# claudiotomasi/LearnMultigrid

Hardware: AMD Instinct MI355X
Metric: fine-level DoF*sweeps/s, 2-D Poisson V-cycle (higher is better)
Workload: dtype f64; 1 GPU; 2-D structured P1 Poisson 4096x4096 elements (16785409 DoF, 83861509 nnz, CSR fp64/int32), 6-level V(3,3) cycle, weighted Jacobi omega=0.80, tensor-product geometric transfer, Galerkin RAP by device SpGEMM; mode=vcycle, step=one full V-cycle, hipgraph=True, partition=row blocks of grid lines over 1 rank(s), sweep_variant=0, packed_csr=True, fine_level_format=stencil, problem=poisson, transfer=geometric

## Files before the change

include/lmg.h:

```cpp
#ifndef LMG_H
#define LMG_H

#include <stddef.h>
#include <stdint.h>

#ifdef __cplusplus
extern "C" {
#endif

#define LMG_VERSION 100

typedef enum {
    LMG_OK = 0,
    LMG_ERR_ARG = -1,
    LMG_ERR_ALIGN = -2,
    LMG_ERR_LAUNCH = -3,
    LMG_ERR_CAPACITY = -4,
    LMG_ERR_NODEVICE = -5
} lmg_status;

int lmg_version(void);
const char *lmg_status_string(int status);
int lmg_device_count(void);

int lmg_tune_set(const char *key, int value);
int lmg_tune_get(const char *key);

int64_t lmg_partials_count(int64_t n);

int lmg_csr_residual_norm2(int64_t n, int64_t nnz, const int32_t *d_rowptr, const int32_t *d_colidx,
                           const double *d_vals, const double *d_x, const double *d_b, double *d_r,
                           double *d_partials, double *d_norm2, void *stream);

int lmg_csr_jacobi(int64_t n, int64_t nnz, const int32_t *d_rowptr, const int32_t *d_colidx,
                   const double *d_vals, const double *d_x_in, const double *d_b, double omega,
                   double *d_x_out, void *stream);

int lmg_csr_spmv(int64_t n_rows, int64_t nnz, const int32_t *d_rowptr, const int32_t *d_colidx,
                 const double *d_vals, const double *d_x, double *d_y, double alpha, double beta,
                 void *stream);

int lmg_pcsr_tile_rows(void);
int lmg_pcsr_sweep(int mode, int64_t n, int64_t nnz, int32_t tile_rows, int32_t tile_cap,
                   const int32_t *d_tile_base,
                   const int32_t *d_tile_colbase, const uint8_t *d_rowlen, const void *d_col,
                   int colmode, const void *d_val, int valmode, const double *d_dict, int32_t ndict,
                   const double *d_x, const double *d_b, double *d_out, double alpha, double beta,
                   double *d_partials, double *d_norm2, void *stream);

int lmg_rpat_limits(int32_t *max_patterns, int32_t *max_entries);
int lmg_rpat_sweep(int mode, int64_t n, const uint8_t *d_pid, int32_t npat, int32_t nent, int32_t max_len,
                   const int32_t *d_pat_ptr, const int32_t *d_pat_off, const double *d_pat_val,
                   const double *d_x, const double *d_b, double *d_out, double alpha, double beta,
                   double *d_partials, double *d_norm2, void *stream);
int lmg_rpat_row_hash(int64_t n, const int32_t *d_rowptr, const int32_t *d_colidx, const double *d_vals,
                      uint64_t *d_hash, void *stream);
int lmg_rpat_claim(int64_t n, const uint8_t *d_pid, int32_t *d_rep, void *stream);
int lmg_rpat_verify(int64_t n, int64_t ncols, const int32_t *d_rowptr, const int32_t *d_colidx,
                    const double *d_vals, const uint8_t *d_pid, int32_t npat, const int32_t *d_pat_ptr,
                    const int32_t *d_pat_off, const double *d_pat_val, int32_t *d_mismatch, void *stream);

int lmg_rpat_sweep_grid(int mode, int64_t n, const int32_t *h_grid_map, const uint8_t *d_pid, int32_t npat,
                        int32_t nent, int32_t max_len, const int32_t *d_pat_ptr, const int32_t *d_pat_off,
                        const double *d_pat_val, const double *d_x, const double *d_b, double *d_out,
                        double alpha, double beta, double *d_partials, double *d_norm2, void *stream);
int lmg_rpat_row_hash_grid(int64_t n, const int32_t *h_grid_map, const int32_t *d_rowptr,
                           const int32_t *d_colidx, const double *d_vals, uint64_t *d_hash, void *stream);
int lmg_rpat_verify_grid(int64_t n, int64_t ncols, const int32_t *h_grid_map, const int32_t *d_rowptr,
                         const int32_t *d_colidx, const double *d_vals, const uint8_t *d_pid, int32_t npat,
                         const int32_t *d_pat_ptr, const int32_t *d_pat_off, const double *d_pat_val,
                         int32_t *d_mismatch, void *stream);

int lmg_stencil_limits(int32_t *max_patterns);
int lmg_stencil_sweep(int mode, int64_t n, int32_t line_stride, const uint8_t *d_pid, int32_t npat,
                      const double *d_st_val, const int32_t *d_st_mask, uint32_t union_mask, const double *d_x,
                      const double *d_b, double *d_out, double alpha, double beta, double *d_partials,
                      double *d_norm2, void *stream);

int lmg_stencil_smooth_supported(uint32_t union_mask);
int lmg_stencil_smooth(int64_t n, int32_t line_stride, const uint8_t *d_pid, int32_t npat,
                       const double *d_st_val, const int32_t *d_st_mask, uint32_t union_mask,
                       int32_t hot_pattern, const double *h_hot_val, int sweeps, const double *d_x_in,
                       const double *d_b, double omega, double *d_x_out, double *d_r_out, void *stream);

int lmg_stencil_smooth_tiled_supported(uint32_t union_mask);
int lmg_stencil_smooth_tiled(int64_t n, int32_t line_stride, const uint8_t *d_pid, int32_t npat,
                             const double *d_st_val, const int32_t *d_st_mask, uint32_t union_mask,
                             int32_t hot_pattern, const double *h_hot_val, int sweeps, const double *d_x_in,
                             const double *d_b, double omega, double *d_x_out, double *d_r_out, void *stream);
int lmg_stencil_smooth_tiled_prolong(int64_t n, int32_t line_stride, const uint8_t *d_pid, int32_t npat,
                                     const double *d_st_val, const int32_t *d_st_mask, uint32_t union_mask,
                                     int32_t hot_pattern, const double *h_hot_val, int sweeps, const double *d_x_in,
                                     const double *d_b, double omega, double *d_x_out, int64_t n_coarse,
                                     int32_t coarse_stride, const double *d_e_coarse, const uint8_t *d_p_pid,
                                     int32_t p_npat, const double *d_p_val, const int32_t *d_p_mask,
                                     const int32_t *h_hot_pairs, const double *h_hot_pval, void *stream);
int lmg_stencil_smooth_tiled_restrict(int64_t n, int32_t line_stride, const uint8_t *d_pid, int32_t npat,
                                      const double *d_st_val, const int32_t *d_st_mask, uint32_t union_mask,
                                      int32_t hot_pattern, const double *h_hot_val, int sweeps, const double *d_x_in,
                                      const double *d_b, double omega, double *d_x_out, int64_t n_coarse,
                                      int32_t coarse_stride, double *d_b_coarse, const uint8_t *d_r_pid,
                                      int32_t r_npat, const double *d_r_val, const int32_t *d_r_mask, int32_t hot_r,
                                      const double *h_hot_rval, void *stream);
int lmg_stencil_cheby_tiled(int64_t n, int32_t line_stride, const uint8_t *d_pid, int32_t npat,
                            const double *d_st_val, const int32_t *d_st_mask, uint32_t union_mask,
                            int32_t hot_pattern, const double *h_hot_val, int degree, const double *h_coef,
                            const double *d_x_in, const double *d_b, double *d_x_out, double *d_r_out, void *stream);
int lmg_stencil_cheby_tiled_prolong(int64_t n, int32_t line_stride, const uint8_t *d_pid, int32_t npat,
                                    const double *d_st_val, const int32_t *d_st_mask, uint32_t union_mask,
                                    int32_t hot_pattern, const double *h_hot_val, int degree, const double *h_coef,
                                    const double *d_x_in, const double *d_b, double *d_x_out, int64_t n_coarse,
                                    int32_t coarse_stride, const double *d_e_coarse, const uint8_t *d_p_pid,
                                    int32_t p_npat, const double *d_p_val, const int32_t *d_p_mask,
                                    const int32_t *h_hot_pairs, const double *h_hot_pval, void *stream);
int lmg_stencil_cheby_tiled_restrict(int64_t n, int32_t line_stride, const uint8_t *d_pid, int32_t npat,
                                     const double *d_st_val, const int32_t *d_st_mask, uint32_t union_mask,
                                     int32_t hot_pattern, const double *h_hot_val, int degree, const double *h_coef,
                                     const double *d_x_in, const double *d_b, double *d_x_out, int64_t n_coarse,
                                     int32_t coarse_stride, double *d_b_coarse, const uint8_t *d_r_pid,
                                     int32_t r_npat, const double *d_r_val, const int32_t *d_r_mask, int32_t hot_r,
                                     const double *h_hot_rval, void *stream);
int lmg_stencil_smooth_tiled_turnaround(int64_t n, int32_t line_stride, const uint8_t *d_pid, int32_t npat,
                                        const double *d_st_val, const int32_t *d_st_mask, uint32_t union_mask,
                                        int32_t hot_pattern, const double *h_hot_val, int sweeps_post, int sweeps_pre,
                                        const double *d_x_in, const double *d_b, double omega, double *d_x_out,
                                        int64_t n_coarse, int32_t coarse_stride, const double *d_e_coarse,
                                        const uint8_t *d_p_pid, int32_t p_npat, const double *d_p_val,
                                        const int32_t *d_p_mask, const int32_t *h_hot_pairs, const double *h_hot_pval,
                                        double *d_b_coarse, const uint8_t *d_r_pid, int32_t r_npat,
                                        const double *d_r_val, const int32_t *d_r_mask, int32_t hot_r,
                                        const double *h_hot_rval, void *stream);

int lmg_dia_smooth_supported(uint32_t union_mask);
int lmg_dia_fill(int64_t n, int32_t line_stride, const int32_t *d_rowptr, const int32_t *d_colidx, const double *d_vals,
                 uint32_t union_mask, double *d_dia, int32_t *d_mismatch, uint32_t *d_mask_out, void *stream);
int lmg_dia_smooth(int64_t n, int32_t line_stride, uint32_t union_mask, const double *d_dia, int sweeps,
                   const double *d_x_in, const double *d_b, double omega, double *d_x_out, double *d_r_out, void *stream);
int lmg_dia_cheby(int64_t n, int32_t line_stride, uint32_t union_mask, const double *d_dia, int degree,
                  const double *h_coef, const double *d_x_in, const double *d_b, double *d_x_out, double *d_r_out,
                  void *stream);
int lmg_dia_fill_f32(int64_t n, int32_t line_stride, const int32_t *d_rowptr, const int32_t *d_colidx, const double *d_vals,
                     uint32_t union_mask, float *d_dia, int32_t *d_mismatch, uint32_t *d_mask_out, void *stream);
int lmg_dia_smooth_f32(int64_t n, int32_t line_stride, uint32_t union_mask, const float *d_dia, int sweeps,
                       const double *d_x_in, const double *d_b, double omega, double *d_x_out, double *d_r_out,
                       void *stream);
int lmg_dia_cheby_f32(int64_t n, int32_t line_stride, uint32_t union_mask, const float *d_dia, int degree,
                      const double *h_coef, const double *d_x_in, const double *d_b, double *d_x_out, double *d_r_out,
                      void *stream);

int lmg_stencil_smooth_prolong_supported(uint32_t union_mask);
int lmg_stencil_smooth_prolong(int64_t n, int32_t line_stride, const uint8_t *d_pid, int32_t npat,
                               const double *d_st_val, const int32_t *d_st_mask, uint32_t union_mask,
                               int32_t hot_pattern, const double *h_hot_val, int sweeps, const double *d_x_in,
                               const double *d_b, double omega, double *d_x_out, int64_t n_coarse,
                               int32_t coarse_stride, const double *d_e_coarse, const uint8_t *d_p_pid,
                               int32_t p_npat, const double *d_p_val, const int32_t *d_p_mask,
                               const int32_t *h_hot_pairs, const double *h_hot_pval, void *stream);

int lmg_stencil_smooth_restrict(int64_t n, int32_t line_stride, const uint8_t *d_pid, int32_t npat,
                                const double *d_st_val, const int32_t *d_st_mask, uint32_t union_mask,
                                int32_t hot_pattern, const double *h_hot_val, int sweeps, const double *d_x_in,
                                const double *d_b, double omega, double *d_x_out, int64_t n_coarse,
                                int32_t coarse_stride, double *d_b_coarse, const uint8_t *d_r_pid,
                                int32_t r_npat, const double *d_r_val, const int32_t *d_r_mask, int32_t hot_r,
                                const double *h_hot_rval, void *stream);

int lmg_sell_sweep(int mode, int64_t n, const int64_t *d_slice_base, const int32_t *d_slice_len,
                   const int32_t *d_slice_cmin, const int32_t *d_rowlen, const void *d_col, int colmode,
                   const double *d_val, int32_t max_len, const double *d_x, const double *d_b, double *d_out,
                   double alpha, double beta, double *d_partials, double *d_norm2, void *stream);
int lmg_sell_slice_info(int64_t n, const int32_t *d_rowptr, const int32_t *d_colidx, int32_t *d_slice_len,
                        int32_t *d_cmin, int32_t *d_cmax, void *stream);
int lmg_sell_fill(int64_t n, const int32_t *d_rowptr, const int32_t *d_colidx, const double *d_vals,
                  const int64_t *d_slice_base, const int32_t *d_slice_cmin, int colmode, void *d_col_out,
                  double *d_val_out, void *stream);
int lmg_sell_sweep_f32(int mode, int64_t n, const int64_t *d_slice_base, const int32_t *d_slice_len,
                       const int32_t *d_slice_cmin, const int32_t *d_rowlen, const void *d_col, int colmode,
                       const float *d_val, int32_t max_len, const double *d_x, const double *d_b, double *d_out,
                       double alpha, double beta, double *d_partials, double *d_norm2, void *stream);
int lmg_sell_fill_f32(int64_t n, const int32_t *d_rowptr, const int32_t *d_colidx, const double *d_vals,
                      const int64_t *d_slice_base, const int32_t *d_slice_cmin, int colmode, void *d_col_out,
                      float *d_val_out, int32_t *d_flag, void *stream);

int64_t lmg_block_partials_count(int64_t n, int k);
int lmg_sell_sweep_block(int mode, int k, int64_t n, const int64_t *d_slice_base, const int32_t *d_slice_len,
                         const int32_t *d_slice_cmin, const int32_t *d_rowlen, const void *d_col, int colmode,
                         const double *d_val, int32_t max_len, const double *d_X, const double *d_B, double *d_Out,
                         double alpha, double beta, double *d_partials, double *d_norm2, void *stream);
int lmg_dense_gemv_block(int k, int64_t n, int64_t m, const double *d_M, const double *d_X, double *d_Y, void *stream);

int lmg_pcsr_tile_colrange(int64_t n, int32_t tile_rows, const int32_t *d_rowptr, const int32_t *d_colidx,
                           int32_t *d_cmin, int32_t *d_cmax, void *stream);
int lmg_pcsr_encode_cols16(int64_t n, int32_t tile_rows, const int32_t *d_rowptr, const int32_t *d_colidx,
                           const int32_t *d_colbase, uint16_t *d_out, void *stream);
int lmg_value_set_collect(const uint64_t *d_table, int64_t table_slots, uint64_t *d_out, int32_t cap, int32_t *d_count,
                          void *stream);
int lmg_value_set_insert(int64_t count, const double *d_vals, uint64_t *d_table, int64_t table_slots,
                         int32_t limit, int32_t *d_state, void *stream);
int lmg_value_encode(int64_t count, const double *d_vals, const double *d_dict, int32_t ndict, int width,
                     void *d_out, int32_t *d_missing, void *stream);
int lmg_csr_inverse_diagonal(int64_t n, const int32_t *d_rowptr, const int32_t *d_colidx, const double *d_vals,
                             double *d_dinv, void *stream);

int lmg_cheby_update(int64_t n, double a, double c, int first, const double *d_dinv, const double *d_r, double *d_d,
                     double *d_x, void *stream);
int lmg_csr_gershgorin(int64_t n, const int32_t *d_rowptr, const int32_t *d_colidx, const double *d_vals, double *d_lmax,
                       void *stream);

int lmg_line_factor(int64_t n, int32_t line_stride, int dir, const int32_t *d_rowptr, const int32_t *d_colidx,
                    const double *d_vals, double *d_lo, double *d_minv, double *d_cp, int32_t *d_flags, void *stream);
int lmg_line_solve(int64_t n, int32_t line_stride, int dir, int64_t first, int64_t step, const double *d_lo,
                   const double *d_minv, const double *d_cp, double *d_r, double omega, double *d_x, void *stream);

int lmg_line_factor_banded(int64_t n, int32_t line_stride, int dir, int band, const int32_t *d_rowptr,
                           const int32_t *d_colidx, const double *d_vals, double *d_fac, int32_t *d_flags, void *stream);
int lmg_line_solve_banded(int64_t n, int32_t line_stride, int dir, int band, int64_t first, int64_t step,
                          const double *d_fac, double *d_r, double omega, double *d_x, void *stream);

int lmg_csr_transpose_max_row(void);
int lmg_csr_transpose_count(int64_t nnz, int64_t ncols, const int32_t *d_colidx, int32_t *d_counts, void *stream);
int lmg_csr_transpose_fill(int64_t n, int64_t ncols, const int32_t *d_rowptr, const int32_t *d_colidx,
                           const double *d_vals, const int32_t *d_t_rowptr, int32_t *d_cursor, int32_t *d_t_colidx,
                           double *d_t_vals, void *stream);

int lmg_csr_gs_rows(const int32_t *d_rowptr, const int32_t *d_colidx, const double *d_vals,
                    double *d_x, const double *d_b, const int32_t *d_rows, int64_t nrows,
                    void *stream);

int lmg_csr_gs_schedule(const int32_t *d_rowptr, const int32_t *d_colidx, const double *d_vals,
                        double *d_x, const double *d_b, const int32_t *d_set_rows,
                        const int32_t *d_set_ptr, const int32_t *h_set_ptr, int64_t nsets,
                        int64_t max_set, int sweeps, void *stream);
int lmg_csr_gs_schedule_ell(int64_t n, const double *d_vals, double *d_x, const double *d_b, const int32_t *d_ell_row,
                            const int32_t *d_ell_start, const int32_t *d_ell_len, const int32_t *d_ell_cols,
                            int32_t ell_k, int64_t total_rows, const int32_t *d_set_ptr, int64_t nsets,
                            int sweeps, void *stream);

int lmg_stencil_gs_supported(uint32_t union_mask);
int64_t lmg_stencil_gs_work_bytes(int64_t n, int32_t line_stride);
int lmg_stencil_gs_sweep(int64_t n, int32_t line_stride, const uint8_t *d_pid, int32_t npat,
                         const double *d_st_val, const int32_t *d_st_mask, uint32_t union_mask,
                         int32_t hot_pattern, const double *h_hot_val, double *d_x, const double *d_b,
                         void *d_work, int sweeps, void *stream);
int lmg_stencil_gs_sweep_backward(int64_t n, int32_t line_stride, const uint8_t *d_pid, int32_t npat,
                                  const double *d_st_val, const int32_t *d_st_mask, uint32_t union_mask,
                                  int32_t hot_pattern, const double *h_hot_val, double *d_x, const double *d_b,
                                  void *d_work, int sweeps, void *stream);

int64_t lmg_host_gs_levels(int64_t n, const int32_t *h_rowptr, const int32_t *h_colidx,
                           int32_t *h_level_out);
int64_t lmg_host_greedy_colors(int64_t n, const int32_t *h_rowptr, const int32_t *h_colidx,
                               int32_t *h_color_out);
int64_t lmg_host_greedy_cf(int64_t n, const int32_t *h_rowptr, const int32_t *h_colidx, const double *h_vals,
                           int32_t *h_is_coarse_out);

int lmg_axpby(int64_t n, double alpha, const double *d_x, double beta, double *d_y, void *stream);
int lmg_vmul(int64_t n, double alpha, const double *d_x, const double *d_y, double *d_out, void *stream);
int lmg_copy(int64_t n, const double *d_src, double *d_dst, void *stream);
int lmg_zero(int64_t n, double *d_x, void *stream);
int lmg_dot(int64_t n, const double *d_x, const double *d_y, double *d_partials, double *d_out,
            void *stream);
int lmg_gather(int64_t n, const int32_t *d_idx, const double *d_x, double *d_buf, void *stream);
int lmg_scatter(int64_t n, const int32_t *d_idx, const double *d_buf, double *d_x, void *stream);

int lmg_krylov_max_vectors(void);
int64_t lmg_multi_partials_count(int64_t n, int k);
int lmg_multi_dot(int64_t n, int k, const double *d_V, int64_t ldv, const double *d_w, double *d_partials, double *d_out,
                  void *stream);
int lmg_multi_axpy(int64_t n, int k, int subtract, const double *d_V, int64_t ldv, const double *d_coef, double *d_w,
                   double *d_partials, double *d_norm2, void *stream);

int64_t lmg_block_dot_partials_count(int64_t n, int k);
int lmg_block_dot(int k, int64_t n, const double *d_X, const double *d_Y, double *d_partials, double *d_out, void *stream);
int lmg_block_cg_step(int k, int64_t n, const double *d_rz, const double *d_pAp, const double *d_tol2, double *d_mask,
                      const double *d_P, const double *d_AP, double *d_X, double *d_R, double *d_partials, double *d_rr,
                      void *stream);
int lmg_block_cg_direction(int k, int64_t n, const double *d_rz_new, const double *d_rz_old, const double *d_mask,
                           const double *d_Z, double *d_P, void *stream);

int64_t lmg_block_multi_partials_count(int64_t n, int k, int nb);
int lmg_block_multi_dot(int k, int64_t n, int nb, const double *d_V, int64_t ldb, const double *d_W, double *d_partials,
                        double *d_out, void *stream);
int lmg_block_multi_axpy(int k, int64_t n, const int *h_counts, int subtract, const double *d_V, int64_t ldb, const double *d_coef,
                         double *d_W, double *d_partials, double *d_norm2, void *stream);
int lmg_block_scale(int k, int64_t n, const double *h_scale, double *d_W, void *stream);

int lmg_dense_gemv(int64_t n, int64_t m, const double *d_M, const double *d_x, double *d_y,
                   void *stream);
int lmg_dense_gemv_blockdiag(int64_t nblocks, int64_t bs, const double *d_M, const double *d_x,
                             double *d_y, void *stream);

int lmg_dense_gemv_windows(int64_t nblocks, int64_t rows, int64_t cols, const double *d_M, const double *d_x,
                           int64_t x_stride, const double *d_z, int64_t z_stride, double alpha, double *d_y,
                           int64_t y_stride, void *stream);

int lmg_dense_gemv_windows_off(int64_t nblocks, int64_t rows, int64_t cols, const double *d_M, const double *d_x,
                               const int32_t *d_x_offsets, const double *d_z, int64_t z_stride, double alpha,
                               double *d_y, int64_t y_stride, void *stream);

int lmg_coarse_front(int64_t nblocks, int64_t bs, const double *d_M, const double *d_b, const int32_t *d_perm, double *d_y,
                     int64_t ntail, double *d_tail_out, void *stream);
int lmg_coarse_back(int64_t nblocks, int64_t rows, int64_t cols, const double *d_M, const double *d_x,
                    const int32_t *d_x_offsets, const double *d_z, int64_t z_stride, double alpha, const int32_t *d_perm,
                    double *d_out, int accumulate, int64_t ntail, void *stream);

int lmg_coarse_front_gather(int64_t nblocks, int64_t bs, const double *d_M, const double *d_b, const int32_t *d_idx,
                            double *d_y, int64_t ntail, const int32_t *d_tail_idx, double *d_tail_out, void *stream);
int lmg_coarse_back_gather(int64_t nblocks, int64_t rows, int64_t cols, const double *d_M, const double *d_x,
                           const int32_t *d_xidx, const double *d_z, int64_t z_stride, double alpha, const int32_t *d_oidx,
                           double *d_out, int accumulate, int64_t ntail, const int32_t *d_tail_idx, void *stream);

int lmg_batched_gemm(int64_t batch, int64_t M, int64_t N, int64_t K, double alpha, const double *d_A, int64_t lda,
                     int64_t stride_a, const double *d_B, int64_t ldb, int64_t stride_b, double beta, double *d_C,
                     int64_t ldc, int64_t stride_c, void *stream);
int lmg_copy2d(int64_t batch, int64_t rows, int64_t cols, double alpha, const double *d_src, int64_t ld_src,
               int64_t stride_src, double *d_dst, int64_t ld_dst, int64_t stride_dst, int accumulate, void *stream);

int lmg_pattern_parity_counts(int64_t n, int32_t line_stride, const uint8_t *d_pid, int32_t *d_counts, void *stream);
int lmg_block_copy(int64_t nblocks, int64_t bs, const double *d_src, int64_t src_stride, double *d_dst,
// ... 234 lines not shown
```

learnmultigrid_amd/_lib.py:

```python
import ctypes
import os
import subprocess

import torch

_HERE = os.path.dirname(os.path.abspath(__file__))
LIB_PATH = os.environ.get("LMG_LIB_PATH") or os.path.join(_HERE, "liblmg_hip.so")
CSRC = os.path.join(_HERE, "csrc")

_c = ctypes
_i64, _i32, _f64, _p, _cp = _c.c_int64, _c.c_int32, _c.c_double, _c.c_void_p, _c.c_char_p

SIGNATURES = {
    "lmg_version": (_c.c_int, []),
    "lmg_status_string": (_cp, [_c.c_int]),
    "lmg_device_count": (_c.c_int, []),
    "lmg_tune_set": (_c.c_int, [_cp, _c.c_int]),
    "lmg_tune_get": (_c.c_int, [_cp]),
    "lmg_partials_count": (_i64, [_i64]),
    "lmg_csr_residual_norm2": (_c.c_int, [_i64, _i64, _p, _p, _p, _p, _p, _p, _p, _p, _p]),
    "lmg_csr_jacobi": (_c.c_int, [_i64, _i64, _p, _p, _p, _p, _p, _f64, _p, _p]),
    "lmg_csr_spmv": (_c.c_int, [_i64, _i64, _p, _p, _p, _p, _p, _f64, _f64, _p]),
    "lmg_pcsr_tile_rows": (_c.c_int, []),
    "lmg_pcsr_sweep": (_c.c_int, [_c.c_int, _i64, _i64, _i32, _i32, _p, _p, _p, _p, _c.c_int, _p, _c.c_int, _p, _i32,
                                  _p, _p, _p, _f64, _f64, _p, _p, _p]),
    "lmg_rpat_limits": (_c.c_int, [_p, _p]),
    "lmg_rpat_sweep": (_c.c_int, [_c.c_int, _i64, _p, _i32, _i32, _i32, _p, _p, _p, _p, _p, _p, _f64, _f64, _p, _p, _p]),
    "lmg_rpat_row_hash": (_c.c_int, [_i64, _p, _p, _p, _p, _p]),
    "lmg_rpat_claim": (_c.c_int, [_i64, _p, _p, _p]),
    "lmg_rpat_verify": (_c.c_int, [_i64, _i64, _p, _p, _p, _p, _i32, _p, _p, _p, _p, _p]),
    "lmg_rpat_sweep_grid": (_c.c_int, [_c.c_int, _i64, _p, _p, _i32, _i32, _i32, _p, _p, _p, _p, _p, _p, _f64, _f64, _p, _p, _p]),
    "lmg_rpat_row_hash_grid": (_c.c_int, [_i64, _p, _p, _p, _p, _p, _p]),
    "lmg_rpat_verify_grid": (_c.c_int, [_i64, _i64, _p, _p, _p, _p, _p, _i32, _p, _p, _p, _p, _p]),
    "lmg_stencil_limits": (_c.c_int, [_p]),
    "lmg_stencil_sweep": (_c.c_int, [_c.c_int, _i64, _i32, _p, _i32, _p, _p, _c.c_uint32, _p, _p, _p, _f64, _f64, _p, _p, _p]),
    "lmg_stencil_smooth_supported": (_c.c_int, [_c.c_uint32]),
    "lmg_stencil_smooth": (_c.c_int, [_i64, _i32, _p, _i32, _p, _p, _c.c_uint32, _i32, _p, _c.c_int, _p, _p, _f64, _p, _p, _p]),
    "lmg_stencil_smooth_tiled_supported": (_c.c_int, [_c.c_uint32]),
    "lmg_stencil_smooth_tiled": (_c.c_int, [_i64, _i32, _p, _i32, _p, _p, _c.c_uint32, _i32, _p, _c.c_int, _p, _p, _f64, _p, _p, _p]),
    "lmg_stencil_smooth_tiled_prolong": (_c.c_int, [_i64, _i32, _p, _i32, _p, _p, _c.c_uint32, _i32, _p, _c.c_int, _p, _p, _f64, _p,
                                                    _i64, _i32, _p, _p, _i32, _p, _p, _p, _p, _p]),
    "lmg_stencil_smooth_tiled_restrict": (_c.c_int, [_i64, _i32, _p, _i32, _p, _p, _c.c_uint32, _i32, _p, _c.c_int, _p, _p, _f64, _p,
                                                     _i64, _i32, _p, _p, _i32, _p, _p, _i32, _p, _p]),
    "lmg_stencil_cheby_tiled": (_c.c_int, [_i64, _i32, _p, _i32, _p, _p, _c.c_uint32, _i32, _p, _c.c_int, _p, _p, _p, _p, _p, _p]),
    "lmg_stencil_cheby_tiled_prolong": (_c.c_int, [_i64, _i32, _p, _i32, _p, _p, _c.c_uint32, _i32, _p, _c.c_int, _p, _p, _p, _p,
                                                   _i64, _i32, _p, _p, _i32, _p, _p, _p, _p, _p]),
    "lmg_stencil_cheby_tiled_restrict": (_c.c_int, [_i64, _i32, _p, _i32, _p, _p, _c.c_uint32, _i32, _p, _c.c_int, _p, _p, _p, _p,
                                                    _i64, _i32, _p, _p, _i32, _p, _p, _i32, _p, _p]),
    "lmg_stencil_smooth_tiled_turnaround": (_c.c_int, [_i64, _i32, _p, _i32, _p, _p, _c.c_uint32, _i32, _p, _c.c_int, _c.c_int, _p,
                                                       _p, _f64, _p, _i64, _i32, _p, _p, _i32, _p, _p, _p, _p,
                                                       _p, _p, _i32, _p, _p, _i32, _p, _p]),
    "lmg_dia_smooth_supported": (_c.c_int, [_c.c_uint32]),
    "lmg_dia_fill": (_c.c_int, [_i64, _i32, _p, _p, _p, _c.c_uint32, _p, _p, _p, _p]),
    "lmg_dia_smooth": (_c.c_int, [_i64, _i32, _c.c_uint32, _p, _c.c_int, _p, _p, _f64, _p, _p, _p]),
    "lmg_dia_cheby": (_c.c_int, [_i64, _i32, _c.c_uint32, _p, _c.c_int, _p, _p, _p, _p, _p, _p]),
    "lmg_dia_fill_f32": (_c.c_int, [_i64, _i32, _p, _p, _p, _c.c_uint32, _p, _p, _p, _p]),
    "lmg_dia_smooth_f32": (_c.c_int, [_i64, _i32, _c.c_uint32, _p, _c.c_int, _p, _p, _f64, _p, _p, _p]),
    "lmg_dia_cheby_f32": (_c.c_int, [_i64, _i32, _c.c_uint32, _p, _c.c_int, _p, _p, _p, _p, _p, _p]),
    "lmg_stencil_smooth_prolong_supported": (_c.c_int, [_c.c_uint32]),
    "lmg_stencil_smooth_prolong": (_c.c_int, [_i64, _i32, _p, _i32, _p, _p, _c.c_uint32, _i32, _p, _c.c_int, _p, _p, _f64, _p,
                                              _i64, _i32, _p, _p, _i32, _p, _p, _p, _p, _p]),
    "lmg_stencil_smooth_restrict": (_c.c_int, [_i64, _i32, _p, _i32, _p, _p, _c.c_uint32, _i32, _p, _c.c_int, _p, _p, _f64, _p,
                                               _i64, _i32, _p, _p, _i32, _p, _p, _i32, _p, _p]),
    "lmg_sell_sweep": (_c.c_int, [_c.c_int, _i64, _p, _p, _p, _p, _p, _c.c_int, _p, _i32, _p, _p, _p, _f64, _f64, _p, _p, _p]),
    "lmg_sell_slice_info": (_c.c_int, [_i64, _p, _p, _p, _p, _p, _p]),
    "lmg_sell_fill": (_c.c_int, [_i64, _p, _p, _p, _p, _p, _c.c_int, _p, _p, _p]),
    "lmg_sell_sweep_f32": (_c.c_int, [_c.c_int, _i64, _p, _p, _p, _p, _p, _c.c_int, _p, _i32, _p, _p, _p, _f64, _f64, _p, _p, _p]),
    "lmg_sell_fill_f32": (_c.c_int, [_i64, _p, _p, _p, _p, _p, _c.c_int, _p, _p, _p, _p]),
    "lmg_block_partials_count": (_i64, [_i64, _c.c_int]),
    "lmg_sell_sweep_block": (_c.c_int, [_c.c_int, _c.c_int, _i64, _p, _p, _p, _p, _p, _c.c_int, _p, _i32, _p, _p, _p, _f64, _f64,
                                        _p, _p, _p]),
    "lmg_dense_gemv_block": (_c.c_int, [_c.c_int, _i64, _i64, _p, _p, _p, _p]),
    "lmg_pcsr_tile_colrange":(_c.c_int, [_i64, _i32, _p, _p, _p, _p, _p]),
    "lmg_pcsr_encode_cols16": (_c.c_int, [_i64, _i32, _p, _p, _p, _p, _p]),
    "lmg_value_set_collect": (_c.c_int, [_p, _i64, _p, _i32, _p, _p]),
    "lmg_value_set_insert": (_c.c_int, [_i64, _p, _p, _i64, _i32, _p, _p]),
    "lmg_value_encode": (_c.c_int, [_i64, _p, _p, _i32, _c.c_int, _p, _p, _p]),
    "lmg_csr_inverse_diagonal": (_c.c_int, [_i64, _p, _p, _p, _p, _p]),
    "lmg_cheby_update": (_c.c_int, [_i64, _f64, _f64, _c.c_int, _p, _p, _p, _p, _p]),
    "lmg_csr_gershgorin": (_c.c_int, [_i64, _p, _p, _p, _p, _p]),
    "lmg_line_factor": (_c.c_int, [_i64, _i32, _c.c_int, _p, _p, _p, _p, _p, _p, _p, _p]),
    "lmg_line_solve": (_c.c_int, [_i64, _i32, _c.c_int, _i64, _i64, _p, _p, _p, _p, _f64, _p, _p]),
    "lmg_line_factor_banded": (_c.c_int, [_i64, _i32, _c.c_int, _c.c_int, _p, _p, _p, _p, _p, _p]),
    "lmg_line_solve_banded": (_c.c_int, [_i64, _i32, _c.c_int, _c.c_int, _i64, _i64, _p, _p, _f64, _p, _p]),
    "lmg_csr_transpose_max_row": (_c.c_int, []),
    "lmg_csr_transpose_count": (_c.c_int, [_i64, _i64, _p, _p, _p]),
    "lmg_csr_transpose_fill": (_c.c_int, [_i64, _i64, _p, _p, _p, _p, _p, _p, _p, _p]),
    "lmg_csr_gs_rows": (_c.c_int, [_p, _p, _p, _p, _p, _p, _i64, _p]),
    "lmg_csr_gs_schedule": (_c.c_int, [_p, _p, _p, _p, _p, _p, _p, _p, _i64, _i64, _c.c_int, _p]),
    "lmg_csr_gs_schedule_ell": (_c.c_int, [_i64, _p, _p, _p, _p, _p, _p, _p, _i32, _i64, _p, _i64, _c.c_int, _p]),
    "lmg_stencil_gs_supported": (_c.c_int, [_c.c_uint32]),
    "lmg_stencil_gs_work_bytes": (_i64, [_i64, _i32]),
    "lmg_stencil_gs_sweep": (_c.c_int, [_i64, _i32, _p, _i32, _p, _p, _c.c_uint32, _i32, _p, _p, _p, _p, _c.c_int, _p]),
    "lmg_stencil_gs_sweep_backward": (_c.c_int, [_i64, _i32, _p, _i32, _p, _p, _c.c_uint32, _i32, _p, _p, _p, _p, _c.c_int, _p]),
    "lmg_host_gs_levels": (_i64, [_i64, _p, _p, _p]),
    "lmg_host_greedy_colors": (_i64, [_i64, _p, _p, _p]),
    "lmg_host_greedy_cf": (_i64, [_i64, _p, _p, _p, _p]),
    "lmg_axpby": (_c.c_int, [_i64, _f64, _p, _f64, _p, _p]),
    "lmg_vmul": (_c.c_int, [_i64, _f64, _p, _p, _p, _p]),
    "lmg_copy": (_c.c_int, [_i64, _p, _p, _p]),
    "lmg_zero": (_c.c_int, [_i64, _p, _p]),
    "lmg_dot": (_c.c_int, [_i64, _p, _p, _p, _p, _p]),
    "lmg_gather": (_c.c_int, [_i64, _p, _p, _p, _p]),
    "lmg_scatter": (_c.c_int, [_i64, _p, _p, _p, _p]),
    "lmg_krylov_max_vectors": (_c.c_int, []),
    "lmg_multi_partials_count": (_i64, [_i64, _c.c_int]),
    "lmg_multi_dot": (_c.c_int, [_i64, _c.c_int, _p, _i64, _p, _p, _p, _p]),
    "lmg_multi_axpy": (_c.c_int, [_i64, _c.c_int, _c.c_int, _p, _i64, _p, _p, _p, _p, _p]),
    "lmg_block_dot_partials_count": (_i64, [_i64, _c.c_int]),
    "lmg_block_dot": (_c.c_int, [_c.c_int, _i64, _p, _p, _p, _p, _p]),
    "lmg_block_cg_step": (_c.c_int, [_c.c_int, _i64, _p, _p, _p, _p, _p, _p, _p, _p, _p, _p, _p]),
    "lmg_block_cg_direction": (_c.c_int, [_c.c_int, _i64, _p, _p, _p, _p, _p, _p]),
    "lmg_block_multi_partials_count": (_i64, [_i64, _c.c_int, _c.c_int]),
    "lmg_block_multi_dot": (_c.c_int, [_c.c_int, _i64, _c.c_int, _p, _i64, _p, _p, _p, _p]),
    "lmg_block_multi_axpy": (_c.c_int, [_c.c_int, _i64, _p, _c.c_int, _p, _i64, _p, _p, _p, _p, _p]),
    "lmg_block_scale": (_c.c_int, [_c.c_int, _i64, _p, _p, _p]),
    "lmg_dense_gemv": (_c.c_int, [_i64, _i64, _p, _p, _p, _p]),
    "lmg_dense_gemv_blockdiag": (_c.c_int, [_i64, _i64, _p, _p, _p, _p]),
    "lmg_dense_gemv_windows": (_c.c_int, [_i64, _i64, _i64, _p, _p, _i64, _p, _i64, _f64, _p, _i64, _p]),
    "lmg_dense_gemv_windows_off": (_c.c_int, [_i64, _i64, _i64, _p, _p, _p, _p, _i64, _f64, _p, _i64, _p]),
    "lmg_coarse_front": (_c.c_int, [_i64, _i64, _p, _p, _p, _p, _i64, _p, _p]),
    "lmg_coarse_back": (_c.c_int, [_i64, _i64, _i64, _p, _p, _p, _p, _i64, _f64, _p, _p, _c.c_int, _i64, _p]),
    "lmg_coarse_front_gather": (_c.c_int, [_i64, _i64, _p, _p, _p, _p, _i64, _p, _p, _p]),
    "lmg_coarse_back_gather": (_c.c_int, [_i64, _i64, _i64, _p, _p, _p, _p, _i64, _f64, _p, _p, _c.c_int, _i64, _p, _p]),
    "lmg_batched_gemm": (_c.c_int, [_i64, _i64, _i64, _i64, _f64, _p, _i64, _i64, _p, _i64, _i64, _f64, _p, _i64, _i64, _p]),
    "lmg_copy2d": (_c.c_int, [_i64, _i64, _i64, _f64, _p, _i64, _i64, _p, _i64, _i64, _c.c_int, _p]),
    "lmg_pattern_parity_counts": (_c.c_int, [_i64, _i32, _p, _p, _p]),
    "lmg_block_copy": (_c.c_int, [_i64, _i64, _p, _i64, _p, _i64, _p]),
    "lmg_csr_to_dense": (_c.c_int, [_i64, _i64, _p, _p, _p, _p, _p]),
    "lmg_batched_inverse": (_c.c_int, [_i64, _i32, _p, _p, _p, _p]),
    "lmg_spgemm_count": (_c.c_int, [_i64, _p, _p, _p, _p, _p, _p]),
    "lmg_spgemm_symbolic": (_c.c_int, [_i64, _p, _p, _p, _p, _p, _i32, _p, _p]),
    "lmg_spgemm_numeric": (_c.c_int, [_i64, _p, _p, _p, _p, _p, _p, _p, _i32, _p, _p, _p, _p]),
    "lmg_spgemm_numeric_record": (_c.c_int, [_i64, _p, _p, _p, _p, _p, _p, _p, _i32, _p, _p, _p, _p, _p, _p, _p]),
    "lmg_spgemm_numeric_replay": (_c.c_int, [_i64, _p, _p, _p, _p, _p, _p, _i32, _p, _p, _p, _p, _p, _p]),
    "lmg_spgemm_long_rows": (_c.c_int, [_c.c_int, _i64, _p, _p, _p, _p, _p, _p, _p, _i64, _i32, _p, _p, _p, _p, _p, _p, _p]),
    "lmg_scan_scratch_count": (_i64, [_i64]),
    "lmg_exclusive_scan_i32": (_c.c_int, [_i64, _p, _p, _p, _p]),
    "lmg_p1_assemble_2d": (_c.c_int, [_i64, _p, _p, _p, _p, _p, _p, _p, _f64, _p, _p, _p, _p, _p, _p]),
    "lmg_l2_coupling_count": (_c.c_int, [_i64, _i64, _p, _p, _p, _p]),
    "lmg_l2_coupling_fill": (_c.c_int, [_c.c_int, _i64, _i64, _p, _p, _p, _p, _p, _p]),
    "lmg_l2p2d_limits": (_c.c_int, [_p, _p]),
    "lmg_l2p2d_cell_count": (_c.c_int, [_i64, _p, _p, _p, _p, _i32, _p, _p]),
    "lmg_l2p2d_cell_fill": (_c.c_int, [_i64, _p, _p, _p, _p, _i32, _i64, _p, _p, _p]),
    "lmg_l2p2d_cand_count": (_c.c_int, [_i64, _p, _p, _p, _i64, _p, _p, _p, _p, _i32, _p, _p, _p, _p]),
    "lmg_l2p2d_cand_fill": (_c.c_int, [_i64, _p, _p, _p, _i64, _p, _p, _p, _p, _i32, _p, _p, _i64, _i32, _p, _p, _p]),
    "lmg_l2p2d_rows_count": (_c.c_int, [_i64, _i64, _p, _p, _p, _p, _p, _p, _i64, _i64, _p, _p, _p, _p, _p, _f64, _p, _p]),
    "lmg_l2p2d_rows_fill": (_c.c_int, [_c.c_int, _i64, _i64, _p, _p, _p, _p, _p, _p, _i64, _i64, _p, _p, _p, _p, _p, _f64,
                                       _i64, _i32, _p, _p, _p, _p]),
    "lmg_nmg2d_check": (_c.c_int, [_i64, _p, _p, _p, _p, _p]),
    "lmg_nmg2d_count": (_c.c_int, [_i64, _p, _p, _p, _p, _p, _p, _p]),
    "lmg_nmg2d_patches": (_c.c_int, [_i64, _p, _p, _i64, _p, _p, _p, _p, _p, _p, _p, _p]),
    "lmg_nmg2d_contrib": (_c.c_int, [_i64, _i64, _i64, _p, _p, _p, _p, _p]),
    "lmg_nmg2d_fold": (_c.c_int, [_i64, _p, _p, _p, _p, _i64, _p, _p, _p, _p]),
    "lmg_nmg2d_normalize": (_c.c_int, [_i64, _p, _p, _p, _p]),
    "lmg_nmg2d_dneighs": (_c.c_int, [_i64, _p, _p, _p, _p, _p]),
    "lmg_nmg2d_cut_mark": (_c.c_int, [_i64, _p, _p, _p, _p, _p]),
    "lmg_nmg2d_cut_fill": (_c.c_int, [_i64, _p, _p, _p, _p, _p, _p, _p, _p]),
    "lmg_mesh2d_limits": (_c.c_int, [_p]),
    "lmg_mesh2d_construct": (_c.c_int, [_i64, _i64, _p, _p, _p, _p]),
    "lmg_mesh2d_check": (_c.c_int, [_i64, _i64, _p, _p, _p]),
    "lmg_mesh2d_edge_keys": (_c.c_int, [_i64, _p, _p, _p]),
    "lmg_mesh2d_edge_runs": (_c.c_int, [_i64, _i64, _p, _p, _p, _p, _p, _p]),
    "lmg_mesh2d_refine": (_c.c_int, [_i64, _i64, _i64, _p, _p, _p, _p, _p, _p, _p, _p, _p, _p]),
    "lmg_mesh2d_n2e_fill": (_c.c_int, [_i64, _p, _p, _p, _p]),
    "lmg_mesh2d_rows_count": (_c.c_int, [_i64, _i64, _p, _p, _p, _p, _p]),
    "lmg_mesh2d_rows_fill": (_c.c_int, [_i64, _i64, _p, _p, _p, _i64, _i32, _p, _p, _p]),
    "lmg_csr_identity_rows": (_c.c_int, [_i64, _p, _p, _p, _p, _p, _p, _p, _p]),
    "lmg_amg_strength_count": (_c.c_int, [_i64, _p, _p, _p, _f64, _p, _p]),
    "lmg_amg_strength_fill": (_c.c_int, [_i64, _p, _p, _p, _f64, _p, _p, _p]),
    "lmg_amg_pmis_keys": (_c.c_int, [_i64, _p, _p, _p, _p, _p, _p]),
    "lmg_amg_pmis_select": (_c.c_int, [_i64, _p, _p, _p, _p, _p, _p, _p, _p]),
    "lmg_amg_pmis_blocks": (_i64, [_i64]),
    "lmg_amg_pmis_update": (_c.c_int, [_i64, _p, _p, _p, _p, _p, _p, _p]),
    "lmg_amg_interp_count": (_c.c_int, [_i64, _p, _p, _p, _p, _p]),
    "lmg_amg_interp_fill": (_c.c_int, [_i64, _p, _p, _p, _p, _p, _p, _p, _p, _p, _p, _p, _p]),
    "lmg_amg_smooth_count": (_c.c_int, [_i64, _p, _p, _p, _p, _p, _p, _p, _p, _p, _p, _p, _f64, _f64, _p, _p]),
    "lmg_amg_smooth_fill": (_c.c_int, [_i64, _p, _p, _p, _p, _p, _p, _p, _p, _p, _p, _p, _f64, _f64, _p, _p, _p, _p]),
    "lmg_sa_diagonal": (_c.c_int, [_i64, _p, _p, _p, _p, _p]),
    "lmg_sa_strength_count": (_c.c_int, [_i64, _p, _p, _p, _p, _f64, _p, _p]),
    "lmg_sa_strength_fill": (_c.c_int, [_i64, _p, _p, _p, _p, _f64, _p, _p, _p]),
    "lmg_sa_graph_count": (_c.c_int, [_i64, _p, _p, _p, _p, _p, _p]),
    "lmg_sa_graph_fill": (_c.c_int, [_i64, _p, _p, _p, _p, _p, _p, _p]),
    "lmg_sa_mis2_init": (_c.c_int, [_i64, _p, _p, _p, _p]),
    "lmg_sa_mis2_t1": (_c.c_int, [_i64, _p, _p, _p, _p, _p]),
    "lmg_sa_mis2_t2": (_c.c_int, [_i64, _p, _p, _p, _p, _p, _p]),
    "lmg_sa_mis2_c1": (_c.c_int, [_i64, _p, _p, _p, _p, _p, _p]),
    "lmg_sa_blocks": (_i64, [_i64]),
    "lmg_sa_mis2_update": (_c.c_int, [_i64, _p, _p, _p, _p, _p, _p, _p, _p]),
    "lmg_sa_assign1": (_c.c_int, [_i64, _p, _p, _p, _p, _p, _p]),
    "lmg_sa_assign2": (_c.c_int, [_i64, _p, _p, _p, _p, _p, _p]),
    "lmg_sa_tentative_count": (_c.c_int, [_i64, _i64, _p, _p, _p]),
    "lmg_sa_tentative_pattern": (_c.c_int, [_i64, _i64, _p, _p, _p, _p, _p, _p]),
    "lmg_sa_norms": (_c.c_int, [_i64, _p, _p, _p, _p, _p, _p]),
    "lmg_sa_tentative_fill": (_c.c_int, [_i64, _i64, _p, _p, _p, _p, _p, _p]),
    "lmg_sa_row_states": (_c.c_int, [_i64, _p, _p, _p]),
    "lmg_color_select": (_c.c_int, [_i64, _p, _p, _p, _p, _p, _p, _p]),
    "lmg_color_blocks": (_i64, [_i64]),
    "lmg_color_assign": (_c.c_int, [_i64, _p, _p, _p, _p, _p, _p, _p, _p, _p]),
    "lmg_color_twin_count": (_c.c_int, [_i64, _i32, _p, _p, _p, _p, _p, _p, _p, _p]),
    "lmg_color_twin_fill": (_c.c_int, [_i64, _p, _p, _p, _p, _p, _p, _p, _p, _p]),
    "lmg_color_twin_refill": (_c.c_int, [_i64, _p, _p, _p, _p]),
    "lmg_color_sweep": (_c.c_int, [_i32, _p, _p, _p, _p, _p, _p, _p, _i32, _i64, _p, _p, _c.c_int, _c.c_int, _p]),
    "lmg_graph_begin": (_c.c_int, [_p]),
    "lmg_graph_end": (_c.c_int, [_p, _c.POINTER(_p)]),
    "lmg_graph_launch": (_c.c_int, [_p, _p]),
    "lmg_graph_destroy": (_c.c_int, [_p]),
}

_lib = None


class LmgError(RuntimeError):
    pass


# ... 33 lines not shown
```

learnmultigrid_amd/csrc/lmg_common.hpp:

```cpp
#pragma once
#include <hip/hip_runtime.h>
#include <limits.h>
#include <stdint.h>
#include <string.h>
#include <type_traits>
#include "lmg.h"

#define LMG_WAVE 64

#define LMG_CHECK_LAUNCH()                                          \
    do {                                                            \
        hipError_t e__ = hipGetLastError();                         \
        if (e__ != hipSuccess) return LMG_ERR_LAUNCH;               \
    } while (0)

static inline hipStream_t lmg_stream(void *s) { return reinterpret_cast<hipStream_t>(s); }
static inline bool lmg_aligned16(const void *p) { return (reinterpret_cast<uintptr_t>(p) & 15u) == 0; }

constexpr int kLmgBlock = 256;
constexpr int kLmgMaxGrid = 256 * 8;

static inline unsigned lmg_grid_for(int64_t n, int per_block)
{
    int64_t g = (n + per_block - 1) / per_block;
    if (g > kLmgMaxGrid) g = kLmgMaxGrid;
    if (g < 1) g = 1;
    return (unsigned)g;
}

enum { MODE_RESIDUAL = 0, MODE_JACOBI = 1, MODE_SPMV = 2 };

static inline int lmg_check_sweep_args(int mode, const double *x, const double *b, const double *out,
                                       const double *partials, const double *norm2)
{
    if (mode == MODE_SPMV) {
        if (!out || x == out) return LMG_ERR_ARG;
    } else if (mode == MODE_JACOBI) {
        if (!b || !out || x == out) return LMG_ERR_ARG;
    } else if (mode == MODE_RESIDUAL) {
        if (!b || (partials == nullptr) != (norm2 == nullptr) || (!out && !partials)) return LMG_ERR_ARG;
    } else {
        return LMG_ERR_ARG;
    }
    return LMG_OK;
}

int lmg_reduce_partials(const double *partials, int64_t count, double *norm2, hipStream_t st);
int lmg_reduce_partials_strided(const double *partials, int64_t count, int k, double *norm2, hipStream_t st);

__device__ __forceinline__ int lmg_xcd_tile(int tiles_per_xcd)
{
    return (int)(blockIdx.x & 7u) * tiles_per_xcd + (int)(blockIdx.x >> 3);
}
struct LmgXcdTiles {
    int begin, end, first, stride;
};
__device__ __forceinline__ LmgXcdTiles lmg_xcd_tiles(int tiles, int tiles_per_xcd)
{
    LmgXcdTiles o;
    const int xcd = (int)(blockIdx.x & 7u), slot = (int)(blockIdx.x >> 3);
    o.stride = (int)(gridDim.x >> 3);
    o.begin = xcd * tiles_per_xcd;
    o.end = min(tiles, o.begin + tiles_per_xcd);
    o.first = o.begin + slot;
    return o;
}
template <int BLOCK, typename Kernel>
static inline unsigned lmg_persistent_grid(Kernel kernel, size_t lds_bytes, int max_per_cu, int tune_per_cu,
                                           int tiles_per_xcd)
{
    int per_cu = 0;
    if (hipOccupancyMaxActiveBlocksPerMultiprocessor(&per_cu, kernel, BLOCK, lds_bytes) != hipSuccess || per_cu < 1)
        per_cu = 4;
    if (per_cu > max_per_cu) per_cu = max_per_cu;
    if (tune_per_cu > 0 && tune_per_cu < per_cu) per_cu = tune_per_cu;
    int64_t grid = 256 * (int64_t)per_cu;
    if (grid > (int64_t)tiles_per_xcd * 8) grid = (int64_t)tiles_per_xcd * 8;
    return (unsigned)grid;
}

__device__ __forceinline__ double lmg_wave_sum(double v)
{
#pragma unroll
    for (int off = LMG_WAVE / 2; off > 0; off >>= 1) v += __shfl_down(v, off, LMG_WAVE);
    return v;
}

template <int BLOCK>
__device__ __forceinline__ double lmg_block_sum(double v, double *s_red)
{
    v = lmg_wave_sum(v);
    const int lane = threadIdx.x & (LMG_WAVE - 1), wave = threadIdx.x / LMG_WAVE;
    if (lane == 0) s_red[wave] = v;
    __syncthreads();
    double tot = 0.0;
    if (threadIdx.x == 0) {
#pragma unroll
        for (int w = 0; w < BLOCK / LMG_WAVE; ++w) tot += s_red[w];
    }
    return tot;
}

template <int CTRL, bool BOUND_CTRL>
__device__ __forceinline__ double lmg_dpp_shift(double old, double src)
{
    const int lo = __builtin_amdgcn_update_dpp(__double2loint(old), __double2loint(src), CTRL, 0xf, 0xf, BOUND_CTRL);
    const int hi = __builtin_amdgcn_update_dpp(__double2hiint(old), __double2hiint(src), CTRL, 0xf, 0xf, BOUND_CTRL);
    return __hiloint2double(hi, lo);
}
template <bool BOUND_CTRL>
__device__ __forceinline__ double dpp_lower(double src)
{
    return lmg_dpp_shift<0x138, BOUND_CTRL>(0.0, src);
}
template <bool BOUND_CTRL>
__device__ __forceinline__ double dpp_upper(double src)
{
    return lmg_dpp_shift<0x130, BOUND_CTRL>(0.0, src);
}
__device__ __forceinline__ double dpp_from_lower_lane(double src, double lane0) { return lmg_dpp_shift<0x138, false>(lane0, src); }
__device__ __forceinline__ double dpp_from_upper_lane(double src, double lane63) { return lmg_dpp_shift<0x130, false>(lane63, src); }

typedef double d2 __attribute__((ext_vector_type(2)));
struct __attribute__((aligned(8))) d2u { double a, b; };

constexpr int kMaxPat = 64;
constexpr unsigned kMask9 = 0x1FFu;
constexpr unsigned kMask5 = 0x0BAu;
constexpr unsigned kMask1D = 0x038u;
constexpr unsigned kMask7a = 0x1BBu;
constexpr unsigned kMask7b = 0x0FEu;
constexpr unsigned kMaskUpper = 0x007u;
constexpr unsigned kMaskLower = 0x1C0u;
constexpr unsigned kMaskCorners = 0x145u;
constexpr unsigned kMaskOffLine = kMaskUpper | kMaskLower;



struct LmgTuneKey {
    const char *key;
    int *value;
    int lo, hi;
    int nlist, list[6];
};
constexpr LmgTuneKey lmg_tune_range(const char *key, int *value, int lo, int hi = INT_MAX)
{
    return {key, value, lo, hi, 0, {}};
}
template <typename... V>
constexpr LmgTuneKey lmg_tune_list(const char *key, int *value, V... v)
{
    return {key, value, 0, 0, (int)sizeof...(V), {v...}};
}
constexpr LmgTuneKey kLmgTuneEnd = {nullptr, nullptr, 0, 0, 0, {}};
extern const LmgTuneKey lmg_tune_sweep[], lmg_tune_pcsr[], lmg_tune_rpat[], lmg_tune_stencil[], lmg_tune_fused[],
    lmg_tune_tile[], lmg_tune_dia[], lmg_tune_sell[], lmg_tune_gsw[], lmg_tune_gs[];

static inline const LmgTuneKey *lmg_tune_find(const LmgTuneKey *table, const char *key)
{
    for (; table->key; ++table)
        if (strcmp(table->key, key) == 0) return table;
    return nullptr;
}
static inline bool lmg_tune_accepts(const LmgTuneKey &k, int v)
{
    if (k.nlist == 0) return v >= k.lo && v <= k.hi;
    for (int i = 0; i < k.nlist; ++i)
        if (k.list[i] == v) return true;
    return false;
}

template <int LO, int HI, typename F>
int lmg_with_sweeps(int sweeps, F &&f)
{
    if constexpr (LO < HI) {
        if (sweeps == LO) return f(std::integral_constant<int, LO>{});
        return lmg_with_sweeps<LO + 1, HI>(sweeps, f);
    } else {
        return f(std::integral_constant<int, HI>{});
    }
}
template <typename F>
int lmg_with_flag(bool flag, F &&f)
{
    return flag ? f(std::true_type{}) : f(std::false_type{});
}
template <unsigned... M, typename F>
int lmg_with_mask(uint32_t union_mask, F &&f)
{
    int rc = LMG_ERR_CAPACITY;
    (void)((union_mask == M && (rc = f(std::integral_constant<unsigned, M>{}), true)) || ...);
    return rc;
}
#define LMG_CT(c) decltype(c)::value

struct LmgOperator {
    int64_t n;
    int32_t line_stride;
    const uint8_t *pid;
    int32_t npat;
    const double *st_val;
    const int32_t *st_mask;
    uint32_t union_mask;
    int32_t hot_pattern;
    const double *h_hot_val;
};
struct LmgSolve {
    int sweeps;
    const double *x_in, *b;
    double omega;
    double *x_out, *r_out;
};
struct LmgProl {
    int64_t n_coarse;
    int32_t coarse_stride;
    const double *e_coarse;
    const uint8_t *p_pid;
    int32_t p_npat;
    const double *p_val;
    const int32_t *p_mask;
    const int32_t *h_hot_pairs;
    const double *h_hot_pval;
};
struct LmgRest {
    int64_t n_coarse;
    int32_t coarse_stride;
    double *b_coarse;
    const uint8_t *r_pid;
    int32_t r_npat;
    const double *r_val;
    const int32_t *r_mask;
    int32_t hot_r;
    const double *h_hot_rval;
};

static inline bool lmg_hot_usable(int32_t hot_pattern, int32_t npat, const double *h_hot_val)
{
    return hot_pattern >= 0 && hot_pattern < npat && h_hot_val && h_hot_val[4] != 0.0;
}

template <typename A>
int lmg_smooth_fill(A &a, const LmgOperator &op, const LmgSolve &v)
{
    const int64_t n = op.n;
    if (n < 0 || n >= A::kRowLimit || op.npat < 1 || op.npat > kMaxPat || (op.union_mask & ~kMask9)) return LMG_ERR_ARG;
    if (v.sweeps < 1 || v.sweeps > 3) return LMG_ERR_ARG;
    if (n == 0) return LMG_OK;
    if (A::kOneRowIsCapacity && n < 2) return LMG_ERR_CAPACITY;
    if (!op.pid || !op.st_val || !op.st_mask || !v.b || !v.x_out || v.x_in == v.x_out || v.r_out == v.x_out ||
        (v.r_out && v.r_out == v.x_in))
        return LMG_ERR_ARG;
    if (op.line_stride < 3 || op.line_stride > n) return LMG_ERR_ARG;
    a.n = (int)n;
    a.W = op.line_stride;
    a.lines = (int)((n + op.line_stride - 1) / op.line_stride);
    a.npat = op.npat;
    a.pid = op.pid;
    a.st_val = op.st_val;
    a.st_mask = op.st_mask;
    a.x = v.x_in;
    a.b = v.b;
    a.out = v.x_out;
    a.r = v.r_out;
    a.omega = v.omega;
    const bool hot = lmg_hot_usable(op.hot_pattern, op.npat, op.h_hot_val);
    a.hot = hot ? op.hot_pattern : -1;
    for (int k = 0; k < 9; ++k) a.hot_val[k] = hot ? op.h_hot_val[k] : 0.0;
    a.hot_rdiag = hot ? 1.0 / op.h_hot_val[4] : 0.0;
    a.ec = nullptr;
    a.nc = a.Wc = 0;
    a.ppid = nullptr;
    a.pp_val = nullptr;
    a.pp_mask = nullptr;
    a.pp_npat = 0;
    a.bc = nullptr;
    a.rpid = nullptr;
    a.rp_val = nullptr;
    a.rp_mask = nullptr;
    a.rp_npat = 0;
    a.phot[0] = a.phot[1] = a.rhot = -1;
    for (int k = 0; k < 9; ++k) a.phv[k] = a.rhv[k] = 0.0;
    return 1;
}

template <typename A>
int lmg_prol_check(const LmgOperator &op, const LmgSolve &v, const LmgProl &p)
{
    if (!v.x_in || !p.e_coarse || !p.p_pid || !p.p_val || !p.p_mask || p.p_npat < 1 || p.p_npat > kMaxPat) return LMG_ERR_ARG;
// ... 69 lines not shown
```

learnmultigrid_amd/csrc/stencil_fused.hip:

```cpp
#include "lmg_common.hpp"

#ifndef LMG_FUSED_NT_REST
#define LMG_FUSED_NT_REST 3
#endif
#ifndef LMG_FUSED_NT_PROL
#define LMG_FUSED_NT_PROL 0
#endif
#ifndef LMG_FUSED_NT_PLAIN
#define LMG_FUSED_NT_PLAIN 0
#endif

namespace {

constexpr int kBlock = 256;
constexpr int kWavesPerBlock = kBlock / LMG_WAVE;
constexpr int kStripCols = 2 * LMG_WAVE;

struct MArgs {
    static constexpr int64_t kRowLimit = (1ll << 29) - 4096;
    static constexpr bool kOneRowIsCapacity = true;
    static constexpr int64_t kProlMinCoarse = 1;
    static constexpr bool kProlStrideCovers = true, kProlChecksPairs = false;
    static constexpr int64_t kRestCoarseLimit = 1ll << 28;
    int n;
    int W;
    int lines;
    int npat;
    unsigned umask;
    int strips, segs, seg_lines;
    int items;
    int nb_strips;
    int segs_b, seg_lines_b;
    int edge_lines;
    int allow_fast;
    const unsigned char *pid;
    const double *st_val;
    const int *st_mask;
    const double *x;
    const double *b;
    double *out;
    double *r;
    double omega;
    int hot;
    double hot_val[9];
    double hot_rdiag;
    const double *ec;
    int nc, Wc;
    const unsigned char *ppid;
    const double *pp_val;
    const int *pp_mask;
    int pp_npat;
    int phot[2];
    double phv[9];
    double *bc;
    const unsigned char *rpid;
    const double *rp_val;
    const int *rp_mask;
    int rp_npat;
    int rhot;
    double rhv[9];
};

template <int H, bool PROL, bool REST> struct StripGeom {
    static constexpr bool EVEN = true;
    static constexpr int MLmin = REST ? H + 1 : H, MRmin = REST ? H + 1 : (PROL ? H + 2 : H);
    static constexpr int ML = EVEN ? ((MLmin + 1) & ~1) : MLmin;
    static constexpr int U = EVEN ? ((kStripCols - ML - MRmin) & ~1) : kStripCols - ML - MRmin;
};

struct Line {
    d2 x, b;
    double e;
    int pp;
    int rp;
    int praw;
    int ok;
};

typedef unsigned int u4 __attribute__((ext_vector_type(4)));
typedef unsigned int u2 __attribute__((ext_vector_type(2)));
constexpr unsigned kOOB = 0xFFFFFFF0u;

template <bool SIDES>
__device__ __forceinline__ void window(const d2 &c, double (&w)[4])
{
    w[1] = c.x;
    w[2] = c.y;
    if (SIDES) {
        w[0] = dpp_lower<true>(c.y);
        w[3] = dpp_upper<true>(c.x);
    } else {
        w[0] = w[3] = 0.0;
    }
}

template <unsigned UM>
__device__ __forceinline__ void apply_rows(const double *s_val, int pA, int pB, int mA, int mB,
                                           const d2 &u, const d2 &c, const d2 &d, double &accA, double &accB)
{
    constexpr bool DIAG = (UM & kMaskCorners) != 0;
    double wu[4], wc[4], wd[4];
    window<true>(c, wc);
    window<DIAG>(u, wu);
    window<DIAG>(d, wd);
    accA = 0.0;
    accB = 0.0;
#pragma unroll
    for (int s = 0; s < 9; ++s) {
        if (!((UM >> s) & 1u)) continue;
        const int cc = s / 3, dd = s % 3;
        const double *w = cc == 0 ? wu : (cc == 1 ? wc : wd);
        const double vA = s_val[pA * 9 + s], vB = s_val[pB * 9 + s];
        const double tA = accA + vA * w[dd], tB = accB + vB * w[dd + 1];
        accA = ((mA >> s) & 1) ? tA : accA;
        accB = ((mB >> s) & 1) ? tB : accB;
    }
}

template <unsigned UM>
__device__ __forceinline__ void apply_rows_hot(const double (&hv)[9], const d2 &u, const d2 &c,
                                               const d2 &d, double &accA, double &accB)
{
    constexpr bool DIAG = (UM & kMaskCorners) != 0;
    double wu[4], wc[4], wd[4];
    window<true>(c, wc);
    window<DIAG>(u, wu);
    window<DIAG>(d, wd);
    accA = 0.0;
    accB = 0.0;
#pragma unroll
    for (int s = 0; s < 9; ++s) {
        if (!((UM >> s) & 1u)) continue;
        const int cc = s / 3, dd = s % 3;
        const double *w = cc == 0 ? wu : (cc == 1 ? wc : wd);
        accA = accA + hv[s] * w[dd];
        accB = accB + hv[s] * w[dd + 1];
    }
}

#ifdef LMG_FUSED_TRACE
__device__ unsigned long long g_fused_trace[64 * 8];
__device__ int g_fused_trace_item;
#define LMG_TRACE(slot)                                                                                   \
    do {                                                                                                  \
        if (FAST && trace_me && (t - y_begin) < 64) g_fused_trace[(t - y_begin) * 8 + (slot)] = __builtin_readcyclecounter(); \
    } while (0)
#else
#define LMG_TRACE(slot)
#endif
#ifdef LMG_FUSED_WAVETIME
__device__ unsigned long long g_fused_wavetime[2 * LMG_FUSED_WAVETIME];
#endif

constexpr int kUF = 6;
constexpr int kNBR = 6;

struct Item {
    int strip, out_y0, out_y1;
};

__device__ __forceinline__ Item decode_item(const MArgs &a, int item)
{
    Item it;
    const int nb_items = a.nb_strips * a.segs_b;
    if (item < nb_items) {
        const int sb = item / a.segs_b, k = item - sb * a.segs_b;
        it.strip = sb == 0 ? 0 : a.strips - 1;
        it.out_y0 = k * a.seg_lines_b;
        it.out_y1 = min(a.lines, it.out_y0 + a.seg_lines_b);
        return it;
    }
    const int k = item - nb_items, ns = a.strips - a.nb_strips;
    const int seg = k / ns;
    it.strip = k - seg * ns + (a.nb_strips > 0 ? 1 : 0);
    if (a.edge_lines > 0) {
        if (seg == 0) {
            it.out_y0 = 0;
            it.out_y1 = a.edge_lines;
        } else if (seg == 1) {
            it.out_y0 = a.lines - a.edge_lines;
            it.out_y1 = a.lines;
        } else {
            it.out_y0 = a.edge_lines + (seg - 2) * a.seg_lines;
            it.out_y1 = min(a.lines - a.edge_lines, it.out_y0 + a.seg_lines);
        }
    } else {
        it.out_y0 = seg * a.seg_lines;
        it.out_y1 = min(a.lines, it.out_y0 + a.seg_lines);
    }
    return it;
}

struct Tables {
    const double *val;
    const int *mask;
    const double *rdiag;
    const double *pv;
    const int *pm;
    const double *rv;
    const int *rm;
};

template <int S, unsigned UM, bool RESID, bool ZERO, int PF, bool PROL, bool REST, bool FAST>
__device__ __forceinline__ void fused_march(const MArgs &a, const Tables &T, const int lane, const int strip, const int out_y0,
                                            const int out_y1)
{
    constexpr int H = S + (RESID ? 1 : 0) - (ZERO ? 1 : 0);
    const double *s_val = T.val;
    const int *s_mask = T.mask;
    const double *s_rdiag = T.rdiag;
    const double *s_pv = T.pv;
    const int *s_pm = T.pm;
    const double *s_rv = T.rv;
    const int *s_rm = T.rm;
    constexpr int U = StripGeom<H, PROL, REST>::U, ML = StripGeom<H, PROL, REST>::ML;
    constexpr int HL = H + (REST ? 1 : 0);
    const int n = a.n;
    const int64_t W = a.W;
    const int c0 = strip * U - ML;
    const int y_begin = out_y0 - HL - ((out_y0 - HL) & 1), y_end = out_y1 + HL;
    const int cidx = 2 * lane;
    const bool colA = cidx >= ML && cidx < ML + U && c0 + cidx < W;
    const bool colB = cidx + 1 >= ML && cidx + 1 < ML + U && c0 + cidx + 1 < W;
    const double omega = a.omega;
    const int hot2 = a.hot >= 0 ? (FAST ? (a.hot | (a.hot << 8)) : (a.hot | (a.hot << 8) | (3 << 16))) : -1;
    double hv[9];
#pragma unroll
    for (int s = 0; s < 9; ++s) hv[s] = a.hot_val[s];
    const double hrd = a.hot_rdiag;
    double hp[9];
#pragma unroll
    for (int s = 0; s < 9; ++s) hp[s] = PROL ? a.phv[s] : 0.0;
    const int okbits = FAST ? 0 : (3 << 16);
    const int hotq_even = (PROL && a.phot[0] >= 0) ? (a.phot[0] | okbits) : -1;
    const int hotq_odd = (PROL && a.phot[1] >= 0) ? (a.phot[1] | okbits) : -1;
    double e_prev = 0.0;

    const unsigned lane16 = (unsigned)lane * 16u, lane8 = (unsigned)lane * 8u, lane2 = (unsigned)lane * 2u;
    const unsigned st_off_ab = (colA && colB) ? lane16 : kOOB;
    const unsigned st_off_a = (colA && !colB) ? lane16 : kOOB;
    const unsigned st_off_c = colA ? lane8 : kOOB;

    constexpr int NTL = REST ? LMG_FUSED_NT_REST : (PROL ? LMG_FUSED_NT_PROL : LMG_FUSED_NT_PLAIN);
    auto fetch = [&](int y, Line &L) {
        if (FAST) {
#ifdef LMG_FUSED_HALOPROBE
            const int64_t i0 = (int64_t)min(max(y, out_y0), out_y1 - 1) * W + c0;
#else
            const int64_t i0 = (int64_t)y * W + c0;
#endif
            L.ok = 3;
            const unsigned short *pp2 = reinterpret_cast<const unsigned short *>(reinterpret_cast<const char *>(a.pid + i0) + lane2);
            L.praw = (int)((NTL & 4) ? __builtin_nontemporal_load(pp2) : *pp2);
            typedef double dv2 __attribute__((ext_vector_type(2), aligned(8)));
            const dv2 *pb = reinterpret_cast<const dv2 *>(reinterpret_cast<const char *>(a.b + i0) + lane16);
            const dv2 bb = (NTL & 1) ? __builtin_nontemporal_load(pb) : *pb;
            L.b.x = bb.x;
            L.b.y = bb.y;
            if (!ZERO) {
                const dv2 *px = reinterpret_cast<const dv2 *>(reinterpret_cast<const char *>(a.x + i0) + lane16);
                const dv2 xx = (NTL & 2) ? __builtin_nontemporal_load(px) : *px;
                L.x.x = xx.x;
                L.x.y = xx.y;
            } else {
                L.x.x = L.x.y = 0.0;
            }
            if (PROL) {
                unsigned short twop;
                __builtin_memcpy(&twop, reinterpret_cast<const char *>(a.ppid + i0) + lane2, 2);
                L.pp = (int)twop;
                const int64_t jc0 = (int64_t)((y + 1) >> 1) * a.Wc + (c0 >> 1);
                L.e = *reinterpret_cast<const double *>(reinterpret_cast<const char *>(a.ec + jc0) + lane8);
            } else {
                L.pp = 0;
                L.e = 0.0;
            }
            if (REST) {
                const int64_t jr0 = (int64_t)((y - S) >> 1) * a.Wc + (c0 >> 1);
                L.rp = (int)*(reinterpret_cast<const unsigned char *>(a.rpid + jr0) + lane);
            } else {
                L.rp = 0;
            }
            return;
        }
        const bool line_ok = y < y_end;
        const int yc = min(max(y, 0), a.lines - 1);
        const int64_t i = (int64_t)y * W + c0 + cidx;
        const bool okA = line_ok && i >= 0 && i < n, okB = line_ok && i + 1 >= 0 && i + 1 < n;
        const int64_t j = min(max(i, (int64_t)0), (int64_t)n - 2);
        L.ok = (okA ? 1 : 0) | (okB ? 2 : 0) | (i == -1 ? 4 : 0) | (i == (int64_t)n - 1 ? 8 : 0);
        unsigned short two;
        __builtin_memcpy(&two, a.pid + j, 2);
        L.praw = (int)two;
        const d2u bb = *reinterpret_cast<const d2u *>(a.b + j);
        L.b.x = bb.a;
        L.b.y = bb.b;
        if (!ZERO) {
            const d2u xx = *reinterpret_cast<const d2u *>(a.x + j);
            L.x.x = xx.a;
            L.x.y = xx.b;
        } else {
            L.x.x = L.x.y = 0.0;
        }
        if (PROL) {
            unsigned short twop;
            __builtin_memcpy(&twop, a.ppid + j, 2);
            L.pp = (int)twop;
            const int64_t jc = (int64_t)((yc + 1) >> 1) * a.Wc + (c0 >> 1) + lane;
            L.e = a.ec[min(max(jc, (int64_t)0), (int64_t)a.nc - 1)];
        } else {
            L.pp = 0;
            L.e = 0.0;
        }
        if (REST) {
            const int64_t jr = (int64_t)((y - S) >> 1) * a.Wc + (c0 >> 1) + lane;
            L.rp = (int)a.rpid[min(max(jr, (int64_t)0), (int64_t)a.nc - 1)];
        } else {
            L.rp = 0;
        }
    };
    const __amdgpu_buffer_rsrc_t rs_out = __builtin_amdgcn_make_buffer_rsrc(a.out, 0, (int)((unsigned)n * 8u), 0x00020000);
    const __amdgpu_buffer_rsrc_t rs_r = __builtin_amdgcn_make_buffer_rsrc((RESID && !REST) ? a.r : a.out, 0, (int)((unsigned)n * 8u), 0x00020000);
    const __amdgpu_buffer_rsrc_t rs_bc = __builtin_amdgcn_make_buffer_rsrc(REST ? a.bc : a.out, 0, (int)((unsigned)(REST ? a.nc : n) * 8u), 0x00020000);
    double hr[9];
#pragma unroll
    for (int s = 0; s < 9; ++s) hr[s] = REST ? a.rhv[s] : 0.0;
    double acc_cur = 0.0;
    int rp_cur = 0, rp_now = 0;
    bool st_cur = false, hot_cur = false;
    bool sty_cur = false;
    auto store2 = [&](const __amdgpu_buffer_rsrc_t &rs, double *base, int y, int p2, double va, double vb) {
        const bool yok = y >= out_y0 && y < out_y1;
        u4 v4;
        v4.x = (unsigned)__double2loint(va);
        v4.y = (unsigned)__double2hiint(va);
        v4.z = (unsigned)__double2loint(vb);
        v4.w = (unsigned)__double2hiint(vb);
        if (FAST) {
            const __amdgpu_buffer_rsrc_t rl = __builtin_amdgcn_make_buffer_rsrc(base + ((int64_t)y * W + c0), 0, yok ? 8 * kStripCols : 0, 0x00020000);
            __builtin_amdgcn_raw_buffer_store_b128(v4, rl, st_off_ab, 0, 0);
            u2 v2;
            v2.x = v4.x;
            v2.y = v4.y;
            __builtin_amdgcn_raw_buffer_store_b64(v2, rl, st_off_a, 0, 0);
            return;
        }
        const int64_t i = (int64_t)y * W + c0 + cidx;
        const bool stA = yok && colA && ((p2 >> 16) & 1), stB = yok && colB && ((p2 >> 17) & 1);
        __builtin_amdgcn_raw_buffer_store_b128(v4, rs, (stA && stB) ? (unsigned)i * 8u : kOOB, 0, 0);
        u2 v2;
        v2.x = stA ? v4.x : v4.z;
        v2.y = stA ? v4.y : v4.w;
        __builtin_amdgcn_raw_buffer_store_b64(v2, rs, (stA != stB) ? (unsigned)(stA ? i : i + 1) * 8u : kOOB, 0, 0);
    };

    d2 X[S + 1][3];
    d2 Bq[kNBR];
    int Pq[kNBR];
    bool Hq[kNBR];
    const d2 zero2 = {0.0, 0.0};
#pragma unroll
    for (int s = 0; s <= S; ++s) X[s][0] = X[s][1] = X[s][2] = zero2;
#pragma unroll
    for (int k = 0; k < kNBR; ++k) {
        Bq[k] = zero2;
        Pq[k] = 0;
        Hq[k] = false;
    }

    Line pre[PF];
#pragma unroll
    for (int u = 0; u < PF; ++u) fetch(y_begin + u, pre[u]);

    const int t_last = out_y1 - 1 + S + (RESID ? 1 : 0) + (REST ? 1 : 0);
#ifdef LMG_FUSED_TRACE
    const bool trace_me = lane == 0 && strip == g_fused_trace_item / 100000 && out_y0 <= g_fused_trace_item % 100000 &&
                          g_fused_trace_item % 100000 < out_y1;
#endif
    for (int tb = y_begin; tb <= t_last; tb += kUF) {
#pragma unroll
        for (int u = 0; u < kUF; ++u) {
            const int t = tb + u;
            LMG_TRACE(0);
            const int q0 = u % kNBR;
            {
                const Line &L = pre[u % PF];
                const bool okA = FAST || (L.ok & 1), okB = FAST || (L.ok & 2), up = !FAST && (L.ok & 4), down = !FAST && (L.ok & 8);
                d2 bv, xv;
                int pa, pb;
                if (FAST) {
                    bv = L.b;
                    xv = L.x;
                    pa = L.praw & 0xff;
                    pb = L.praw >> 8;
                } else {
                    bv.x = okA ? (down ? L.b.y : L.b.x) : 0.0;
                    bv.y = okB ? (up ? L.b.x : L.b.y) : 0.0;
                    xv.x = okA ? (down ? L.x.y : L.x.x) : 0.0;
                    xv.y = okB ? (up ? L.x.x : L.x.y) : 0.0;
                    pa = down ? (L.praw >> 8) & 0xff : L.praw & 0xff;
                    pb = up ? L.praw & 0xff : (L.praw >> 8) & 0xff;
                }
                if (REST) rp_now = L.rp;
                if (PROL) {
                    const bool odd = (u & 1) != 0;
                    int qa, qb, q2;
                    if (FAST) {
                        qa = L.pp & 0xff;
                        qb = L.pp >> 8;
                        q2 = L.pp;
                    } else {
                        qa = down ? (L.pp >> 8) & 0xff : L.pp & 0xff;
                        qb = up ? L.pp & 0xff : (L.pp >> 8) & 0xff;
                        q2 = (okA ? qa : 0) | ((okB ? qb : 0) << 8) | ((L.ok & 3) << 16);
                    }
                    const double en = L.e;
                    const double e0 = odd ? e_prev : en, e1 = en;
                    const double e0r = dpp_upper<true>(e0), e1r = dpp_upper<true>(e1);
                    double accA, accB;
                    if (__all(q2 == (odd ? hotq_odd : hotq_even))) {
                        if (!odd) {
                            accA = 0.0 + hp[0] * e0;
                            accB = (0.0 + hp[1] * e0) + hp[2] * e0r;
                        } else {
                            accA = (0.0 + hp[3] * e0) + hp[4] * e1;
                            accB = (((0.0 + hp[5] * e0) + hp[6] * e0r) + hp[7] * e1) + hp[8] * e1r;
                        }
                    } else {
                        const int mA = s_pm[qa], mB = s_pm[qb];
                        const double w[4] = {e0, e0r, e1, e1r};
                        accA = 0.0;
                        accB = 0.0;
#pragma unroll
                        for (int k = 0; k < 4; ++k) {
                            const double tA = accA + s_pv[qa * 4 + k] * w[k], tB = accB + s_pv[qb * 4 + k] * w[k];
                            accA = ((mA >> k) & 1) ? tA : accA;
                            accB = ((mB >> k) & 1) ? tB : accB;
                        }
                    }
                    xv.x = okA ? xv.x + accA : 0.0;
                    xv.y = okB ? xv.y + accB : 0.0;
                    e_prev = en;
                }
                Bq[q0] = bv;
                X[0][u % 3] = xv;
                Pq[q0] = FAST ? L.praw : ((okA ? pa : 0) | ((okB ? pb : 0) << 8) | ((L.ok & 3) << 16));
                Hq[q0] = __all(Pq[q0] == hot2);
            }
            LMG_TRACE(1);
            fetch(t + PF, pre[u % PF]);
            LMG_TRACE(2);
#pragma unroll
            for (int s = 1; s <= S; ++s) {
                const int q = ((u - s) % kNBR + kNBR) % kNBR;
                const int xm = ((u - s - 1) % 3 + 3) % 3, xc = ((u - s) % 3 + 3) % 3, xp = ((u - s + 1) % 3 + 3) % 3;
                const int p2 = Pq[q];
                const d2 bq = Bq[q];
                d2 nx;
                if (Hq[q]) {
                    if (ZERO && s == 1) {
                        nx.x = omega * (hrd * bq.x);
                        nx.y = omega * (hrd * bq.y);
                    } else {
                        double accA, accB;
                        apply_rows_hot<UM>(hv, X[s - 1][xm], X[s - 1][xc], X[s - 1][xp], accA, accB);
                        nx.x = X[s - 1][xc].x + omega * (hrd * (bq.x - accA));
                        nx.y = X[s - 1][xc].y + omega * (hrd * (bq.y - accB));
                    }
                } else {
                    const int pA = p2 & 0xff, pB = (p2 >> 8) & 0xff;
                    const int mA = s_mask[pA], mB = s_mask[pB];
                    if (ZERO && s == 1) {
                        nx.x = omega * (s_rdiag[pA] * bq.x);
                        nx.y = omega * (s_rdiag[pB] * bq.y);
                    } else {
                        double accA, accB;
                        apply_rows<UM>(s_val, pA, pB, mA, mB, X[s - 1][xm], X[s - 1][xc], X[s - 1][xp], accA, accB);
                        const double xa = X[s - 1][xc].x, xb = X[s - 1][xc].y;
                        const double rA = bq.x - accA, rB = bq.y - accB;
                        nx.x = (mA >> 16) ? xa : xa + omega * (s_rdiag[pA] * rA);
                        nx.y = (mB >> 16) ? xb : xb + omega * (s_rdiag[pB] * rB);
                    }
                    if (!FAST) {
                        if (!((p2 >> 16) & 1)) nx.x = 0.0;
                        if (!((p2 >> 17) & 1)) nx.y = 0.0;
                    }
                }
                X[s][xc] = nx;
                if (s == S) store2(rs_out, a.out, t - S, p2, nx.x, nx.y);
                LMG_TRACE(2 + s);
            }
            if (RESID) {
                const int y = t - S - 1;
                const int q = ((u - S - 1) % kNBR + kNBR) % kNBR;
                const int xm = ((u - S - 2) % 3 + 3) % 3, xc = ((u - S - 1) % 3 + 3) % 3, xp = ((u - S) % 3 + 3) % 3;
                const int p2 = Pq[q];
                double accA, accB;
                if (Hq[q]) {
                    apply_rows_hot<UM>(hv, X[S][xm], X[S][xc], X[S][xp], accA, accB);
                } else {
                    const int pA = p2 & 0xff, pB = (p2 >> 8) & 0xff;
                    apply_rows<UM>(s_val, pA, pB, s_mask[pA], s_mask[pB], X[S][xm], X[S][xc], X[S][xp], accA, accB);
                }
                if (!REST) {
                    store2(rs_r, a.r, y, p2, Bq[q].x - accA, Bq[q].y - accB);
                } else {
                    const double rA = Bq[q].x - accA, rB = Bq[q].y - accB;
                    const double wl[3] = {dpp_lower<true>(rB), rA, rB};
                    const bool y_odd = ((u - S - 1) & 1) != 0;
                    unsigned off_bc = kOOB;
                    bool emit_line = false;
                    double emit = 0.0;
                    if (!y_odd) {
                        if (hot_cur) {
#pragma unroll
                            for (int k = 0; k < 3; ++k) acc_cur = acc_cur + hr[3 + k] * wl[k];
                        } else {
                            const int mk = s_rm[rp_cur];
#pragma unroll
                            for (int k = 0; k < 3; ++k) {
                                const double tv = acc_cur + s_rv[rp_cur * 9 + 3 + k] * wl[k];
                                acc_cur = ((mk >> (3 + k)) & 1) ? tv : acc_cur;
                            }
                        }
                    } else {
                        if (hot_cur) {
#pragma unroll
                            for (int k = 0; k < 3; ++k) acc_cur = acc_cur + hr[6 + k] * wl[k];
                        } else {
                            const int mk = s_rm[rp_cur];
#pragma unroll
                            for (int k = 0; k < 3; ++k) {
                                const double tv = acc_cur + s_rv[rp_cur * 9 + 6 + k] * wl[k];
                                acc_cur = ((mk >> (6 + k)) & 1) ? tv : acc_cur;
                            }
                        }
                        emit = acc_cur;
                        emit_line = sty_cur;
                        if (!FAST && st_cur) off_bc = (unsigned)(((y - 1) >> 1) * a.Wc + (c0 >> 1) + lane) * 8u;
                        rp_cur = rp_now;
                        sty_cur = y + 1 >= out_y0 && y + 1 < out_y1;
                        st_cur = sty_cur && colA;
                        hot_cur = __all(!st_cur || rp_cur == a.rhot);
                        acc_cur = 0.0;
                        if (hot_cur) {
#pragma unroll
                            for (int k = 0; k < 3; ++k) acc_cur = acc_cur + hr[k] * wl[k];
                        } else {
                            const int mk = s_rm[rp_cur];
#pragma unroll
                            for (int k = 0; k < 3; ++k) {
                                const double tv = acc_cur + s_rv[rp_cur * 9 + k] * wl[k];
                                acc_cur = ((mk >> k) & 1) ? tv : acc_cur;
                            }
                        }
                    }
                    u2 v2;
                    v2.x = (unsigned)__double2loint(emit);
                    v2.y = (unsigned)__double2hiint(emit);
                    if (FAST) {
                        const __amdgpu_buffer_rsrc_t rl = __builtin_amdgcn_make_buffer_rsrc(
                            a.bc + ((int64_t)((y - 1) >> 1) * a.Wc + (c0 >> 1)), 0, (y_odd && emit_line) ? 8 * LMG_WAVE : 0, 0x00020000);
                        __builtin_amdgcn_raw_buffer_store_b64(v2, rl, st_off_c, 0, 0);
                    } else {
                        __builtin_amdgcn_raw_buffer_store_b64(v2, rs_bc, off_bc, 0, 0);
                    }
                }
            }
            LMG_TRACE(7);
        }
    }
}

template <int S, unsigned UM, bool RESID, bool ZERO, int PF, bool PROL = false, bool REST = false>
__global__ void __launch_bounds__(kBlock, (REST && S >= 3) ? 2 : 3) stencil_fused_kernel(MArgs a)
{
    static_assert(!PROL || (!RESID && !ZERO), "the correction is fused into post-smoothing passes only");
    static_assert(!REST || (RESID && !PROL), "the restriction replaces the store of the residual");
    static_assert(kUF % 3 == 0 && kUF % kNBR == 0 && kUF % PF == 0 && S + 2 <= kNBR, "ring periods");
    constexpr int H = S + (RESID ? 1 : 0) - (ZERO ? 1 : 0);
    __shared__ double s_val[kMaxPat * 9];
    __shared__ int s_mask[kMaxPat];
    __shared__ double s_rdiag[kMaxPat];
    __shared__ double s_pv[PROL ? kMaxPat * 4 : 1];
    __shared__ int s_pm[PROL ? kMaxPat : 1];
    __shared__ double s_rv[REST ? kMaxPat * 9 : 1];
    __shared__ int s_rm[REST ? kMaxPat : 1];

    const int t_ = threadIdx.x;
    for (int i = t_; i < a.npat * 9; i += kBlock) s_val[i] = a.st_val[i];
    for (int i = t_; i < a.npat; i += kBlock) {
        const int m = a.st_mask[i];
        const double dg = (m & 16) ? a.st_val[i * 9 + 4] : 0.0;
        s_rdiag[i] = dg != 0.0 ? 1.0 / dg : 0.0;
        s_mask[i] = dg == 0.0 ? (m | (1 << 16)) : m;
    }
    if (PROL) {
        for (int i = t_; i < a.pp_npat * 4; i += kBlock) s_pv[i] = a.pp_val[i];
        for (int i = t_; i < a.pp_npat; i += kBlock) s_pm[i] = a.pp_mask[i];
    }
    if (REST) {
        for (int i = t_; i < a.rp_npat * 9; i += kBlock) s_rv[i] = a.rp_val[i];
        for (int i = t_; i < a.rp_npat; i += kBlock) s_rm[i] = a.rp_mask[i];
    }
    __syncthreads();

    const int lane = t_ & (LMG_WAVE - 1);
    const int item = (int)blockIdx.x * kWavesPerBlock + __builtin_amdgcn_readfirstlane(t_ >> 6);
    if (item >= a.items) return;
    const Item it = decode_item(a, item);
    const Tables T = {s_val, s_mask, s_rdiag, s_pv, s_pm, s_rv, s_rm};

    constexpr int U = StripGeom<H, PROL, REST>::U, ML = StripGeom<H, PROL, REST>::ML;
    constexpr int HL = H + (REST ? 1 : 0);
    const int c0 = it.strip * U - ML;
    const int y_begin = it.out_y0 - HL - ((it.out_y0 - HL) & 1);
    const int t_last = it.out_y1 - 1 + S + (RESID ? 1 : 0) + (REST ? 1 : 0);
    const int y_fetch = y_begin + ((t_last - y_begin) / kUF + 1) * kUF - 1 + PF;
    bool fast = a.allow_fast && y_begin >= (REST ? S + 2 : 1) && y_fetch <= a.lines - 2 &&
                (int64_t)y_begin * a.W + c0 >= 0 && (int64_t)y_fetch * a.W + c0 + kStripCols < (int64_t)a.n;
    if (PROL) fast = fast && (int64_t)((y_fetch + 1) >> 1) * a.Wc + (c0 >> 1) + LMG_WAVE <= (int64_t)a.nc;
    if (REST) fast = fast && (int64_t)((y_fetch - S) >> 1) * a.Wc + (c0 >> 1) + LMG_WAVE <= (int64_t)a.nc;
#ifdef LMG_FUSED_WAVETIME
    const unsigned long long wt0 = __builtin_amdgcn_s_memrealtime();
#endif
    if (fast) fused_march<S, UM, RESID, ZERO, PF, PROL, REST, true>(a, T, lane, it.strip, it.out_y0, it.out_y1);
    else fused_march<S, UM, RESID, ZERO, PF, PROL, REST, false>(a, T, lane, it.strip, it.out_y0, it.out_y1);
#ifdef LMG_FUSED_WAVETIME
    if (lane == 0 && item < LMG_FUSED_WAVETIME) {
        g_fused_wavetime[2 * item] = wt0;
        g_fused_wavetime[2 * item + 1] = (__builtin_amdgcn_s_memrealtime() & ~3ull) | (fast ? 1ull : 0ull) | 2ull;
    }
#endif
}

int g_fused_seg_lines = 0;
int g_fused_seg_min_lines = 0;
int g_fused_seg_max_lines = 0x7fffffff;
int g_fused_pf = 0;
int g_fused_seg_lines_prol = 0;
int g_fused_seg_lines_rest = 0;
int g_fused_want_waves = 5120;
int g_fused_want_waves_rest3 = 2700;
int g_fused_floor_halos = 4;
int g_fused_balance = 1;
int g_fused_slow_pct = 55;
int g_fused_fast = 1;

template <int S, unsigned UM, bool RESID, bool ZERO, bool PROL = false, bool REST = false>
int launch4(MArgs a, hipStream_t st)
{
    constexpr int H = S + (RESID ? 1 : 0) - (ZERO ? 1 : 0);
    constexpr int U = StripGeom<H, PROL, REST>::U;
    constexpr int HL = H + (REST ? 1 : 0);
    a.strips = (a.W + U - 1) / U;
    int seg_lines = (a.lines >= g_fused_seg_min_lines && a.lines <= g_fused_seg_max_lines) ? g_fused_seg_lines : 0;
    if (PROL && g_fused_seg_lines_prol > 0) seg_lines = g_fused_seg_lines_prol;
    if (REST && g_fused_seg_lines_rest > 0) seg_lines = g_fused_seg_lines_rest;
    if (seg_lines <= 0) {
        const int want = ((REST || PROL) && S >= 3 && !ZERO) ? g_fused_want_waves_rest3 : g_fused_want_waves;
        const int want_segs = (want + a.strips - 1) / a.strips;
        seg_lines = (a.lines + want_segs - 1) / want_segs;
        const int floor_lines = H > 0 ? g_fused_floor_halos * H : 4;
        if (seg_lines < floor_lines) seg_lines = floor_lines;
    }
    a.seg_lines = seg_lines;
    a.allow_fast = g_fused_fast;
    a.nb_strips = 0;
    a.segs_b = 1;
    a.seg_lines_b = seg_lines;
    a.edge_lines = 0;
    if (g_fused_balance) {
        const int steps = seg_lines + 2 * HL;
        int slow = (steps * g_fused_slow_pct) / 100 - 2 * HL;
        if (slow < 2) slow = 2;
        if (slow < seg_lines) {
            a.nb_strips = a.strips < 2 ? a.strips : 2;
            a.seg_lines_b = slow;
            a.segs_b = (a.lines + slow - 1) / slow;
            int edge = slow < HL + 2 + kUF + 2 ? HL + 2 + kUF + 2 : slow;
            if (a.strips > a.nb_strips && a.lines >= 2 * edge + seg_lines) a.edge_lines = edge;
        }
    }
    if (a.edge_lines > 0) a.segs = 2 + (a.lines - 2 * a.edge_lines + seg_lines - 1) / seg_lines;
    else a.segs = (a.lines + seg_lines - 1) / seg_lines;
    a.items = a.nb_strips * a.segs_b + (a.strips - a.nb_strips) * a.segs;
    const int grid = (a.items + kWavesPerBlock - 1) / kWavesPerBlock;
    hipLaunchKernelGGL((stencil_fused_kernel<S, UM, RESID, ZERO, 2, PROL, REST>), dim3((unsigned)grid), dim3(kBlock), 0, st, a);
    LMG_CHECK_LAUNCH();
    return LMG_OK;
}

template <unsigned UM>
int launch_plain(MArgs a, int sweeps, bool resid, bool zero, hipStream_t st)
{
    return lmg_with_sweeps<1, 3>(sweeps, [&](auto s) {
        return lmg_with_flag(resid, [&](auto r) {
            return lmg_with_flag(zero, [&](auto z) { return launch4<LMG_CT(s), UM, LMG_CT(r), LMG_CT(z)>(a, st); });
        });
    });
}

template <unsigned UM>
int launch_prol(MArgs a, int sweeps, hipStream_t st)
{
    return lmg_with_sweeps<1, 3>(sweeps, [&](auto s) { return launch4<LMG_CT(s), UM, false, false, true>(a, st); });
}

template <unsigned UM>
int launch_rest(MArgs a, int sweeps, bool zero, hipStream_t st)
{
    return lmg_with_sweeps<1, 3>(sweeps, [&](auto s) {
        return lmg_with_flag(zero, [&](auto z) { return launch4<LMG_CT(s), UM, true, LMG_CT(z), false, true>(a, st); });
    });
}

MArgs own_fields(uint32_t union_mask)
{
    MArgs a;
    a.umask = union_mask;
    a.strips = a.segs = a.seg_lines = 0;
    a.items = a.nb_strips = a.edge_lines = a.allow_fast = 0;
    a.segs_b = a.seg_lines_b = 1;
    return a;
}

}

constexpr LmgTuneKey lmg_tune_fused[] = {
    lmg_tune_range("fused_seg_lines", &g_fused_seg_lines, 0),
    lmg_tune_range("fused_seg_min_lines", &g_fused_seg_min_lines, 0),
    lmg_tune_range("fused_seg_max_lines", &g_fused_seg_max_lines, 0),
    lmg_tune_list("fused_pf", &g_fused_pf, 0, 2),
    lmg_tune_range("fused_seg_lines_prol", &g_fused_seg_lines_prol, 0),
    lmg_tune_range("fused_seg_lines_rest", &g_fused_seg_lines_rest, 0),
    lmg_tune_range("fused_want_waves", &g_fused_want_waves, 1),
    lmg_tune_range("fused_want_waves_rest3", &g_fused_want_waves_rest3, 1),
    lmg_tune_range("fused_floor_halos", &g_fused_floor_halos, 1),
    lmg_tune_list("fused_balance", &g_fused_balance, 0, 1),
    lmg_tune_range("fused_slow_pct", &g_fused_slow_pct, 10, 100),
    lmg_tune_list("fused_fast", &g_fused_fast, 0, 1),
    kLmgTuneEnd,
};

extern "C" {

int lmg_stencil_smooth(int64_t n, int32_t line_stride, const uint8_t *pid, int32_t npat, const double *st_val,
                       const int32_t *st_mask, uint32_t union_mask, int32_t hot_pattern, const double *h_hot_val,
                       int sweeps, const double *x_in, const double *b, double omega, double *x_out, double *r_out,
                       void *stream)
{
    return lmg_fused_pass<kMask5, kMask9, kMask1D>(
        own_fields(union_mask), {n, line_stride, pid, npat, st_val, st_mask, union_mask, hot_pattern, h_hot_val},
        {sweeps, x_in, b, omega, x_out, r_out}, nullptr, nullptr, [&](const MArgs &a, auto m) {
            return launch_plain<LMG_CT(m)>(a, sweeps, r_out != nullptr, x_in == nullptr, lmg_stream(stream));
        });
}

int lmg_stencil_smooth_prolong(int64_t n, int32_t line_stride, const uint8_t *pid, int32_t npat, const double *st_val,
                               const int32_t *st_mask, uint32_t union_mask, int32_t hot_pattern, const double *h_hot_val,
                               int sweeps, const double *x_in, const double *b, double omega, double *x_out,
                               int64_t n_coarse, int32_t coarse_stride, const double *e_coarse, const uint8_t *p_pid,
                               int32_t p_npat, const double *p_val, const int32_t *p_mask, const int32_t *h_hot_pairs,
                               const double *h_hot_pval, void *stream)
{
    const LmgProl p = {n_coarse, coarse_stride, e_coarse, p_pid, p_npat, p_val, p_mask, h_hot_pairs, h_hot_pval};
    return lmg_fused_pass<kMask5, kMask9>(
        own_fields(union_mask), {n, line_stride, pid, npat, st_val, st_mask, union_mask, hot_pattern, h_hot_val},
        {sweeps, x_in, b, omega, x_out, nullptr}, &p, nullptr,
        [&](const MArgs &a, auto m) { return launch_prol<LMG_CT(m)>(a, sweeps, lmg_stream(stream)); });
}

int lmg_stencil_smooth_restrict(int64_t n, int32_t line_stride, const uint8_t *pid, int32_t npat, const double *st_val,
                                const int32_t *st_mask, uint32_t union_mask, int32_t hot_pattern, const double *h_hot_val,
                                int sweeps, const double *x_in, const double *b, double omega, double *x_out,
                                int64_t n_coarse, int32_t coarse_stride, double *b_coarse, const uint8_t *r_pid,
                                int32_t r_npat, const double *r_val, const int32_t *r_mask, int32_t hot_r,
                                const double *h_hot_rval, void *stream)
{
    const LmgRest r = {n_coarse, coarse_stride, b_coarse, r_pid, r_npat, r_val, r_mask, hot_r, h_hot_rval};
    return lmg_fused_pass<kMask5, kMask9>(
        own_fields(union_mask), {n, line_stride, pid, npat, st_val, st_mask, union_mask, hot_pattern, h_hot_val},
        {sweeps, x_in, b, omega, x_out, nullptr}, nullptr, &r,
        [&](const MArgs &a, auto m) { return launch_rest<LMG_CT(m)>(a, sweeps, x_in == nullptr, lmg_stream(stream)); });
}

int lmg_stencil_smooth_supported(uint32_t union_mask)
{
    return union_mask == kMask5 || union_mask == kMask9 || union_mask == kMask1D;
}

int lmg_stencil_smooth_prolong_supported(uint32_t union_mask)
{
    return union_mask == kMask5 || union_mask == kMask9;
}

}
```

learnmultigrid_amd/csrc/vec.hip:

```cpp
#include "lmg_common.hpp"

namespace {

__global__ void __launch_bounds__(kLmgBlock) axpby_kernel(int64_t n, double alpha, const double *x,
                                                          double beta, double *y)
{
    const int64_t n2 = n >> 1;
    const int64_t stride = (int64_t)gridDim.x * kLmgBlock;
    const double2 *x2 = reinterpret_cast<const double2 *>(x);
    double2 *y2 = reinterpret_cast<double2 *>(y);
    for (int64_t i = (int64_t)blockIdx.x * kLmgBlock + threadIdx.x; i < n2; i += stride) {
        const double2 xv = x2[i];
        double2 yv;
        if (beta == 0.0) {
            yv.x = alpha * xv.x;
            yv.y = alpha * xv.y;
        } else {
            yv = y2[i];
            yv.x = alpha * xv.x + beta * yv.x;
            yv.y = alpha * xv.y + beta * yv.y;
        }
        y2[i] = yv;
    }
    if ((n & 1) && blockIdx.x == 0 && threadIdx.x == 0) {
        const int64_t i = n - 1;
        y[i] = (beta == 0.0) ? alpha * x[i] : alpha * x[i] + beta * y[i];
    }
}

__global__ void __launch_bounds__(kLmgBlock) vmul_kernel(int64_t n, double alpha, const double *x,
                                                         const double *y, double *out)
{
    const int64_t stride = (int64_t)gridDim.x * kLmgBlock;
    for (int64_t i = (int64_t)blockIdx.x * kLmgBlock + threadIdx.x; i < n; i += stride)
        out[i] = alpha * (x[i] * y[i]);
}

template <bool FIRST>
__global__ void __launch_bounds__(kLmgBlock) cheby_update_kernel(int64_t n, double a, double c, const double *dinv,
                                                                 const double *r, double *d, double *x)
{
    const int64_t n2 = n >> 1;
    const int64_t stride = (int64_t)gridDim.x * kLmgBlock;
    const double2 *dinv2 = reinterpret_cast<const double2 *>(dinv), *r2 = reinterpret_cast<const double2 *>(r);
    double2 *d2 = reinterpret_cast<double2 *>(d), *x2 = reinterpret_cast<double2 *>(x);
    for (int64_t i = (int64_t)blockIdx.x * kLmgBlock + threadIdx.x; i < n2; i += stride) {
        const double2 iv = dinv2[i], rv = r2[i];
        double2 xv = x2[i], dv;
        if (FIRST) {
            dv.x = c * (iv.x * rv.x);
            dv.y = c * (iv.y * rv.y);
        } else {
            dv = d2[i];
            dv.x = a * dv.x + c * (iv.x * rv.x);
            dv.y = a * dv.y + c * (iv.y * rv.y);
        }
        xv.x = xv.x + dv.x;
        xv.y = xv.y + dv.y;
        d2[i] = dv;
        x2[i] = xv;
    }
    if ((n & 1) && blockIdx.x == 0 && threadIdx.x == 0) {
        const int64_t i = n - 1;
        const double z = c * (dinv[i] * r[i]);
        const double dv = FIRST ? z : a * d[i] + z;
        d[i] = dv;
        x[i] = x[i] + dv;
    }
}

__global__ void __launch_bounds__(kLmgBlock) csr_gershgorin_kernel(int64_t n, const int *rowptr, const int *colidx,
                                                                   const double *vals, unsigned long long *out)
{
    const int64_t stride = (int64_t)gridDim.x * kLmgBlock;
    double m = 0.0;
    for (int64_t row = (int64_t)blockIdx.x * kLmgBlock + threadIdx.x; row < n; row += stride) {
        double sum = 0.0, dg = 0.0;
        for (int e = rowptr[row]; e < rowptr[row + 1]; ++e) {
            const double v = vals[e];
            sum += fabs(v);
            if (colidx[e] == row) dg += v;
        }
        if (dg != 0.0) {
            const double q = sum / fabs(dg);
            m = q > m ? q : m;
        }
    }
#pragma unroll
    for (int off = LMG_WAVE / 2; off > 0; off >>= 1) {
        const double o = __shfl_down(m, off, LMG_WAVE);
        m = o > m ? o : m;
    }
    if ((threadIdx.x & (LMG_WAVE - 1)) == 0 && m > 0.0) atomicMax(out, (unsigned long long)__double_as_longlong(m));
}

__global__ void __launch_bounds__(kLmgBlock) dot_kernel(int64_t n, const double *x, const double *y,
                                                        double *partial)
{
    __shared__ double s_red[kLmgBlock / LMG_WAVE];
    double v = 0.0;
    const int64_t stride = (int64_t)gridDim.x * kLmgBlock;
    for (int64_t i = (int64_t)blockIdx.x * kLmgBlock + threadIdx.x; i < n; i += stride) v += x[i] * y[i];
    const double tot = lmg_block_sum<kLmgBlock>(v, s_red);
    if (threadIdx.x == 0) partial[blockIdx.x] = tot;
}

__global__ void __launch_bounds__(1024) dot_final_kernel(const double *partial, int count, double *out)
{
    __shared__ double s_red[1024 / LMG_WAVE];
    double v = (int)threadIdx.x < count ? partial[threadIdx.x] : 0.0;
    const double tot = lmg_block_sum<1024>(v, s_red);
    if (threadIdx.x == 0) out[0] = tot;
}

__global__ void __launch_bounds__(kLmgBlock) gather_kernel(int64_t n, const int *idx, const double *x,
                                                           double *buf)
{
    const int64_t stride = (int64_t)gridDim.x * kLmgBlock;
    for (int64_t i = (int64_t)blockIdx.x * kLmgBlock + threadIdx.x; i < n; i += stride) buf[i] = x[idx[i]];
}

__global__ void __launch_bounds__(kLmgBlock) scatter_kernel(int64_t n, const int *idx, const double *buf,
                                                            double *x)
{
    const int64_t stride = (int64_t)gridDim.x * kLmgBlock;
    for (int64_t i = (int64_t)blockIdx.x * kLmgBlock + threadIdx.x; i < n; i += stride) x[idx[i]] = buf[i];
}

__global__ void __launch_bounds__(kLmgBlock) pattern_parity_counts_kernel(int64_t n, int W, const unsigned char *pid, int *counts)
{
    __shared__ int s_cnt[4 * 256];
    for (int i = threadIdx.x; i < 4 * 256; i += kLmgBlock) s_cnt[i] = 0;
    __syncthreads();
    for (int64_t i = (int64_t)blockIdx.x * kLmgBlock + threadIdx.x; i < n; i += (int64_t)gridDim.x * kLmgBlock) {
        const unsigned y = (unsigned)(i / W), x = (unsigned)(i - (int64_t)y * W);
        atomicAdd(&s_cnt[(((y & 1u) << 1) | (x & 1u)) * 256 + pid[i]], 1);
    }
    __syncthreads();
    for (int i = threadIdx.x; i < 4 * 256; i += kLmgBlock)
        if (s_cnt[i]) atomicAdd(&counts[i], s_cnt[i]);
}

constexpr int kScanBlock = 1024;
constexpr int kScanItems = 4;
constexpr int kScanTile = kScanBlock * kScanItems;

__device__ __forceinline__ int wave_incl_scan(int v, int lane)
{
#pragma unroll
    for (int off = 1; off < LMG_WAVE; off <<= 1) {
        const int u = __shfl_up(v, off, LMG_WAVE);
        if (lane >= off) v += u;
    }
    return v;
}

__global__ void __launch_bounds__(kScanBlock) scan_tile_kernel(int64_t n, const int *in, int *out,
                                                               int *block_sums)
{
    __shared__ int s_wave[kScanBlock / LMG_WAVE];
    const int t = threadIdx.x, lane = t & 63, wave = t >> 6;
    const int64_t base = (int64_t)blockIdx.x * kScanTile + (int64_t)t * kScanItems;
    int v[kScanItems];
    int sum = 0;
#pragma unroll
    for (int k = 0; k < kScanItems; ++k) {
        v[k] = (base + k < n) ? in[base + k] : 0;
        sum += v[k];
    }
    const int incl = wave_incl_scan(sum, lane);
    if (lane == 63) s_wave[wave] = incl;
    __syncthreads();
    if (wave == 0) {
        const int w = (lane < kScanBlock / LMG_WAVE) ? s_wave[lane] : 0;
        const int wi = wave_incl_scan(w, lane);
        if (lane < kScanBlock / LMG_WAVE) s_wave[lane] = wi - w;
        if (lane == kScanBlock / LMG_WAVE - 1 && block_sums) block_sums[blockIdx.x] = wi;
    }
    __syncthreads();
    int run = s_wave[wave] + incl - sum;
#pragma unroll
    for (int k = 0; k < kScanItems; ++k) {
        run += v[k];
        if (base + k < n) out[base + k + 1] = run;
    }
    if (blockIdx.x == 0 && t == 0) out[0] = 0;
}

__global__ void __launch_bounds__(kScanBlock) scan_add_kernel(int64_t n, int *out, const int *block_offs)
{
    const int off = block_offs[blockIdx.x];
    if (off == 0) return;
    const int64_t base = (int64_t)blockIdx.x * kScanTile;
    for (int i = threadIdx.x; i < kScanTile; i += kScanBlock)
        if (base + i < n) out[base + i + 1] += off;
}

int scan_rec(int64_t n, const int *in, int *out, int *scratch, hipStream_t st)
{
    const int64_t blocks = (n + kScanTile - 1) / kScanTile;
    if (blocks <= 1) {
        hipLaunchKernelGGL(scan_tile_kernel, dim3(1), dim3(kScanBlock), 0, st, n, in, out, (int *)nullptr);
        LMG_CHECK_LAUNCH();
        return LMG_OK;
    }
    int *sums = scratch;
    int *offs = scratch + blocks;
    int *rest = offs + blocks + 1;
    hipLaunchKernelGGL(scan_tile_kernel, dim3((unsigned)blocks), dim3(kScanBlock), 0, st, n, in, out, sums);
    LMG_CHECK_LAUNCH();
    int rc = scan_rec(blocks, sums, offs, rest, st);
    if (rc != LMG_OK) return rc;
    hipLaunchKernelGGL(scan_add_kernel, dim3((unsigned)blocks), dim3(kScanBlock), 0, st, n, out, offs);
    LMG_CHECK_LAUNCH();
    return LMG_OK;
}

}

extern "C" {

int lmg_version(void) { return LMG_VERSION; }

const char *lmg_status_string(int s)
{
    switch (s) {
    case LMG_OK: return "ok";
    case LMG_ERR_ARG: return "invalid argument";
    case LMG_ERR_ALIGN: return "array base not 16-byte aligned";
    case LMG_ERR_LAUNCH: return "HIP launch/runtime error";
    case LMG_ERR_CAPACITY: return "row exceeds kernel capacity";
    case LMG_ERR_NODEVICE: return "no HIP device";
    default: return "unknown status";
    }
}

int lmg_device_count(void)
{
    int c = 0;
    if (hipGetDeviceCount(&c) != hipSuccess) return LMG_ERR_NODEVICE;
    return c;
}

static const LmgTuneKey *const kTuneTables[] = {lmg_tune_sweep, lmg_tune_pcsr,  lmg_tune_rpat, lmg_tune_stencil, lmg_tune_fused,
                                                lmg_tune_tile,  lmg_tune_dia,   lmg_tune_sell, lmg_tune_gsw,     lmg_tune_gs};

static const LmgTuneKey *tune_find(const char *key)
{
    if (!key) return nullptr;
    for (const LmgTuneKey *table : kTuneTables)
        if (const LmgTuneKey *k = lmg_tune_find(table, key)) return k;
    return nullptr;
}

int lmg_tune_set(const char *key, int value)
{
    if (key && strcmp(key, "rpat_variant") == 0 && value >= 1000) key = "rpat_nt_rows";
    const LmgTuneKey *k = tune_find(key);
    if (!k || !lmg_tune_accepts(*k, value)) return LMG_ERR_ARG;
    *k->value = value;
    return LMG_OK;
}

int lmg_tune_get(const char *key)
{
    const LmgTuneKey *k = tune_find(key);
    return k ? *k->value : LMG_ERR_ARG;
}

int lmg_axpby(int64_t n, double alpha, const double *x, double beta, double *y, void *stream)
{
    if (n < 0 || (n > 0 && (!x || !y))) return LMG_ERR_ARG;
    if (n == 0) return LMG_OK;
    if (!lmg_aligned16(x) || !lmg_aligned16(y)) return LMG_ERR_ALIGN;
    hipLaunchKernelGGL(axpby_kernel, dim3(lmg_grid_for(n, kLmgBlock * 2)), dim3(kLmgBlock), 0, lmg_stream(stream),
                       n, alpha, x, beta, y);
    LMG_CHECK_LAUNCH();
    return LMG_OK;
}

int lmg_vmul(int64_t n, double alpha, const double *x, const double *y, double *out, void *stream)
{
    if (n < 0 || (n > 0 && (!x || !y || !out))) return LMG_ERR_ARG;
    if (n == 0) return LMG_OK;
    hipLaunchKernelGGL(vmul_kernel, dim3(lmg_grid_for(n, kLmgBlock)), dim3(kLmgBlock), 0, lmg_stream(stream), n, alpha, x, y, out);
    LMG_CHECK_LAUNCH();
    return LMG_OK;
}

int lmg_cheby_update(int64_t n, double a, double c, int first, const double *dinv, const double *r, double *d, double *x,
                     void *stream)
{
    if (n < 0 || (n > 0 && (!dinv || !r || !d || !x))) return LMG_ERR_ARG;
    if (n == 0) return LMG_OK;
    if (d == x || d == r || d == dinv || x == r || x == dinv) return LMG_ERR_ARG;
    if (!lmg_aligned16(dinv) || !lmg_aligned16(r) || !lmg_aligned16(d) || !lmg_aligned16(x)) return LMG_ERR_ALIGN;
    const unsigned grid = lmg_grid_for(n, kLmgBlock * 2);
    if (first)
        hipLaunchKernelGGL(cheby_update_kernel<true>, dim3(grid), dim3(kLmgBlock), 0, lmg_stream(stream), n, a, c, dinv, r, d, x);
    else
        hipLaunchKernelGGL(cheby_update_kernel<false>, dim3(grid), dim3(kLmgBlock), 0, lmg_stream(stream), n, a, c, dinv, r, d, x);
    LMG_CHECK_LAUNCH();
    return LMG_OK;
}

int lmg_csr_gershgorin(int64_t n, const int32_t *rowptr, const int32_t *colidx, const double *vals, double *lmax, void *stream)
{
    if (n < 0 || n >= INT32_MAX || !lmax || (n > 0 && (!rowptr || !colidx || !vals))) return LMG_ERR_ARG;
    if (hipMemsetAsync(lmax, 0, sizeof(double), lmg_stream(stream)) != hipSuccess) return LMG_ERR_LAUNCH;
    if (n == 0) return LMG_OK;
    hipLaunchKernelGGL(csr_gershgorin_kernel, dim3(lmg_grid_for(n, kLmgBlock)), dim3(kLmgBlock), 0, lmg_stream(stream), n, rowptr, colidx,
                       vals, reinterpret_cast<unsigned long long *>(lmax));
    LMG_CHECK_LAUNCH();
    return LMG_OK;
}

int lmg_copy(int64_t n, const double *src, double *dst, void *stream)
{
    if (n < 0 || (n > 0 && (!src || !dst))) return LMG_ERR_ARG;
    if (n == 0) return LMG_OK;
    if (hipMemcpyAsync(dst, src, (size_t)n * sizeof(double), hipMemcpyDeviceToDevice,
                       lmg_stream(stream)) != hipSuccess)
        return LMG_ERR_LAUNCH;
    return LMG_OK;
}

int lmg_zero(int64_t n, double *x, void *stream)
{
    if (n < 0 || (n > 0 && !x)) return LMG_ERR_ARG;
    if (n == 0) return LMG_OK;
    if (hipMemsetAsync(x, 0, (size_t)n * sizeof(double), lmg_stream(stream)) != hipSuccess)
        return LMG_ERR_LAUNCH;
    return LMG_OK;
}

int lmg_dot(int64_t n, const double *x, const double *y, double *partials, double *out, void *stream)
{
    if (n < 0 || !partials || !out || (n > 0 && (!x || !y))) return LMG_ERR_ARG;
    const unsigned grid = 1024;
    hipLaunchKernelGGL(dot_kernel, dim3(grid), dim3(kLmgBlock), 0, lmg_stream(stream), n, x, y, partials);
    LMG_CHECK_LAUNCH();
    hipLaunchKernelGGL(dot_final_kernel, dim3(1), dim3(1024), 0, lmg_stream(stream), partials, (int)grid, out);
    LMG_CHECK_LAUNCH();
    return LMG_OK;
}

int lmg_gather(int64_t n, const int32_t *idx, const double *x, double *buf, void *stream)
{
    if (n < 0 || (n > 0 && (!idx || !x || !buf))) return LMG_ERR_ARG;
    if (n == 0) return LMG_OK;
    hipLaunchKernelGGL(gather_kernel, dim3(lmg_grid_for(n, kLmgBlock)), dim3(kLmgBlock), 0, lmg_stream(stream), n, idx, x, buf);
    LMG_CHECK_LAUNCH();
    return LMG_OK;
}

int lmg_scatter(int64_t n, const int32_t *idx, const double *buf, double *x, void *stream)
{
    if (n < 0 || (n > 0 && (!idx || !x || !buf))) return LMG_ERR_ARG;
    if (n == 0) return LMG_OK;
    hipLaunchKernelGGL(scatter_kernel, dim3(lmg_grid_for(n, kLmgBlock)), dim3(kLmgBlock), 0, lmg_stream(stream), n, idx, buf, x);
    LMG_CHECK_LAUNCH();
    return LMG_OK;
}

int lmg_pattern_parity_counts(int64_t n, int32_t line_stride, const uint8_t *pid, int32_t *counts, void *stream)
{
    if (n < 0 || line_stride < 1 || (n > 0 && (!pid || !counts))) return LMG_ERR_ARG;
    if (n == 0) return LMG_OK;
    hipLaunchKernelGGL(pattern_parity_counts_kernel, dim3(lmg_grid_for(n, kLmgBlock * 16)), dim3(kLmgBlock), 0, lmg_stream(stream), n,
                       line_stride, pid, counts);
    LMG_CHECK_LAUNCH();
    return LMG_OK;
}

int64_t lmg_scan_scratch_count(int64_t n)
{
    int64_t total = 0;
    int64_t blocks = (n + kScanTile - 1) / kScanTile;
    while (blocks > 1) {
        total += 2 * blocks + 1;
        blocks = (blocks + kScanTile - 1) / kScanTile;
    }
    return total + 16;
}

int lmg_exclusive_scan_i32(int64_t n, const int32_t *in, int32_t *out, int32_t *scratch, void *stream)
{
    if (n < 0 || !out || (n > 0 && !in)) return LMG_ERR_ARG;
    if (n > kScanTile && !scratch) return LMG_ERR_ARG;
    return scan_rec(n, in, out, scratch, lmg_stream(stream));
}

int lmg_graph_begin(void *stream)
{
    if (hipStreamBeginCapture(lmg_stream(stream), hipStreamCaptureModeThreadLocal) != hipSuccess)
        return LMG_ERR_LAUNCH;
    return LMG_OK;
}

int lmg_graph_end(void *stream, void **exec_out)
{
    if (!exec_out) return LMG_ERR_ARG;
    hipGraph_t g = nullptr;
    if (hipStreamEndCapture(lmg_stream(stream), &g) != hipSuccess || !g) return LMG_ERR_LAUNCH;
    hipGraphExec_t ex = nullptr;
    hipError_t e = hipGraphInstantiate(&ex, g, nullptr, nullptr, 0);
    (void)hipGraphDestroy(g);
    if (e != hipSuccess) return LMG_ERR_LAUNCH;
    *exec_out = ex;
    return LMG_OK;
}

int lmg_graph_launch(void *exec, void *stream)
{
    if (!exec) return LMG_ERR_ARG;
    if (hipGraphLaunch(reinterpret_cast<hipGraphExec_t>(exec), lmg_stream(stream)) != hipSuccess)
        return LMG_ERR_LAUNCH;
    return LMG_OK;
}

int lmg_graph_destroy(void *exec)
{
    if (!exec) return LMG_OK;
    (void)hipGraphExecDestroy(reinterpret_cast<hipGraphExec_t>(exec));
    return LMG_OK;
}

}
```

learnmultigrid_amd/hierarchy.py:

```python
import math

import numpy as np
import scipy.sparse as sp
import torch

from . import ops, smoothing
from .coarse import make_coarse_solver
from .ops import DeviceCSR, F64
from .smoothing import (CHEBY_RATIO, GS_SWEEPS, LINE_DIRS, LINE_ORDERS, _directions, chebyshev_coefficients,
                        chebyshev_degree, gs_sweep_pair, line_band_value, line_config, line_half_steps)
from .twins import DiaTwin, check_values, line_reach, line_stride


CYCLE_SHAPES = ("V", "W", "F")
_CHILDREN = {"V": ("V",), "W": ("W", "W"), "F": ("F", "V")}


def cycle_children(shape):
    if shape not in _CHILDREN:
        raise ValueError("cycle shape must be one of %s, got %r" % (CYCLE_SHAPES, shape))
    return _CHILDREN[shape]


def capture_cycle(ops_mod, levels, run, swap_from=None):
# ... 447 lines not shown
        if smoother == "Chebyshev":
            name = CHEBY_TWIN[name]
        return smoothing.ask(self.ops, name, *args)

    def _wavefront_gs(self, l, gs_mode, direction="forward"):
        return gs_mode == "lexicographic" and smoothing.wavefront_gs(self.ops, self.levels[l].A, direction)

    def _fusable(self, l, smoother, steps):
        if smoother not in ("Jacobi", "Chebyshev") or steps < 1:
            return False
        if not self._ask("stencil_smooth_available", self.levels[l].A, smoother=smoother):
            return False
        return smoother == "Jacobi" or steps <= self.ops.FUSED_MAX_SWEEPS

    def smooth_fused(self, l, steps, omega, x_is_zero=False, want_residual=False, correction=None, restrict_to=None,
                     smoother="Jacobi"):
        coef = self._cheby_coef(l, steps) if smoother == "Chebyshev" and steps > 0 else None
        smoothing.fused_passes(self.ops, self.levels[l].A, self.levels[l], steps, omega, x_is_zero, want_residual,
                               correction, restrict_to, coef)

    def coarse_solve(self):
        lev = self.levels[-1]
        self.coarse.apply(lev.b, lev.x)
        for _ in range(self.coarse_refine):
            self.ops.csr_residual_norm2(lev.A, lev.x, lev.b, lev.r, None, None)
            if getattr(self.coarse, "supports_accumulate", False):
                self.coarse.apply(lev.r, lev.x, accumulate=True)
            else:
                self.coarse.apply(lev.r, lev.tmp)
                self.ops.axpby(1.0, lev.tmp, 1.0, lev.x)

    def cycle(self, smoother, steps, omega=1.0, gs_mode="lexicographic", l=0, depth=None,
              after_presmooth=None, x_is_zero=False, gs_sweep=("forward", "forward"), shape="V", *,
              cheby_lmax=None, cheby_ratio=None, line_dir=None, line_order=None, line_band=None):
        children = cycle_children(shape)
        if smoother == "Chebyshev":
            chebyshev_degree(steps)
        pair = gs_sweep_pair(gs_sweep)
        self._prepare(smoother, cheby_lmax, cheby_ratio, line_dir, line_order, line_band)
        if smoother == "Line":
            pair = ("forward", "backward")
        self._visit(smoother, steps, omega, gs_mode, l, (len(self.levels) if depth is None else depth) - 1, children,
                    pair, x_is_zero, after_presmooth)

    def _visit(self, smoother, steps, omega, gs_mode, l, last, children, pair, x_is_zero=False, after_presmooth=None,
               entered=False, leave_open=False):
        if not entered:
            self._presmooth(smoother, steps, omega, gs_mode, l, x_is_zero, pair[0], after_presmooth)
        if l + 1 == last:
            self.coarse_solve()
        else:
            open_ = False
            for i, sub in enumerate(children):
                more = i + 1 < len(children)
                if open_:
                    self._turnaround(l + 1, steps, omega)
                open_ = self._visit(smoother, steps, omega, gs_mode, l + 1, last, cycle_children(sub), pair,
                                    x_is_zero=(i == 0), entered=open_, leave_open=more)
        if leave_open and self._turnaround_ok(l, smoother, steps):
            return True
        self._postsmooth(smoother, steps, omega, gs_mode, l, pair[1])
        return False

    def _presmooth(self, smoother, steps, omega, gs_mode, l, x_is_zero, pre, after_presmooth):
        lev, nxt = self.levels[l], self.levels[l + 1]
        fused = self._fusable(l, smoother, steps)
        restricted = fused and self._ask("stencil_smooth_restrict_available", lev.A, lev.R, smoother=smoother)
        if restricted:
            self.smooth_fused(l, steps, omega, x_is_zero, restrict_to=(lev.R, nxt.b), smoother=smoother)
        elif fused:
            self.smooth_fused(l, steps, omega, x_is_zero, want_residual=True, smoother=smoother)
        else:
            self.smooth(l, smoother, steps, omega, gs_mode, x_is_zero, pre)
        if after_presmooth is not None:
            after_presmooth(lev.x)
        if not fused:
            self.ops.csr_residual_norm2(lev.A, lev.x, lev.b, lev.r, None, None)
        if not restricted:
            self.ops.csr_spmv(lev.R, lev.r, nxt.b, 1.0, 0.0)

    def _postsmooth(self, smoother, steps, omega, gs_mode, l, post):
        lev, nxt = self.levels[l], self.levels[l + 1]
        fused = self._fusable(l, smoother, steps)
        if fused and self._ask("stencil_smooth_prolong_available", lev.A, lev.P, smoother=smoother):
            self.smooth_fused(l, steps, omega, correction=(lev.P, nxt.x), smoother=smoother)
            return
        self.ops.csr_spmv(lev.P, nxt.x, lev.x, 1.0, 1.0)
        if fused:
            self.smooth_fused(l, steps, omega, smoother=smoother)
        else:
            self.smooth(l, smoother, steps, omega, gs_mode, direction=post)

    def _turnaround_ok(self, l, smoother, steps):
        lev = self.levels[l]
        return bool(smoother == "Jacobi" and self._fusable(l, smoother, steps)
                    and self._ask("stencil_smooth_turnaround_selected", lev.A, lev.P, lev.R) and steps <= self.ops.FUSED_MAX_SWEEPS)

    def _turnaround(self, l, steps, omega):
        lev, nxt = self.levels[l], self.levels[l + 1]
        self.ops.stencil_smooth_turnaround(lev.A, lev.x, lev.b, omega, steps, steps, lev.tmp,
                                           prolong=(lev.P, nxt.x), restrict=(lev.R, nxt.b))
        lev.x, lev.tmp = lev.tmp, lev.x

    def residual_norm(self, want_vector=True):
        if self.cycle_values != "f64":
            raise ValueError("a hierarchy with cycle_values=%r is a preconditioner, not the operator of the outer iteration: "
                             "its sweeps read rounded values, so this would be the residual of A32 x = b.  Use it through "
                             "CG.solve / GMRES.solve(preconditioner=H), which take the residual with their own fp64 "
                             "operator" % (self.cycle_values,))
        lev = self.levels[0]
        self.ops.csr_residual_norm2(lev.A, lev.x, lev.b, self.outer_r if want_vector else None,
                               self.partials, self.norm2)
        return math.sqrt(self.norm2.item())

    def check_smoothers(self):
        for lev in self.levels[:-1]:
            self._ask("stencil_gs_check", lev.A)

    def prepare_smoother(self, smoother, gs_mode="lexicographic", l_from=0, gs_sweep=("forward", "forward"), *,
                         cheby_lmax=None, cheby_ratio=None, line_dir=None, line_order=None, line_band=None):
        self._prepare(smoother, cheby_lmax, cheby_ratio, line_dir, line_order, line_band)
        if smoother != "GaussSeidel":
            return
        dirs = []
        for sw in gs_sweep_pair(gs_sweep):
            dirs += [d for d in _directions(sw) if d not in dirs]
        for l in range(l_from, len(self.levels) - 1):
            for d in dirs:
                if self._wavefront_gs(l, gs_mode, d):
                    self.ops.stencil_gs(self.levels[l].A, self.levels[l].tmp, self.levels[l].b, 0)
                else:
                    self.gs_schedule(l, gs_mode, d)

    def captured_cycle(self, smoother, steps, omega, gs_mode, gs_sweep=("forward", "forward"), shape="V", *,
                       cheby_lmax=None, cheby_ratio=None, line_dir=None, line_order=None, line_band=None):
        pair = gs_sweep_pair(gs_sweep)
        cycle_children(shape)
        self._prepare(smoother, cheby_lmax, cheby_ratio, line_dir, line_order, line_band)
        key = (smoother, steps, omega, gs_mode, pair, shape) + self._smoother_key(smoother)
        g = self._graphs.get(key)
        if g is None:
            self.prepare_smoother(smoother, gs_mode, gs_sweep=pair)
            g = self._graphs[key] = capture_cycle(self.ops, self.levels, swap_from=1, run=lambda: self.cycle(
                smoother, steps, omega, gs_mode, gs_sweep=pair, shape=shape))
        return g

    def twin_bytes(self):
        tot = 0
        for lev in self.levels:
            for M in (lev.A, lev.P, lev.R):
                for name in ("patterns", "sell", "packed", "dia"):
                    T = getattr(M, name, None) if M is not None else None
                    tot += 0 if T is None else T.bytes()
        return tot

    @staticmethod
    def _csr_model_bytes(M):
        S = getattr(M, "sell", None)
        narrow = S is not None and getattr(S, "values", "f64") == "f32"
        return (8 if narrow else 12) * M.nnz + 4 * (M.shape[0] + 1)

    def memory_bytes(self):
        tot = 0
        for lev in self.levels:
            tot += lev.A.bytes() + (4 + (lev.d is not None)) * 8 * lev.n
            tot += 0 if lev.line is None else sum(8 * (2 * lev.line_band[d] + 1) * lev.n for d in lev.line if d != "W")
            for M in (lev.P, lev.R, lev.RA):
                if M is not None:
                    tot += M.bytes()
        return tot + self.coarse.bytes_per_apply()

    def cycle_bytes(self, steps):
        tot = 0
        for lev in self.levels[:-1]:
            n, nnz = lev.n, lev.A.nnz
            nc = lev.P.shape[1]
            D = getattr(lev.A, "dia", None)
            a_bytes = self._csr_model_bytes(lev.A) - (4 * nnz if D is not None and getattr(D, "values", "f64") == "f32" else 0)
            tot += (2 * steps + 1) * (a_bytes + 24 * n)
            tot += self._csr_model_bytes(lev.R) + 8 * n + 8 * nc
            tot += self._csr_model_bytes(lev.P) + 8 * nc + 16 * n
        coarse = (1 + self.coarse_refine) * self.coarse.bytes_per_apply()
        return tot, coarse
```

learnmultigrid_amd/ops.py:

```python
import ctypes

import numpy as np
import torch

from . import _lib
from ._lib import LmgError, check
from .twins import (F32, F64, I32, ColorSell, DiaTwin, PackedCSR, ProlongTwin, RestrictTwin, RowPatterns, SellCSR,
                    StencilTwin, _p, _s, check_values)


def _vec_ok(*ts):
    for t in ts:
        if t is None:
            continue
        if t.dtype != F64 or not t.is_contiguous() or not t.is_cuda:
            raise TypeError("expected contiguous float64 device tensors, got %s %s contiguous=%s"
                            % (t.dtype, t.device, t.is_contiguous()))


class DeviceCSR:

    __slots__ = ("rowptr", "colidx", "vals", "shape", "nnz", "packed", "patterns", "sell", "stencil", "prolong", "restrict",
                 "dia", "values", "twin_values")

    def __init__(self, rowptr, colidx, vals, shape):
        if rowptr.dtype != I32 or colidx.dtype != I32 or vals.dtype != F64:
            raise TypeError("DeviceCSR wants int32 indices and float64 values")
        if rowptr.numel() != shape[0] + 1 or colidx.numel() != vals.numel():
            raise ValueError("inconsistent CSR arrays")
        self.rowptr, self.colidx, self.vals = rowptr.contiguous(), colidx.contiguous(), vals.contiguous()
        self.shape = (int(shape[0]), int(shape[1]))
        self.nnz = int(vals.numel())
        self.packed = None
        self.patterns = None
        self.sell = None
        self.stencil = None
        self.prolong = None
        self.restrict = None
        self.dia = None
        self.values = "f64"
        self.twin_values = "f64"

    def pack(self, patterns=None, line_strides=None, values=None):
        if values is not None:
            check_values(values)
        if not self.vals.is_cuda:
            return None
        src = self
        if values is not None and values != self.values:
            self.values = values
            src = self._retarget()
        elif self.twin_values == "f32":
            src = self.cycle_source()
        vkw = {} if self.twin_values == "f64" else {"values": "f32"}
        if patterns is None:
            patterns = _PATTERNS_ENABLED
        if patterns and self.patterns is None and self.packed is None and self.sell is None:
            if self.shape[0] == self.shape[1]:
                self.patterns = RowPatterns.from_csr(src)
            else:
                for gm in (RowPatterns.grid_map_candidates(self.shape, line_strides) if _GRID_MAPS_ENABLED else []):
                    self.patterns = RowPatterns.from_csr(src, gm)
                    if self.patterns is not None:
                        break
            self._derive_grid_twins()
        if patterns and self.patterns is not None:
            return self.patterns
        if self.sell is not None:
            return self.sell
        if self.packed is None:
            if self.dia is None and _DIA_ENABLED and self.shape[0] == self.shape[1]:
                self.dia = DiaTwin.from_csr(self, **vkw)
            self.packed = PackedCSR.from_csr(src)
            pk = self.packed
            long_raw = pk is not None and pk.valmode == 2 and pk.tile_rows < 512
            unpackable = pk is None and self.nnz > 0
            if _SELL_ENABLED and (long_raw or unpackable) and self.nnz >= SELL_MIN_AVG * self.shape[0]:
                self.sell = SellCSR.from_csr(self, **vkw)
                if self.sell is not None:
                    self.packed = None
                    return self.sell
        return self.packed

    def _derive_grid_twins(self):
        self.stencil, self.prolong, self.restrict = (
            T.from_patterns(self.patterns, self.shape) if _STENCIL_ENABLED else None
            for T in (StencilTwin, ProlongTwin, RestrictTwin))
        S = self.stencil
        if S is not None and S.n >= min(FUSED_TRANSFER_MIN_ROWS, REG_PROLONG_MIN_ROWS, REG_RESTRICT_MIN_ROWS):
            S.line_end_coupling

    def invalidate_packed(self):
        self.packed = self.patterns = self.sell = self.stencil = self.prolong = self.restrict = self.dia = None

    def _rounded(self):
        v = self.vals
        r = v.to(F32).to(F64)
        m = r.abs()
        bad = (v != 0) & ~((m >= float(np.finfo(np.float32).tiny)) & (m <= float(np.finfo(np.float32).max)))
        return None if bool(bad.any()) else r

    def _retarget(self):
        r = self._rounded() if self.values == "f32" else None
        want = "f64" if r is None else "f32"
        if want != self.twin_values:
            self.invalidate_packed()
            self.twin_values = want
        return self if r is None else DeviceCSR(self.rowptr, self.colidx, r, self.shape)

    def cycle_source(self):
        if self.twin_values == "f64":
            return self
        r = self._rounded()
        if r is None:
            raise LmgError("the values no longer fit fp32: call repack_values() after changing the values of a matrix")
        return DeviceCSR(self.rowptr, self.colidx, r, self.shape)

    def plain(self):
        return DeviceCSR(self.rowptr, self.colidx, self.vals, self.shape)

    def repack_values(self):
        had = any(t is not None for t in (self.patterns, self.sell, self.dia, self.packed))
        src = self._retarget() if self.values == "f32" else self
        if had and not any(t is not None for t in (self.patterns, self.sell, self.dia, self.packed)):
            self.pack()
            return
        if self.patterns is not None:
            self.patterns = RowPatterns.from_csr(src, self.patterns.grid_map)
            self._derive_grid_twins()
            if self.patterns is None:
                self.pack()
        if self.sell is not None and not self.sell.update_values(self):
            self.sell = SellCSR.from_csr(self, colmode=self.sell.colmode, max_padding=float("inf"))
        if self.dia is not None and not self.dia.update_values(self):
            self.dia = None
        if self.packed is not None and not self.packed.update_values(src):
            self.packed = None
            self.pack(patterns=False)

    @classmethod
    def from_scipy(cls, A, device, canonical=True):
        import scipy.sparse as sp
        if not (sp.isspmatrix_csr(A) and A.dtype == np.float64):
            A = sp.csr_matrix(A, dtype=np.float64)
        if canonical and not A.has_canonical_format:
            A = A.copy()
            A.sum_duplicates()
        if A.nnz >= 2 ** 31 - 8192 or max(A.shape) >= 2 ** 31 - 1:
            raise ValueError("matrix too large for int32 indices")
        return cls(torch.from_numpy(np.ascontiguousarray(A.indptr, dtype=np.int32)).to(device),
                   torch.from_numpy(np.ascontiguousarray(A.indices, dtype=np.int32)).to(device),
                   torch.from_numpy(np.ascontiguousarray(A.data, dtype=np.float64)).to(device), A.shape)

    def transpose(self):
        n, m = self.shape
        dev = self.vals.device
        if self.vals.is_cuda and self.nnz and self.nnz < 2 ** 31 - 1:
            L = _lib.lib()
            counts = torch.zeros(m, dtype=I32, device=dev)
            check(L.lmg_csr_transpose_count(self.nnz, m, _p(self.colidx), _p(counts), _s(self.colidx)), "lmg_csr_transpose_count")
            if int(counts.max()) <= int(L.lmg_csr_transpose_max_row()):
                rp = torch.empty(m + 1, dtype=I32, device=dev)
                exclusive_scan_i32(counts, rp)
                counts.zero_()
                tc = torch.empty(self.nnz, dtype=I32, device=dev)
                tv = torch.empty(self.nnz, dtype=F64, device=dev)
                check(L.lmg_csr_transpose_fill(n, m, _p(self.rowptr), _p(self.colidx), _p(self.vals), _p(rp), _p(counts),
                                               _p(tc), _p(tv), _s(self.rowptr)), "lmg_csr_transpose_fill")
                return DeviceCSR(rp, tc, tv, (m, n))
        rows = torch.repeat_interleave(torch.arange(n, device=dev, dtype=I32),
                                       (self.rowptr[1:] - self.rowptr[:-1]).long())
        order = torch.sort(self.colidx, stable=True).indices
        rp = torch.zeros(m + 1, dtype=I32, device=dev)
        if self.nnz:
            rp[1:] = torch.cumsum(torch.bincount(self.colidx, minlength=m), 0).to(I32)
        return DeviceCSR(rp, rows[order].contiguous(), self.vals[order].contiguous(), (m, n))

    def to_scipy(self):
        import scipy.sparse as sp
        return sp.csr_matrix((self.vals.cpu().numpy(), self.colidx.cpu().numpy(),
                              self.rowptr.cpu().numpy()), shape=self.shape)

    @property
    def device(self):
        return self.vals.device

    def bytes(self):
        return 12 * self.nnz + 4 * (self.shape[0] + 1)


_PACKED_ENABLED = True
_PATTERNS_ENABLED = True
_STENCIL_ENABLED = True
_GRID_MAPS_ENABLED = True
_DIA_ENABLED = True


def set_dia_enabled(flag):
    global _DIA_ENABLED
    _DIA_ENABLED = bool(flag)


def set_grid_maps_enabled(flag):
    global _GRID_MAPS_ENABLED
    _GRID_MAPS_ENABLED = bool(flag)


def set_stencil_enabled(flag):
    global _STENCIL_ENABLED
    _STENCIL_ENABLED = bool(flag)


FUSED_MAX_SWEEPS = 3
FUSED_MIN_ROWS = 12_000_000
REG_MAX_ROWS = (1 << 29) - 4096
GS_WAVE_MAX_ROWS = (1 << 29) - 8192
TILED_MIN_ROWS = 4096
_TILED_ENABLED = True


def set_tiled_enabled(flag):
    global _TILED_ENABLED
    _TILED_ENABLED = bool(flag)


def _pass_kind(A, cheby):
    S = getattr(A, "stencil", None)
    D = getattr(A, "dia", None)
    if S is None and D is not None and _PACKED_ENABLED and _DIA_ENABLED and _FUSED_ENABLED:
        return "dia"
    if not (_PACKED_ENABLED and _STENCIL_ENABLED and _FUSED_ENABLED and S is not None):
        return None
    if S.n >= FUSED_MIN_ROWS and not cheby:
        return "reg" if (S.n < REG_MAX_ROWS and _lib.lib().lmg_stencil_smooth_supported(S.umask)) else None
    if (_TILED_ENABLED and S.n >= TILED_MIN_ROWS and not (cheby and S.n > CHEBY_TILED_MAX_ROWS) and S.W >= 3
            and _lib.lib().lmg_stencil_smooth_tiled_supported(S.umask)):
        return "tile"
    return None


def _fused_kind(A):
    return _pass_kind(A, False)


def stencil_smooth_available(A):
    return _fused_kind(A) is not None


_FUSED_ENABLED = True


def set_fused_enabled(flag):
    global _FUSED_ENABLED
    _FUSED_ENABLED = bool(flag)


def stencil_smooth(A, x_in, b, omega, sweeps, x_out, r_out=None, prolong=None, restrict=None):
    _vec_ok(x_in, b, x_out, r_out)
    if A.stencil is not None:
        kind = "tile" if _fused_kind(A) == "tile" else "reg"
    elif getattr(A, "dia", None) is not None:
        kind = "dia"
    else:
        raise LmgError("stencil_smooth needs a grid-stencil matrix")
    _run_pass("smooth", kind, A, (int(sweeps), _p(x_in), _p(b), float(omega), _p(x_out)), x_in, r_out, prolong, restrict)


def _run_pass(stem, kind, A, head, x_in, r_out, prolong, restrict):
    who = "stencil_" + stem
    if kind == "dia":
        D = A.dia
        if prolong is not None or restrict is not None:
            raise LmgError("%s: transfers cannot be fused into the pass of a variable-coefficient operator" % who)
        name = "lmg_dia_" + stem + ("_f32" if D.values == "f32" else "")
        check(getattr(_lib.lib(), name)(D.n, D.W, D.umask, _p(D.dia), *head, _p(r_out), _s(D.dia)), name)
        return
    S = A.stencil
    tiled = kind == "tile"
    form = "restrict" if restrict is not None else "prolong" if prolong is not None else None
    if form is None:
        tail = (_p(r_out),)
    else:
        M, vec = restrict if form == "restrict" else prolong
        T = getattr(M, form)
        _vec_ok(vec)
        other = prolong is not None if form == "restrict" else x_in is None
        if T is None or r_out is not None or other or T.n != S.n or T.W != S.W or vec.numel() != T.nc:
            what = "restriction" if form == "restrict" else "prolongation"
            raise LmgError("%s: this %s cannot be fused into the pass" % (who, what))
        reg_min = REG_RESTRICT_MIN_ROWS if form == "restrict" else REG_PROLONG_MIN_ROWS
        if (stem == "smooth" and S.n >= reg_min and _lib.lib().lmg_stencil_smooth_prolong_supported(S.umask)
                and not S.line_end_coupling):
            tiled = False
        if not tiled and S.line_end_coupling:
            raise LmgError("%s: the register pass folds no transfer into an operator with entries across a line end" % who)
        tail = T.c_args(vec)
    name = "lmg_stencil_%s%s%s" % (stem, "_tiled" if tiled else "", "_" + form if form else "")
    check(getattr(_lib.lib(), name)(*S.c_args(), *head, *tail, _s(S.pid)), name)


FUSED_TRANSFER_MIN_ROWS = 12_000_000
REG_PROLONG_MIN_ROWS = 1 << 62
REG_RESTRICT_MIN_ROWS = 1 << 62
_FUSED_PROLONG_ENABLED = True


def set_fused_prolong_enabled(flag):
    global _FUSED_PROLONG_ENABLED
    _FUSED_PROLONG_ENABLED = bool(flag)


def _twin_on_grid(A, M, form):
    T = getattr(M, form, None)
    S = getattr(A, "stencil", None)
    return T if (T is not None and S is not None and T.n == S.n and T.W == S.W) else None


def _prolong_available(A, P, kind):
    if not (_FUSED_PROLONG_ENABLED and kind in ("reg", "tile") and _twin_on_grid(A, P, "prolong") is not None):
        return False
    if kind == "tile":
        return True
    S = A.stencil
    return bool(S.n >= FUSED_TRANSFER_MIN_ROWS and _lib.lib().lmg_stencil_smooth_prolong_supported(S.umask)
                and not S.line_end_coupling)


def stencil_smooth_prolong_available(A, P):
    return _prolong_available(A, P, _fused_kind(A))


_FUSED_RESTRICT_ENABLED = True
TILED_RESTRICT_MAX_ROWS = 1 << 62


def set_fused_restrict_enabled(flag):
    global _FUSED_RESTRICT_ENABLED
    _FUSED_RESTRICT_ENABLED = bool(flag)


def _restrict_available(A, R, kind):
    T = _twin_on_grid(A, R, "restrict")
    if not (_FUSED_RESTRICT_ENABLED and kind in ("reg", "tile") and T is not None):
        return False
    S = A.stencil
    if kind == "reg" and not (S.n >= FUSED_TRANSFER_MIN_ROWS and _lib.lib().lmg_stencil_smooth_prolong_supported(S.umask)
                              and not S.line_end_coupling):
        return False
    if kind == "tile" and S.n > TILED_RESTRICT_MAX_ROWS:
        return False
    lines = (S.n + S.W - 1) // S.W
    return T.nc >= ((lines + 1) // 2 - 1) * T.Wc + (S.W + 1) // 2


def stencil_smooth_restrict_available(A, R):
    return _restrict_available(A, R, _fused_kind(A))


_FUSED_TURNAROUND_ENABLED = True
TURNAROUND_MIN_ROWS = 100_000
TURNAROUND_MAX_ROWS = 2_000_000


def set_fused_turnaround_enabled(flag):
    global _FUSED_TURNAROUND_ENABLED
    _FUSED_TURNAROUND_ENABLED = bool(flag)


def stencil_smooth_turnaround_available(A, P, R):
    if not (_FUSED_TURNAROUND_ENABLED and _fused_kind(A) == "tile"):
        return False
    if not (stencil_smooth_prolong_available(A, P) and stencil_smooth_restrict_available(A, R)):
        return False
    S, TP, TR = A.stencil, P.prolong, R.restrict
    lines = (S.n + S.W - 1) // S.W
    return bool(TP.nc == TR.nc and TP.Wc == TR.Wc and TR.nc >= 2 and S.n % S.W == 0
                and TR.Wc == (S.W + 1) // 2 and TR.nc == ((lines + 1) // 2) * TR.Wc)


def stencil_smooth_turnaround_selected(A, P, R):
    return bool(stencil_smooth_turnaround_available(A, P, R) and TURNAROUND_MIN_ROWS <= A.shape[0] <= TURNAROUND_MAX_ROWS)


def stencil_smooth_turnaround(A, x_in, b, omega, sweeps_post, sweeps_pre, x_out, prolong, restrict):
    (P, e), (R, bc) = prolong, restrict
    _vec_ok(x_in, b, x_out, e, bc)
    S, TP, TR = A.stencil, getattr(P, "prolong", None), getattr(R, "restrict", None)
    if (S is None or TP is None or TR is None or x_in is None or _fused_kind(A) != "tile" or TP.n != S.n or TP.W != S.W
            or TR.n != S.n or TR.W != S.W or e.numel() != TP.nc or bc.numel() != TR.nc):
        raise LmgError("stencil_smooth_turnaround: this level and its transfers cannot run the turnaround pass")
    check(_lib.lib().lmg_stencil_smooth_tiled_turnaround(
        *S.c_args(), int(sweeps_post), int(sweeps_pre), _p(x_in), _p(b), float(omega), _p(x_out), *TP.c_args(e),
        *TR.c_args(bc)[2:], _s(S.pid)), "lmg_stencil_smooth_tiled_turnaround")


CHEBY_TILED_MAX_ROWS = (1 << 31) - 4096 - 1


def _cheby_kind(A):
    return _pass_kind(A, True)


def stencil_cheby_available(A):
    return _cheby_kind(A) is not None


def stencil_cheby_prolong_available(A, P):
    return _prolong_available(A, P, _cheby_kind(A))


def stencil_cheby_restrict_available(A, R):
    return _restrict_available(A, R, _cheby_kind(A))


def _cheby_coef(coef):
    flat = [float(v) for pair in coef for v in pair]
    if not 1 <= len(coef) <= FUSED_MAX_SWEEPS or len(flat) != 2 * len(coef):
        raise LmgError("stencil_cheby takes 1..%d (a_k, c_k) pairs, got %r" % (FUSED_MAX_SWEEPS, coef))
    return (ctypes.c_double * len(flat))(*flat)


def stencil_cheby(A, x_in, b, coef, x_out, r_out=None, prolong=None, restrict=None):
    _vec_ok(x_in, b, x_out, r_out)
    kind = _cheby_kind(A)
    hc = _cheby_coef(coef)
    if kind is None:
        raise LmgError("stencil_cheby needs a level that runs the tiled passes (stencil_cheby_available)")
    _run_pass("cheby", kind, A, (len(coef), ctypes.addressof(hc), _p(x_in), _p(b), _p(x_out)), x_in, r_out, prolong, restrict)


def cheby_update(a, c, dinv, r, d, x, first=False):
    _vec_ok(dinv, r, d, x)
    check(_lib.lib().lmg_cheby_update(x.numel(), float(a), float(c), int(bool(first)), _p(dinv), _p(r), _p(d), _p(x), _s(x)),
          "lmg_cheby_update")


def csr_gershgorin(A, out):
    _vec_ok(out)
    check(_lib.lib().lmg_csr_gershgorin(A.shape[0], _p(A.rowptr), _p(A.colidx), _p(A.vals), _p(out), _s(A.rowptr)),
          "lmg_csr_gershgorin")


LINE_DIRS = {"x": 0, "y": 1}
LINE_COUPLED, LINE_PIVOT = 1, 2


def line_factor_flags(A, W, dir):
    if dir not in LINE_DIRS:
        raise ValueError("line direction must be 'x' or 'y', got %r" % (dir,))
    n = A.shape[0]
    if A.shape[0] != A.shape[1] or int(W) < 1 or n % int(W) != 0:
# ... 1181 lines not shown
```

learnmultigrid_amd/twins.py:

```python
import ctypes
import math

import numpy as np
import torch

from . import _lib
from ._lib import LmgError, check

F64 = torch.float64
F32 = torch.float32
I32 = torch.int32
VALUES = ("f64", "f32")


def check_values(values, what="values"):
    if values not in VALUES:
        raise ValueError("%s must be one of %s, got %r" % (what, VALUES, values))
    return values


def _s(*ts):
    for t in ts:
        if t is not None and getattr(t, "is_cuda", False):
            if t.device.index != torch.cuda.current_device():
                raise LmgError("operands live on %s but the current device is cuda:%d: wrap the call in "
                               "torch.cuda.device(...)" % (t.device, torch.cuda.current_device()))
            return torch.cuda.current_stream(t.device).cuda_stream
    return torch.cuda.current_stream().cuda_stream


def _p(t):
    return None if t is None else t.data_ptr()


def _decompose(off, W, radius=1):
    for c in range(-radius, radius + 1):
        d = off - c * W
        if -radius <= d <= radius:
            return c, d
    return None


def slot_3x3(W):
    def slot(off):
        cd = _decompose(off, W)
        return None if cd is None else (cd[0] + 1) * 3 + (cd[1] + 1)
    return slot


def slot_2x2(Wc):
    return {0: 0, 1: 1, Wc: 2, Wc + 1: 3}.get


def decode_window(ptr, off, val, nslots, slot_of):
    npat = len(ptr) - 1
    values = np.zeros(npat * nslots)
    mask = np.zeros(npat, dtype=np.int32)
    for p in range(npat):
        o = off[ptr[p]:ptr[p + 1]]
        if o.size > nslots or np.any(np.diff(o) <= 0):
            return None
        for j in range(ptr[p], ptr[p + 1]):
            k = slot_of(int(off[j]))
            if k is None or mask[p] & (1 << k):
                return None
            mask[p] |= 1 << k
            values[p * nslots + k] = val[j]
    return values, mask


def line_stride(off, n, radius=1):
    mx = int(np.abs(off).max()) if off.size else 0
    if mx <= 1:
        cands = [n] if n >= 3 else []
    else:
        cands = []
        for cy in range(1, radius + 1):
            for dx in [0] + [s * k for k in range(1, radius + 1) for s in (1, -1)]:
                w, rem = divmod(mx - dx, cy)
                if rem == 0 and 2 * radius + 1 <= w < n and w not in cands:
                    cands.append(w)
    fits = [w for w in cands if all(_decompose(int(o), w, radius) is not None for o in off)]
    return next((w for w in fits if n % w == 0), fits[0]) if fits else None


def line_reach(off, W, radius):
    cd = [_decompose(int(o), W, radius) for o in off]
    return max([1] + [abs(d) for _, d in cd]), max([1] + [abs(c) for c, _ in cd])


def hot_pattern(cand, counts):
    if len(cand) <= 1:
        return int(cand[0]) if cand else -1
    return int(max(cand, key=lambda p: counts[p]))


def prolong_hot_pairs(p_val, p_mask, counts):
    if np.any((counts[0].sum(axis=0) > 0) & ((p_mask & 0xC) != 0)):
        return None
    pairs, pval = [], []
    for yl, want in enumerate(((0x1, 0x3), (0x5, 0xF))):
        ids = [hot_pattern([p for p in range(len(p_mask)) if p_mask[p] == want[xl] and counts[yl][xl][p] > 0], counts[yl][xl])
               for xl in range(2)]
        pairs.append(-1 if min(ids) < 0 else ids[0] | (ids[1] << 8))
        for xl in range(2):
            pval += [float(p_val[ids[xl] * 4 + k]) if ids[xl] >= 0 else 0.0 for k in range(4) if (want[xl] >> k) & 1]
    return pairs, pval


def _table(R):
    return (R.pat_ptr.cpu().numpy(), R.pat_off.cpu().numpy().astype(np.int64)[: R.nent], R.pat_val.cpu().numpy()[: R.nent])


def _hot_values(values, hot):
    return None if hot < 0 else (ctypes.c_double * 9)(*[float(v) for v in values[hot * 9: hot * 9 + 9]])


class PackedCSR:

    __slots__ = ("n", "nnz", "shape", "tile_rows", "tile_cap", "tile_base", "tile_colbase", "rowlen", "col",
                 "colmode", "val", "valmode", "dict", "ndict", "bytes_")

    @staticmethod
    def _padded(t):
        raw = t.contiguous().view(torch.uint8)
        out = torch.zeros(((raw.numel() + 15) // 16) * 16 + 16, dtype=torch.uint8, device=t.device)
        out[: raw.numel()] = raw
        return out

    _VSET_SLOTS = 1 << 20
    _VSET_LIMIT = 65536

    @staticmethod
    def _padded_empty(nbytes, device):
        return torch.zeros(((nbytes + 15) // 16) * 16 + 16, dtype=torch.uint8, device=device)

    @classmethod
    def _distinct_values(cls, vals, limit=None):
        L = _lib.lib()
        dev = vals.device
        limit = cls._VSET_LIMIT if limit is None else int(limit)
        table = torch.full((cls._VSET_SLOTS,), -1, dtype=torch.int64, device=dev)
        state = torch.zeros(4, dtype=I32, device=dev)
        check(L.lmg_value_set_insert(vals.numel(), _p(vals), _p(table), cls._VSET_SLOTS, limit,
                                     _p(state), _s(vals)), "lmg_value_set_insert")
        st = state.cpu()
        if int(st[1]):
            return None
        cap = limit + 8
        out = torch.empty(cap, dtype=torch.int64, device=dev)
        cnt = torch.zeros(1, dtype=I32, device=dev)
        check(L.lmg_value_set_collect(_p(table), cls._VSET_SLOTS, _p(out), cap, _p(cnt), _s(vals)), "lmg_value_set_collect")
        k = int(cnt.cpu()[0])
        if k > cap:
            return None
        keys = out[:k].cpu().numpy()
        if int(st[2]):
            keys = np.concatenate([keys, np.array([-1], dtype=np.int64)])
        if keys.size > limit:
            return None
        return torch.from_numpy(np.sort(keys)).to(dev)

    @staticmethod
    def _encode_values(vals, uniq, width, out):
        missing = torch.zeros(1, dtype=I32, device=vals.device)
        check(_lib.lib().lmg_value_encode(vals.numel(), _p(vals), _p(uniq), int(uniq.numel()), width, _p(out),
                                          _p(missing), _s(vals)), "lmg_value_encode")
        if int(missing):
            raise LmgError("value dictionary does not cover the matrix values")

    @classmethod
    def from_csr(cls, A, tile_rows=None, colmode=None):
        n, nnz = A.shape[0], A.nnz
        if n == 0 or nnz == 0:
            return None
        if tile_rows is not None and int(tile_rows) not in (512, 128, 64):
            raise ValueError("tile_rows must be 512, 128 or 64, got %r" % (tile_rows,))
        if colmode is not None and int(colmode) not in (0, 1):
            raise ValueError("colmode must be 0 or 1, got %r" % (colmode,))
        L = _lib.lib()
        dev = A.vals.device
        rowlen = (A.rowptr[1:] - A.rowptr[:-1])
        if int(rowlen.max()) > 255 or int(rowlen.min()) < 0:
            return None
        uniq = cls._distinct_values(A.vals)
        ndict = int(uniq.numel()) if uniq is not None else 1 << 30
        avg = nnz / n
        T = int(L.lmg_pcsr_tile_rows())
        bpe = 2 + (1 if ndict <= 256 else (2 if ndict <= 65536 else 8))
        if tile_rows is not None:
            T = int(tile_rows)
        elif T * avg * bpe > 20480:
            T = 128 if 128 * avg * (2 + (1 if ndict <= 256 else 8)) <= 20480 else 64
            if 256 < ndict <= 65536:
                ndict = 1 << 30
        ntile = (n + T - 1) // T
        tb = A.rowptr[0:n:T]
        tile_base = torch.cat([tb, A.rowptr[n:n + 1]]).contiguous()
        tile_nnz = tile_base[1:] - tile_base[:-1]
        self = cls()
        self.n, self.nnz, self.shape = n, nnz, A.shape
        self.tile_rows = T
        self.tile_cap = int(tile_nnz.max())
        self.tile_base = tile_base
        self.rowlen = rowlen.to(torch.uint8).contiguous()
        cmin = torch.empty(ntile, dtype=I32, device=dev)
        cmax = torch.empty(ntile, dtype=I32, device=dev)
        check(L.lmg_pcsr_tile_colrange(n, T, _p(A.rowptr), _p(A.colidx), _p(cmin), _p(cmax), _s(A.rowptr)),
              "lmg_pcsr_tile_colrange")
        self.tile_colbase = cmin
        fits16 = int((cmax - cmin).max()) < 65536
        if colmode == 0 and not fits16:
            raise ValueError("colmode 0: a tile spans 65536 columns or more")
        if (fits16 if colmode is None else int(colmode) == 0):
            self.colmode = 0
            self.col = cls._padded_empty(2 * nnz, dev)
            check(L.lmg_pcsr_encode_cols16(n, T, _p(A.rowptr), _p(A.colidx), _p(cmin), _p(self.col), _s(A.rowptr)),
                  "lmg_pcsr_encode_cols16")
        else:
            self.colmode = 1
            self.col = cls._padded(A.colidx)
        self.ndict = ndict
        if self.ndict <= 256:
            self.valmode = 0
            self.val = cls._padded_empty(nnz, dev)
            cls._encode_values(A.vals, uniq, 1, self.val)
            self.dict = uniq.view(F64)
        elif self.ndict <= 65536:
            self.valmode = 1
            self.val = cls._padded_empty(2 * nnz, dev)
            cls._encode_values(A.vals, uniq, 2, self.val)
            self.dict = uniq.view(F64)
        else:
            self.valmode = 2
            self.val = cls._padded(A.vals)
            self.dict = None
            self.ndict = 0
        self.bytes_ = (self.rowlen.numel() + 8 * ntile + nnz * ((2, 4)[self.colmode] + (1, 2, 8)[self.valmode]))
        return self

    def bytes(self):
        return int(self.bytes_)

    def sweep_args(self):
        return (self.n, self.nnz, self.tile_rows, self.tile_cap, _p(self.tile_base), _p(self.tile_colbase), _p(self.rowlen),
                _p(self.col), self.colmode, _p(self.val), self.valmode, _p(self.dict), self.ndict), self.tile_base

    def update_values(self, A):
        if A.nnz != self.nnz:
            return False
        if self.valmode == 2:
            self.val[: self.nnz * 8].view(F64).copy_(A.vals)
            return True
        uniq = self._distinct_values(A.vals)
        nd = int(uniq.numel()) if uniq is not None else 1 << 30
        if (self.valmode == 0 and nd > 256) or (self.valmode == 1 and nd > 65536):
            return False
        self._encode_values(A.vals, uniq, 1 if self.valmode == 0 else 2, self.val)
        self.dict = uniq.view(F64)
        self.ndict = nd
        return True


class SellCSR:

    __slots__ = ("n", "nnz", "shape", "slice_base", "slice_len", "slice_cmin", "rowlen", "col", "colmode", "val",
                 "max_len", "padded", "bytes_", "values")

# ... 77 lines not shown
        self.h_color_slice = np.zeros(nc + 1, dtype=np.int32)
        np.cumsum((np.diff(h_ptr) + 63) // 64, out=self.h_color_slice[1:])
        self.nslices = nsl = int(self.h_color_slice[-1])
        self.trow = torch.empty(max(64 * nsl, 1), dtype=I32, device=dev)
        self.tlen = torch.empty(max(64 * nsl, 1), dtype=I32, device=dev)
        self.slice_len = torch.empty(max(nsl, 1), dtype=I32, device=dev)
        if nsl == 0:
            self.slice_base = torch.zeros(1, dtype=torch.int64, device=dev)
            self.max_len = self.padded = 0
            self.col, self.src = (torch.zeros(64, dtype=I32, device=dev) for _ in range(2))
            self.val = torch.zeros(64, dtype=F64, device=dev)
            return self
        d_ptr = torch.from_numpy(h_ptr).to(dev)
        d_cs = torch.from_numpy(self.h_color_slice).to(dev)
        check(L.lmg_color_twin_count(nsl, nc, _p(d_ptr), _p(d_cs), _p(d_rows), _p(A.rowptr), _p(self.trow), _p(self.tlen),
                                     _p(self.slice_len), _s(A.rowptr)), "lmg_color_twin_count")
        sl = self.slice_len.long() * 64
        ends = torch.cumsum(sl, 0)
        self.slice_base = (ends - sl).contiguous()
        self.padded, self.max_len = (int(v) for v in torch.stack((ends[-1], self.slice_len.max().long())).cpu())
        self.col = torch.zeros(self.padded + 64, dtype=I32, device=dev)
        self.val = torch.zeros(self.padded + 64, dtype=F64, device=dev)
        self.src = torch.full((self.padded + 64,), -1, dtype=I32, device=dev)
        entries = A.colidx if A.nnz else torch.zeros(1, dtype=I32, device=dev)
        values = A.vals if A.nnz else torch.zeros(1, dtype=F64, device=dev)
        check(L.lmg_color_twin_fill(nsl, _p(self.trow), _p(A.rowptr), _p(entries), _p(values), _p(self.slice_base),
                                    _p(self.col), _p(self.val), _p(self.src), _s(A.rowptr)), "lmg_color_twin_fill")
        return self

    def update_values(self, A):
        if self.padded and A.nnz:
            check(_lib.lib().lmg_color_twin_refill(self.padded, _p(self.src), _p(A.vals), _p(self.val), _s(A.vals)),
                  "lmg_color_twin_refill")

    def bytes(self):
        return 16 * self.padded + 12 * self.nslices + 8 * 64 * self.nslices

    def sweep(self, x, b, sweeps, backward):
        check(_lib.lib().lmg_color_sweep(self.ncolors, self.h_color_slice.ctypes.data, _p(self.slice_base), _p(self.slice_len),
                                         _p(self.trow), _p(self.tlen), _p(self.col), _p(self.val), self.max_len, self.padded,
                                         _p(x), _p(b), int(sweeps), int(bool(backward)), _s(x)), "lmg_color_sweep")


def _pid_counts(R):
    cnt = torch.zeros(4 * 256, dtype=I32, device=R.pid.device)
    check(_lib.lib().lmg_pattern_parity_counts(int(R.n), 1, _p(R.pid), _p(cnt), _s(R.pid)), "lmg_pattern_parity_counts")
    return cnt.cpu().numpy().reshape(4, 256).sum(axis=0)[:R.npat].astype(np.int64)


class RowPatterns:

    __slots__ = ("n", "nnz", "shape", "pid", "npat", "nent", "max_len", "pat_ptr", "pat_off", "pat_val", "bytes_",
                 "grid_map", "_gm")

    @staticmethod
    def grid_map_candidates(shape, line_strides=None):
        nr, nc = int(shape[0]), int(shape[1])
        if nr == nc or nr < 2 or nc < 2:
            return []
        out = []
        if line_strides is not None:
            wf, wcs = int(line_strides[0]), int(line_strides[1])
            if wf >= 2 and wcs >= 2:
                out.append((wf, wcs, 1, 1, 0) if nr > nc else (wcs, 2 * wf, 0, 0, 1))
        wr, wc = math.isqrt(nr), math.isqrt(nc)
        if wr * wr == nr and wc * wc == nc and min(wr, wc) >= 2:
            out.append((wr, wc, 1, 1, 0) if nr > nc else (wr, 2 * wc, 0, 0, 1))
        out.append((nr + 1, 0, 0, 1, 0) if nr > nc else (nr + 1, 0, 0, 0, 1))
        return out

    @staticmethod
    def grid_base(grid_map, rows):
        if grid_map is None:
            return rows
        rl, cs, ysh, xsh, xshl = grid_map
        y, x = rows // rl, rows % rl
        return (y >> ysh) * cs + ((x >> xsh) << xshl)

    @classmethod
    def from_csr(cls, A, grid_map=None):
        n, nnz = A.shape[0], A.nnz
        if n == 0 or nnz == 0 or not A.vals.is_cuda:
            return None
        L = _lib.lib()
        dev = A.vals.device
        gm = None if grid_map is None else (ctypes.c_int32 * 5)(*[int(v) for v in grid_map])
        gmp = None if gm is None else ctypes.addressof(gm)
        mp, me = ctypes.c_int32(0), ctypes.c_int32(0)
        check(L.lmg_rpat_limits(ctypes.addressof(mp), ctypes.addressof(me)), "lmg_rpat_limits")
        max_pat, max_ent = int(mp.value), int(me.value)
        hashes = torch.empty(n, dtype=torch.int64, device=dev)
        check(L.lmg_rpat_row_hash_grid(n, gmp, _p(A.rowptr), _p(A.colidx), _p(A.vals), _p(hashes), _s(A.rowptr)),
              "lmg_rpat_row_hash_grid")
        uniq = PackedCSR._distinct_values(hashes.view(F64), limit=max_pat)
        if uniq is None:
            return None
        npat = int(uniq.numel())
        pid = torch.zeros(n + 32, dtype=torch.uint8, device=dev)[:n]
        PackedCSR._encode_values(hashes.view(F64), uniq, 1, pid)
        del hashes
        rep = torch.full((256,), -1, dtype=I32, device=dev)
        check(L.lmg_rpat_claim(n, _p(pid), _p(rep), _s(pid)), "lmg_rpat_claim")
        rep_h = rep[:npat].cpu().numpy().astype(np.int64)
        if npat == 0 or rep_h.min() < 0:
            return None
        rep = torch.from_numpy(rep_h).to(dev)
        starts, ends = A.rowptr[rep].cpu().numpy().astype(np.int64), A.rowptr[torch.from_numpy(rep_h + 1).to(dev)].cpu().numpy().astype(np.int64)
        lens = ends - starts
        nent = int(lens.sum())
        if nent > max_ent:
            return None
        idx = np.concatenate([np.arange(s_, e_) for s_, e_ in zip(starts, ends)]) if nent else np.zeros(0, np.int64)
        d_idx = torch.from_numpy(idx).to(dev)
        self = cls()
        self.n, self.nnz, self.shape = n, nnz, A.shape
        self.pid = pid
        self.npat, self.nent = npat, nent
        self.max_len = int(lens.max())
        ptr = np.zeros(npat + 1, dtype=np.int32)
        np.cumsum(lens, out=ptr[1:])
        self.pat_ptr = torch.from_numpy(ptr).to(dev)
        base_of = cls.grid_base(grid_map, np.repeat(rep_h, lens).astype(np.int64))
        if nent:
            off_h = A.colidx[d_idx].cpu().numpy().astype(np.int64) - base_of
            if np.abs(off_h).max() >= 2 ** 31:
                return None
            self.pat_off = torch.from_numpy(off_h.astype(np.int32)).to(dev)
        else:
            self.pat_off = torch.zeros(1, dtype=I32, device=dev)
        self.pat_val = A.vals[d_idx].contiguous() if nent else torch.zeros(1, dtype=F64, device=dev)
        mismatch = torch.zeros(1, dtype=I32, device=dev)
        check(L.lmg_rpat_verify_grid(n, A.shape[1], gmp, _p(A.rowptr), _p(A.colidx), _p(A.vals), _p(pid), npat,
                                     _p(self.pat_ptr), _p(self.pat_off), _p(self.pat_val), _p(mismatch), _s(A.rowptr)),
              "lmg_rpat_verify_grid")
        if int(mismatch):
            return None
        self.bytes_ = n + 4 * (npat + 1) + 12 * nent
        self.grid_map = None if grid_map is None else tuple(int(v) for v in grid_map)
        self._gm = gm
        return self

    def bytes(self):
        return int(self.bytes_)

    def sweep_args(self):
        gmp = None if self._gm is None else ctypes.addressof(self._gm)
        return (self.n, gmp, _p(self.pid), self.npat, self.nent, self.max_len, _p(self.pat_ptr), _p(self.pat_off),
                _p(self.pat_val)), self.pid


class StencilTwin:

    __slots__ = ("n", "W", "npat", "pid", "st_val", "st_mask", "umask", "bytes_", "patterns", "hot", "_hot_val",
                 "_gs_ok", "_gs_work", "_line_end")
    _decompose = staticmethod(_decompose)

    @classmethod
    def from_patterns(cls, R, shape):
        if R is None or shape[0] != shape[1] or R.n < 2:
            return None
        mp = ctypes.c_int32(0)
        check(_lib.lib().lmg_stencil_limits(ctypes.addressof(mp)), "lmg_stencil_limits")
        if R.npat > int(mp.value):
            return None
        ptr, off, val = _table(R)
        W = line_stride(off, int(R.n))
        dec = None if W is None else decode_window(ptr, off, val, 9, slot_3x3(W))
        if dec is None:
            return None
        st_val, st_mask = dec
        dev = R.pid.device
        self = cls()
        self.n, self.W, self.npat, self.pid, self.patterns = int(R.n), int(W), int(R.npat), R.pid, R
        self.st_val = torch.from_numpy(st_val).to(dev)
        self.st_mask = torch.from_numpy(st_mask).to(dev)
        self.umask = int(np.bitwise_or.reduce(st_mask)) if R.npat else 0
        self.bytes_ = R.n + 76 * R.npat
        cand = [p for p in range(R.npat) if st_mask[p] == self.umask and (st_mask[p] & 16) and st_val[p * 9 + 4] != 0.0]
        self.hot = hot_pattern(cand, _pid_counts(R) if len(cand) > 1 else None)
        self._hot_val = _hot_values(st_val, self.hot)
        self._gs_work = None
        self._gs_ok = None
        self._line_end = None
        return self

    def sweep_args(self):
        return (self.n, self.W, _p(self.pid), self.npat, _p(self.st_val), _p(self.st_mask), self.umask), self.pid

    def c_args(self):
        hv = None if self._hot_val is None else ctypes.addressof(self._hot_val)
        return (self.n, self.W, _p(self.pid), self.npat, _p(self.st_val), _p(self.st_mask), self.umask, self.hot, hv)

    @property
    def gs_ok(self):
        if self._gs_ok is None:
            ok = bool(_lib.lib().lmg_stencil_gs_supported(self.umask)) and self.n >= 2 and bool(self.umask & 0x1C7)
            self._gs_ok = ok and not self.line_end_coupling
        return self._gs_ok

    @property
    def line_end_coupling(self):
        if self._line_end is None:
            mk = self.st_mask.cpu().numpy()
            W = self.W
            first = mk[self.pid[0::W].cpu().numpy()]
            last = mk[self.pid[W - 1::W].cpu().numpy()]
            self._line_end = bool(((first & 0x49) != 0).any()) or bool(((last & 0x124) != 0).any())
        return self._line_end

    def bytes(self):
        return int(self.bytes_)


class ProlongTwin:

    __slots__ = ("n", "W", "nc", "Wc", "npat", "pid", "p_val", "p_mask", "_hot_pairs", "_hot_pval", "patterns")

    @classmethod
    def from_patterns(cls, R, shape):
        if R is None or R.grid_map is None or R.npat > 64 or R.n < 2:
            return None
        W, Wc, ysh, xsh, xshl = R.grid_map
        if (ysh, xsh, xshl) != (1, 1, 0) or Wc < 2 or W < 3 or 2 * Wc < W + 1 or shape[1] >= 2 ** 31:
            return None
        dec = decode_window(*_table(R), 4, slot_2x2(Wc))
        if dec is None:
            return None
        p_val, p_mask = dec
        dev = R.pid.device
        n = int(R.n)
        cnt = torch.zeros(4 * 256, dtype=I32, device=dev)
        check(_lib.lib().lmg_pattern_parity_counts(n, int(W), _p(R.pid), _p(cnt), _s(R.pid)), "lmg_pattern_parity_counts")
        counts = cnt.cpu().numpy().reshape(2, 2, 256)[:, :, :R.npat].astype(np.int64)
        hot = prolong_hot_pairs(p_val, p_mask, counts)
        if hot is None:
            return None
        self = cls()
        self.n, self.W, self.nc, self.Wc, self.npat = n, int(W), int(shape[1]), int(Wc), int(R.npat)
        self.pid, self.patterns = R.pid, R
        self.p_val = torch.from_numpy(p_val).to(dev)
        self.p_mask = torch.from_numpy(p_mask).to(dev)
        self._hot_pairs = (ctypes.c_int32 * 2)(*hot[0])
        self._hot_pval = (ctypes.c_double * 9)(*hot[1])
        return self

    def c_args(self, e):
        return (self.nc, self.Wc, _p(e), _p(self.pid), self.npat, _p(self.p_val), _p(self.p_mask),
                ctypes.addressof(self._hot_pairs), ctypes.addressof(self._hot_pval))


class RestrictTwin:

    __slots__ = ("nc", "Wc", "n", "W", "npat", "pid", "r_val", "r_mask", "hot", "_hot_val", "patterns")

    @classmethod
    def from_patterns(cls, R, shape):
        if R is None or R.grid_map is None or R.npat > 64:
            return None
        Wc, cs, ysh, xsh, xshl = R.grid_map
        if (ysh, xsh, xshl) != (0, 0, 1) or cs % 2 or Wc < 2 or shape[0] >= 2 ** 28:
            return None
        W = cs // 2
        if W < 3 or Wc != (W + 1) // 2 or shape[1] % W or int(R.n) != ((shape[1] // W + 1) // 2) * Wc:
            return None
        dec = decode_window(*_table(R), 9, slot_3x3(W))
        if dec is None:
            return None
        r_val, r_mask = dec
        dev = R.pid.device
        self = cls()
        self.nc, self.Wc, self.n, self.W, self.npat = int(R.n), int(Wc), int(shape[1]), int(W), int(R.npat)
        self.pid, self.patterns = R.pid, R
        self.r_val = torch.from_numpy(r_val).to(dev)
        self.r_mask = torch.from_numpy(r_mask).to(dev)
        cand = [p for p in range(R.npat) if r_mask[p] == 0x1FF]
        self.hot = hot_pattern(cand, _pid_counts(R) if len(cand) > 1 else None)
        self._hot_val = _hot_values(r_val, self.hot)
        return self

    def c_args(self, bc):
        hr = None if self._hot_val is None else ctypes.addressof(self._hot_val)
        return (self.nc, self.Wc, _p(bc), _p(self.pid), self.npat, _p(self.r_val), _p(self.r_mask), self.hot, hr)


class DiaTwin:

    __slots__ = ("n", "W", "umask", "nslots", "dia", "bytes_", "values")
    MIN_ROWS = 4096

    @staticmethod
    def _probe(A, W, umask, dia):
        dev = A.vals.device
        flags = torch.zeros(2, dtype=I32, device=dev)
        name = "lmg_dia_fill_f32" if dia is not None and dia.dtype == F32 else "lmg_dia_fill"
        check(getattr(_lib.lib(), name)(A.shape[0], int(W), _p(A.rowptr), _p(A.colidx), _p(A.vals), int(umask), _p(dia),
                                        flags.data_ptr(), flags.data_ptr() + 4, _s(A.rowptr)), name)
        f = flags.cpu().numpy()
        return int(f[0]), int(f[1]) & 0x1FF

    @classmethod
    def from_csr(cls, A, values="f64"):
        check_values(values)
        n = A.shape[0]
        if n < cls.MIN_ROWS or A.nnz == 0 or A.nnz > 9 * n or not A.vals.is_cuda or n >= 2 ** 31 - 4096:
            return None
        mid = n // 2
        rp = A.rowptr[mid:mid + 9].cpu().numpy().astype(np.int64)
        ci = A.colidx[rp[0]:rp[-1]].cpu().numpy().astype(np.int64)
        rows = np.repeat(np.arange(mid, mid + 8), np.diff(rp))
        off = np.abs(ci - rows)
        mx = int(off.max()) if off.size else 0
        if mx < 4:
            return None
        for W in sorted((mx, mx - 1, mx + 1), key=lambda w: (n % w != 0 if w > 0 else True)):
            if not (3 <= W < n):
                continue
            bad, seen = cls._probe(A, W, 0x1FF, None)
            if bad or not (seen & 16):
                continue
            umask = next((m for m in (0x0BA, 0x1BB, 0x0FE, 0x1FF) if not (seen & ~m)), None)
            if umask is None or not _lib.lib().lmg_dia_smooth_supported(umask):
                return None
            self = cls()
            self.n, self.W, self.umask = int(n), int(W), int(umask)
            self.nslots = bin(umask).count("1")
            self.values = values
            self.dia = torch.empty(self.nslots * n, dtype=F64 if values == "f64" else F32, device=A.vals.device)
            bad, _seen = cls._probe(A, W, umask, self.dia)
            if bad:
                return None
            self.bytes_ = self.dia.element_size() * self.nslots * n
            return self
        return None

    def update_values(self, A):
        bad, _seen = self._probe(A, self.W, self.umask, self.dia)
        return not bad

    def bytes(self):
        return int(self.bytes_)
```

Before: 274.8 billion DoF*sweeps/s.

## Skip pattern-id loads in fused stencil strips proven uniform by census table

Builds a 2-D prefix-sum census of cells whose pattern id differs from the hot pattern, for the stencil, prolongation and restriction maps. At setup the census is computed once; at run time each fused smoothing strip checks it in O(1) and, when the whole window is uniform, runs a specialized body that skips the pid/ppid/rpid loads and the per-wave hot-pattern votes. This removes pattern-id memory traffic and branch checks on the interior of the Poisson grid, at the cost of an extra template instantiation (code size and register pressure) and a small census table.

```diff
diff --git a/include/lmg.h b/include/lmg.h
--- a/include/lmg.h
+++ b/include/lmg.h
@@ -165,6 +165,34 @@
                                 int32_t r_npat, const double *d_r_val, const int32_t *d_r_mask, int32_t hot_r,
                                 const double *h_hot_rval, void *stream);
 
+int64_t lmg_pattern_census_count(int64_t n, int32_t line_stride);
+int lmg_pattern_census(int64_t n, int32_t line_stride, const uint8_t *d_pid, const int32_t *h_expected, int32_t *d_table,
+                       void *stream);
+int lmg_stencil_smooth_census(int64_t n, int32_t line_stride, const uint8_t *d_pid, int32_t npat,
+                              const double *d_st_val, const int32_t *d_st_mask, uint32_t union_mask,
+                              int32_t hot_pattern, const double *h_hot_val, int sweeps, const double *d_x_in,
+                              const double *d_b, double omega, double *d_x_out, double *d_r_out,
+                              const int32_t *d_census, int32_t census_stride, void *stream);
+int lmg_stencil_smooth_prolong_census(int64_t n, int32_t line_stride, const uint8_t *d_pid, int32_t npat,
+                                      const double *d_st_val, const int32_t *d_st_mask, uint32_t union_mask,
+                                      int32_t hot_pattern, const double *h_hot_val, int sweeps, const double *d_x_in,
+                                      const double *d_b, double omega, double *d_x_out, int64_t n_coarse,
+                                      int32_t coarse_stride, const double *d_e_coarse, const uint8_t *d_p_pid,
+                                      int32_t p_npat, const double *d_p_val, const int32_t *d_p_mask,
+                                      const int32_t *h_hot_pairs, const double *h_hot_pval, const int32_t *d_census,
+                                      const int32_t *d_p_census, int32_t census_stride, void *stream);
+int lmg_stencil_smooth_restrict_census(int64_t n, int32_t line_stride, const uint8_t *d_pid, int32_t npat,
+                                       const double *d_st_val, const int32_t *d_st_mask, uint32_t union_mask,
+                                       int32_t hot_pattern, const double *h_hot_val, int sweeps, const double *d_x_in,
+                                       const double *d_b, double omega, double *d_x_out, int64_t n_coarse,
+                                       int32_t coarse_stride, double *d_b_coarse, const uint8_t *d_r_pid,
+                                       int32_t r_npat, const double *d_r_val, const int32_t *d_r_mask, int32_t hot_r,
+                                       const double *h_hot_rval, const int32_t *d_census, int32_t census_stride,
+                                       const int32_t *d_r_census, int32_t r_census_stride, void *stream);
+int lmg_stencil_smooth_uniform_items(int64_t n, int32_t line_stride, int sweeps, int with_residual, int zero_iterate,
+                                     int form, int64_t n_coarse, int32_t coarse_stride, const int32_t *h_census,
+                                     const int32_t *h_p_census, const int32_t *h_r_census, int64_t *h_counts);
+
 int lmg_sell_sweep(int mode, int64_t n, const int64_t *d_slice_base, const int32_t *d_slice_len,
                    const int32_t *d_slice_cmin, const int32_t *d_rowlen, const void *d_col, int colmode,
                    const double *d_val, int32_t max_len, const double *d_x, const double *d_b, double *d_out,
diff --git a/learnmultigrid_amd/_lib.py b/learnmultigrid_amd/_lib.py
--- a/learnmultigrid_amd/_lib.py
+++ b/learnmultigrid_amd/_lib.py
@@ -62,6 +62,15 @@
                                               _i64, _i32, _p, _p, _i32, _p, _p, _p, _p, _p]),
     "lmg_stencil_smooth_restrict": (_c.c_int, [_i64, _i32, _p, _i32, _p, _p, _c.c_uint32, _i32, _p, _c.c_int, _p, _p, _f64, _p,
                                                _i64, _i32, _p, _p, _i32, _p, _p, _i32, _p, _p]),
+    "lmg_pattern_census_count": (_i64, [_i64, _i32]),
+    "lmg_pattern_census": (_c.c_int, [_i64, _i32, _p, _p, _p, _p]),
+    "lmg_stencil_smooth_census": (_c.c_int, [_i64, _i32, _p, _i32, _p, _p, _c.c_uint32, _i32, _p, _c.c_int, _p, _p, _f64, _p, _p,
+                                             _p, _i32, _p]),
+    "lmg_stencil_smooth_prolong_census": (_c.c_int, [_i64, _i32, _p, _i32, _p, _p, _c.c_uint32, _i32, _p, _c.c_int, _p, _p, _f64, _p,
+                                                     _i64, _i32, _p, _p, _i32, _p, _p, _p, _p, _p, _p, _i32, _p]),
+    "lmg_stencil_smooth_restrict_census": (_c.c_int, [_i64, _i32, _p, _i32, _p, _p, _c.c_uint32, _i32, _p, _c.c_int, _p, _p, _f64, _p,
+                                                      _i64, _i32, _p, _p, _i32, _p, _p, _i32, _p, _p, _i32, _p, _i32, _p]),
+    "lmg_stencil_smooth_uniform_items": (_c.c_int, [_i64, _i32, _c.c_int, _c.c_int, _c.c_int, _c.c_int, _i64, _i32, _p, _p, _p, _p]),
     "lmg_sell_sweep": (_c.c_int, [_c.c_int, _i64, _p, _p, _p, _p, _p, _c.c_int, _p, _i32, _p, _p, _p, _f64, _f64, _p, _p, _p]),
     "lmg_sell_slice_info": (_c.c_int, [_i64, _p, _p, _p, _p, _p, _p]),
     "lmg_sell_fill": (_c.c_int, [_i64, _p, _p, _p, _p, _p, _c.c_int, _p, _p, _p]),
diff --git a/learnmultigrid_amd/csrc/lmg_common.hpp b/learnmultigrid_amd/csrc/lmg_common.hpp
--- a/learnmultigrid_amd/csrc/lmg_common.hpp
+++ b/learnmultigrid_amd/csrc/lmg_common.hpp
@@ -134,6 +134,18 @@
 constexpr unsigned kMaskLower = 0x1C0u;
 constexpr unsigned kMaskCorners = 0x145u;
 constexpr unsigned kMaskOffLine = kMaskUpper | kMaskLower;
+
+constexpr int kLmgCensusCell = 32;
+__host__ __device__ inline int lmg_census_cells(int W) { return (W + kLmgCensusCell - 1) / kLmgCensusCell; }
+__host__ __device__ inline int64_t lmg_census_count(int lines, int W) { return (int64_t)(lines + 1) * (lmg_census_cells(W) + 1); }
+__host__ __device__ inline bool lmg_census_all_expected(const int32_t *table, int lines, int W, int y0, int y1, int x0, int x1)
+{
+    if (!table || y0 < 0 || y1 >= lines || y0 > y1 || x0 < 0 || x1 >= W || x0 > x1) return false;
+    const int64_t cs = lmg_census_cells(W) + 1;
+    const int ca = x0 / kLmgCensusCell, cb = x1 / kLmgCensusCell + 1;
+    const int32_t *lo = table + (int64_t)y0 * cs, *hi = table + (int64_t)(y1 + 1) * cs;
+    return hi[cb] - lo[cb] - hi[ca] + lo[ca] == 0;
+}
 
 
 
diff --git a/learnmultigrid_amd/csrc/stencil_fused.hip b/learnmultigrid_amd/csrc/stencil_fused.hip
--- a/learnmultigrid_amd/csrc/stencil_fused.hip
+++ b/learnmultigrid_amd/csrc/stencil_fused.hip
@@ -59,6 +59,7 @@
     int rp_npat;
     int rhot;
     double rhv[9];
+    const int *cen_a, *cen_p, *cen_r;
 };
 
 template <int H, bool PROL, bool REST> struct StripGeom {
@@ -159,7 +160,7 @@
     int strip, out_y0, out_y1;
 };
 
-__device__ __forceinline__ Item decode_item(const MArgs &a, int item)
+__host__ __device__ __forceinline__ Item decode_item(const MArgs &a, int item)
 {
     Item it;
     const int nb_items = a.nb_strips * a.segs_b;
@@ -191,6 +192,33 @@
     return it;
 }
 
+enum { BODY_GENERAL = 0, BODY_FAST = 1, BODY_UNIFORM = 2 };
+template <int S, bool RESID, bool ZERO>
+constexpr bool kHasUniform = S == 3 && (RESID || !ZERO);
+template <int S, bool RESID, bool ZERO, int PF, bool PROL, bool REST>
+__host__ __device__ __forceinline__ int item_body(const MArgs &a, const Item &it)
+{
+    constexpr int H = S + (RESID ? 1 : 0) - (ZERO ? 1 : 0);
+    constexpr int U = StripGeom<H, PROL, REST>::U, ML = StripGeom<H, PROL, REST>::ML;
+    constexpr int HL = H + (REST ? 1 : 0);
+    const int c0 = it.strip * U - ML;
+    const int y_begin = it.out_y0 - HL - ((it.out_y0 - HL) & 1);
+    const int t_last = it.out_y1 - 1 + S + (RESID ? 1 : 0) + (REST ? 1 : 0);
+    const int y_fetch = y_begin + ((t_last - y_begin) / kUF + 1) * kUF - 1 + PF;
+    bool fast = a.allow_fast && y_begin >= (REST ? S + 2 : 1) && y_fetch <= a.lines - 2 &&
+                (int64_t)y_begin * a.W + c0 >= 0 && (int64_t)y_fetch * a.W + c0 + kStripCols < (int64_t)a.n;
+    if (PROL) fast = fast && (int64_t)((y_fetch + 1) >> 1) * a.Wc + (c0 >> 1) + LMG_WAVE <= (int64_t)a.nc;
+    if (REST) fast = fast && (int64_t)((y_fetch - S) >> 1) * a.Wc + (c0 >> 1) + LMG_WAVE <= (int64_t)a.nc;
+    if (!fast) return BODY_GENERAL;
+    if (!kHasUniform<S, RESID, ZERO>) return BODY_FAST;
+    bool uni = a.hot >= 0 && lmg_census_all_expected(a.cen_a, a.lines, a.W, y_begin, y_fetch, c0, c0 + kStripCols - 1);
+    if (PROL) uni = uni && a.phot[0] >= 0 && a.phot[1] >= 0 && lmg_census_all_expected(a.cen_p, a.lines, a.W, y_begin, y_fetch, c0, c0 + kStripCols - 1);
+    if (REST)
+        uni = uni && a.rhot >= 0 &&
+              lmg_census_all_expected(a.cen_r, a.nc / a.Wc, a.Wc, (y_begin - S) >> 1, (y_fetch - S) >> 1, c0 >> 1, (c0 >> 1) + LMG_WAVE - 1);
+    return uni ? BODY_UNIFORM : BODY_FAST;
+}
+
 struct Tables {
     const double *val;
     const int *mask;
@@ -201,7 +229,7 @@
     const int *rm;
 };
 
-template <int S, unsigned UM, bool RESID, bool ZERO, int PF, bool PROL, bool REST, bool FAST>
+template <int S, unsigned UM, bool RESID, bool ZERO, int PF, bool PROL, bool REST, bool FAST, bool UNI>
 __device__ __forceinline__ void fused_march(const MArgs &a, const Tables &T, const int lane, const int strip, const int out_y0,
                                             const int out_y1)
 {
@@ -250,8 +278,12 @@
             const int64_t i0 = (int64_t)y * W + c0;
 #endif
             L.ok = 3;
-            const unsigned short *pp2 = reinterpret_cast<const unsigned short *>(reinterpret_cast<const char *>(a.pid + i0) + lane2);
-            L.praw = (int)((NTL & 4) ? __builtin_nontemporal_load(pp2) : *pp2);
+            if (!UNI) {
+                const unsigned short *pp2 = reinterpret_cast<const unsigned short *>(reinterpret_cast<const char *>(a.pid + i0) + lane2);
+                L.praw = (int)((NTL & 4) ? __builtin_nontemporal_load(pp2) : *pp2);
+            } else {
+                L.praw = 0;
+            }
             typedef double dv2 __attribute__((ext_vector_type(2), aligned(8)));
             const dv2 *pb = reinterpret_cast<const dv2 *>(reinterpret_cast<const char *>(a.b + i0) + lane16);
             const dv2 bb = (NTL & 1) ? __builtin_nontemporal_load(pb) : *pb;
@@ -266,16 +298,19 @@
                 L.x.x = L.x.y = 0.0;
             }
             if (PROL) {
-                unsigned short twop;
-                __builtin_memcpy(&twop, reinterpret_cast<const char *>(a.ppid + i0) + lane2, 2);
-                L.pp = (int)twop;
+                L.pp = 0;
+                if (!UNI) {
+                    unsigned short twop;
+                    __builtin_memcpy(&twop, reinterpret_cast<const char *>(a.ppid + i0) + lane2, 2);
+                    L.pp = (int)twop;
+                }
                 const int64_t jc0 = (int64_t)((y + 1) >> 1) * a.Wc + (c0 >> 1);
                 L.e = *reinterpret_cast<const double *>(reinterpret_cast<const char *>(a.ec + jc0) + lane8);
             } else {
                 L.pp = 0;
                 L.e = 0.0;
             }
-            if (REST) {
+            if (REST && !UNI) {
                 const int64_t jr0 = (int64_t)((y - S) >> 1) * a.Wc + (c0 >> 1);
                 L.rp = (int)*(reinterpret_cast<const unsigned char *>(a.rpid + jr0) + lane);
             } else {
@@ -418,7 +453,7 @@
                     const double e0 = odd ? e_prev : en, e1 = en;
                     const double e0r = dpp_upper<true>(e0), e1r = dpp_upper<true>(e1);
                     double accA, accB;
-                    if (__all(q2 == (odd ? hotq_odd : hotq_even))) {
+                    if (UNI || __all(q2 == (odd ? hotq_odd : hotq_even))) {
                         if (!odd) {
                             accA = 0.0 + hp[0] * e0;
                             accB = (0.0 + hp[1] * e0) + hp[2] * e0r;
@@ -445,7 +480,7 @@
                 Bq[q0] = bv;
                 X[0][u % 3] = xv;
                 Pq[q0] = FAST ? L.praw : ((okA ? pa : 0) | ((okB ? pb : 0) << 8) | ((L.ok & 3) << 16));
-                Hq[q0] = __all(Pq[q0] == hot2);
+                Hq[q0] = UNI || __all(Pq[q0] == hot2);
             }
             LMG_TRACE(1);
             fetch(t + PF, pre[u % PF]);
@@ -457,7 +492,7 @@
                 const int p2 = Pq[q];
                 const d2 bq = Bq[q];
                 d2 nx;
-                if (Hq[q]) {
+                if (UNI || Hq[q]) {
                     if (ZERO && s == 1) {
                         nx.x = omega * (hrd * bq.x);
                         nx.y = omega * (hrd * bq.y);
@@ -496,7 +531,7 @@
                 const int xm = ((u - S - 2) % 3 + 3) % 3, xc = ((u - S - 1) % 3 + 3) % 3, xp = ((u - S) % 3 + 3) % 3;
                 const int p2 = Pq[q];
                 double accA, accB;
-                if (Hq[q]) {
+                if (UNI || Hq[q]) {
                     apply_rows_hot<UM>(hv, X[S][xm], X[S][xc], X[S][xp], accA, accB);
                 } else {
                     const int pA = p2 & 0xff, pB = (p2 >> 8) & 0xff;
@@ -512,7 +547,7 @@
                     bool emit_line = false;
                     double emit = 0.0;
                     if (!y_odd) {
-                        if (hot_cur) {
+                        if (UNI || hot_cur) {
 #pragma unroll
                             for (int k = 0; k < 3; ++k) acc_cur = acc_cur + hr[3 + k] * wl[k];
                         } else {
@@ -524,7 +559,7 @@
                             }
                         }
                     } else {
-                        if (hot_cur) {
+                        if (UNI || hot_cur) {
 #pragma unroll
                             for (int k = 0; k < 3; ++k) acc_cur = acc_cur + hr[6 + k] * wl[k];
                         } else {
@@ -541,9 +576,9 @@
                         rp_cur = rp_now;
                         sty_cur = y + 1 >= out_y0 && y + 1 < out_y1;
                         st_cur = sty_cur && colA;
-                        hot_cur = __all(!st_cur || rp_cur == a.rhot);
+                        hot_cur = UNI || __all(!st_cur || rp_cur == a.rhot);
                         acc_cur = 0.0;
-                        if (hot_cur) {
+                        if (UNI || hot_cur) {
 #pragma unroll
                             for (int k = 0; k < 3; ++k) acc_cur = acc_cur + hr[k] * wl[k];
                         } else {
@@ -578,7 +613,6 @@
     static_assert(!PROL || (!RESID && !ZERO), "the correction is fused into post-smoothing passes only");
     static_assert(!REST || (RESID && !PROL), "the restriction replaces the store of the residual");
     static_assert(kUF % 3 == 0 && kUF % kNBR == 0 && kUF % PF == 0 && S + 2 <= kNBR, "ring periods");
-    constexpr int H = S + (RESID ? 1 : 0) - (ZERO ? 1 : 0);
     __shared__ double s_val[kMaxPat * 9];
     __shared__ int s_mask[kMaxPat];
     __shared__ double s_rdiag[kMaxPat];
@@ -611,21 +645,31 @@
     const Item it = decode_item(a, item);
     const Tables T = {s_val, s_mask, s_rdiag, s_pv, s_pm, s_rv, s_rm};
 
-    constexpr int U = StripGeom<H, PROL, REST>::U, ML = StripGeom<H, PROL, REST>::ML;
-    constexpr int HL = H + (REST ? 1 : 0);
-    const int c0 = it.strip * U - ML;
-    const int y_begin = it.out_y0 - HL - ((it.out_y0 - HL) & 1);
-    const int t_last = it.out_y1 - 1 + S + (RESID ? 1 : 0) + (REST ? 1 : 0);
-    const int y_fetch = y_begin + ((t_last - y_begin) / kUF + 1) * kUF - 1 + PF;
-    bool fast = a.allow_fast && y_begin >= (REST ? S + 2 : 1) && y_fetch <= a.lines - 2 &&
-                (int64_t)y_begin * a.W + c0 >= 0 && (int64_t)y_fetch * a.W + c0 + kStripCols < (int64_t)a.n;
-    if (PROL) fast = fast && (int64_t)((y_fetch + 1) >> 1) * a.Wc + (c0 >> 1) + LMG_WAVE <= (int64_t)a.nc;
-    if (REST) fast = fast && (int64_t)((y_fetch - S) >> 1) * a.Wc + (c0 >> 1) + LMG_WAVE <= (int64_t)a.nc;
 #ifdef LMG_FUSED_WAVETIME
     const unsigned long long wt0 = __builtin_amdgcn_s_memrealtime();
 #endif
-    if (fast) fused_march<S, UM, RESID, ZERO, PF, PROL, REST, true>(a, T, lane, it.strip, it.out_y0, it.out_y1);
-    else fused_march<S, UM, RESID, ZERO, PF, PROL, REST, false>(a, T, lane, it.strip, it.out_y0, it.out_y1);
+    bool fast;
+    if constexpr (kHasUniform<S, RESID, ZERO>) {
+        const int body = item_body<S, RESID, ZERO, PF, PROL, REST>(a, it);
+        fast = body != BODY_GENERAL;
+        if (body == BODY_UNIFORM) fused_march<S, UM, RESID, ZERO, PF, PROL, REST, true, true>(a, T, lane, it.strip, it.out_y0, it.out_y1);
+        else if (fast) fused_march<S, UM, RESID, ZERO, PF, PROL, REST, true, false>(a, T, lane, it.strip, it.out_y0, it.out_y1);
+        else fused_march<S, UM, RESID, ZERO, PF, PROL, REST, false, false>(a, T, lane, it.strip, it.out_y0, it.out_y1);
+    } else {
+        constexpr int H = S + (RESID ? 1 : 0) - (ZERO ? 1 : 0);
+        constexpr int U = StripGeom<H, PROL, REST>::U, ML = StripGeom<H, PROL, REST>::ML;
+        constexpr int HL = H + (REST ? 1 : 0);
+        const int c0 = it.strip * U - ML;
+        const int y_begin = it.out_y0 - HL - ((it.out_y0 - HL) & 1);
+        const int t_last = it.out_y1 - 1 + S + (RESID ? 1 : 0) + (REST ? 1 : 0);
+        const int y_fetch = y_begin + ((t_last - y_begin) / kUF + 1) * kUF - 1 + PF;
+        fast = a.allow_fast && y_begin >= (REST ? S + 2 : 1) && y_fetch <= a.lines - 2 &&
+               (int64_t)y_begin * a.W + c0 >= 0 && (int64_t)y_fetch * a.W + c0 + kStripCols < (int64_t)a.n;
+        if (PROL) fast = fast && (int64_t)((y_fetch + 1) >> 1) * a.Wc + (c0 >> 1) + LMG_WAVE <= (int64_t)a.nc;
+        if (REST) fast = fast && (int64_t)((y_fetch - S) >> 1) * a.Wc + (c0 >> 1) + LMG_WAVE <= (int64_t)a.nc;
+        if (fast) fused_march<S, UM, RESID, ZERO, PF, PROL, REST, true, false>(a, T, lane, it.strip, it.out_y0, it.out_y1);
+        else fused_march<S, UM, RESID, ZERO, PF, PROL, REST, false, false>(a, T, lane, it.strip, it.out_y0, it.out_y1);
+    }
 #ifdef LMG_FUSED_WAVETIME
     if (lane == 0 && item < LMG_FUSED_WAVETIME) {
         g_fused_wavetime[2 * item] = wt0;
@@ -647,8 +691,10 @@
 int g_fused_slow_pct = 55;
 int g_fused_fast = 1;
 
-template <int S, unsigned UM, bool RESID, bool ZERO, bool PROL = false, bool REST = false>
-int launch4(MArgs a, hipStream_t st)
+constexpr int kPF = 2;
+
+template <int S, bool RESID, bool ZERO, bool PROL, bool REST>
+void decompose(MArgs &a)
 {
     constexpr int H = S + (RESID ? 1 : 0) - (ZERO ? 1 : 0);
     constexpr int U = StripGeom<H, PROL, REST>::U;
@@ -685,8 +731,14 @@
     if (a.edge_lines > 0) a.segs = 2 + (a.lines - 2 * a.edge_lines + seg_lines - 1) / seg_lines;
     else a.segs = (a.lines + seg_lines - 1) / seg_lines;
     a.items = a.nb_strips * a.segs_b + (a.strips - a.nb_strips) * a.segs;
+}
+
+template <int S, unsigned UM, bool RESID, bool ZERO, bool PROL = false, bool REST = false>
+int launch4(MArgs a, hipStream_t st)
+{
+    decompose<S, RESID, ZERO, PROL, REST>(a);
     const int grid = (a.items + kWavesPerBlock - 1) / kWavesPerBlock;
-    hipLaunchKernelGGL((stencil_fused_kernel<S, UM, RESID, ZERO, 2, PROL, REST>), dim3((unsigned)grid), dim3(kBlock), 0, st, a);
+    hipLaunchKernelGGL((stencil_fused_kernel<S, UM, RESID, ZERO, kPF, PROL, REST>), dim3((unsigned)grid), dim3(kBlock), 0, st, a);
     LMG_CHECK_LAUNCH();
     return LMG_OK;
 }
@@ -715,14 +767,30 @@
     });
 }
 
-MArgs own_fields(uint32_t union_mask)
+MArgs own_fields(uint32_t union_mask, const int32_t *cen_a = nullptr, const int32_t *cen_p = nullptr, const int32_t *cen_r = nullptr)
 {
     MArgs a;
     a.umask = union_mask;
     a.strips = a.segs = a.seg_lines = 0;
     a.items = a.nb_strips = a.edge_lines = a.allow_fast = 0;
     a.segs_b = a.seg_lines_b = 1;
+    a.cen_a = cen_a;
+    a.cen_p = cen_p;
+    a.cen_r = cen_r;
     return a;
+}
+
+bool census_fits(const int32_t *table, int32_t census_stride, int32_t grid_stride)
+{
+    return !table || (grid_stride >= 1 && census_stride == lmg_census_cells(grid_stride) + 1);
+}
+
+template <int S, bool RESID, bool ZERO, bool PROL, bool REST>
+int count_bodies(MArgs a, int64_t *counts)
+{
+    decompose<S, RESID, ZERO, PROL, REST>(a);
+    for (int item = 0; item < a.items; ++item) ++counts[item_body<S, RESID, ZERO, kPF, PROL, REST>(a, decode_item(a, item))];
+    return LMG_OK;
 }
 
 }
@@ -745,16 +813,43 @@
 
 extern "C" {
 
+int lmg_stencil_smooth_census(int64_t n, int32_t line_stride, const uint8_t *pid, int32_t npat, const double *st_val,
+                              const int32_t *st_mask, uint32_t union_mask, int32_t hot_pattern, const double *h_hot_val,
+                              int sweeps, const double *x_in, const double *b, double omega, double *x_out, double *r_out,
+                              const int32_t *census, int32_t census_stride, void *stream)
+{
+    if (!census_fits(census, census_stride, line_stride)) return LMG_ERR_ARG;
+    return lmg_fused_pass<kMask5, kMask9, kMask1D>(
+        own_fields(union_mask, census), {n, line_stride, pid, npat, st_val, st_mask, union_mask, hot_pattern, h_hot_val},
+        {sweeps, x_in, b, omega, x_out, r_out}, nullptr, nullptr, [&](const MArgs &a, auto m) {
+            return launch_plain<LMG_CT(m)>(a, sweeps, r_out != nullptr, x_in == nullptr, lmg_stream(stream));
+        });
+}
+
 int lmg_stencil_smooth(int64_t n, int32_t line_stride, const uint8_t *pid, int32_t npat, const double *st_val,
                        const int32_t *st_mask, uint32_t union_mask, int32_t hot_pattern, const double *h_hot_val,
                        int sweeps, const double *x_in, const double *b, double omega, double *x_out, double *r_out,
                        void *stream)
 {
-    return lmg_fused_pass<kMask5, kMask9, kMask1D>(
-        own_fields(union_mask), {n, line_stride, pid, npat, st_val, st_mask, union_mask, hot_pattern, h_hot_val},
-        {sweeps, x_in, b, omega, x_out, r_out}, nullptr, nullptr, [&](const MArgs &a, auto m) {
-            return launch_plain<LMG_CT(m)>(a, sweeps, r_out != nullptr, x_in == nullptr, lmg_stream(stream));
-        });
+    return lmg_stencil_smooth_census(n, line_stride, pid, npat, st_val, st_mask, union_mask, hot_pattern, h_hot_val, sweeps, x_in,
+                                     b, omega, x_out, r_out, nullptr, 0, stream);
+}
+
+int lmg_stencil_smooth_prolong_census(int64_t n, int32_t line_stride, const uint8_t *pid, int32_t npat, const double *st_val,
+                                      const int32_t *st_mask, uint32_t union_mask, int32_t hot_pattern,
+                                      const double *h_hot_val, int sweeps, const double *x_in, const double *b, double omega,
+                                      double *x_out, int64_t n_coarse, int32_t coarse_stride, const double *e_coarse,
+                                      const uint8_t *p_pid, int32_t p_npat, const double *p_val, const int32_t *p_mask,
+                                      const int32_t *h_hot_pairs, const double *h_hot_pval, const int32_t *census,
+                                      const int32_t *p_census, int32_t census_stride, void *stream)
+{
+    if (!census_fits(census, census_stride, line_stride) || !census_fits(p_census, census_stride, line_stride)) return LMG_ERR_ARG;
+    const LmgProl p = {n_coarse, coarse_stride, e_coarse, p_pid, p_npat, p_val, p_mask, h_hot_pairs, h_hot_pval};
+    return lmg_fused_pass<kMask5, kMask9>(
+        own_fields(union_mask, census, p_census),
+        {n, line_stride, pid, npat, st_val, st_mask, union_mask, hot_pattern, h_hot_val},
+        {sweeps, x_in, b, omega, x_out, nullptr}, &p, nullptr,
+        [&](const MArgs &a, auto m) { return launch_prol<LMG_CT(m)>(a, sweeps, lmg_stream(stream)); });
 }
 
 int lmg_stencil_smooth_prolong(int64_t n, int32_t line_stride, const uint8_t *pid, int32_t npat, const double *st_val,
@@ -764,11 +859,26 @@
                                int32_t p_npat, const double *p_val, const int32_t *p_mask, const int32_t *h_hot_pairs,
                                const double *h_hot_pval, void *stream)
 {
-    const LmgProl p = {n_coarse, coarse_stride, e_coarse, p_pid, p_npat, p_val, p_mask, h_hot_pairs, h_hot_pval};
+    return lmg_stencil_smooth_prolong_census(n, line_stride, pid, npat, st_val, st_mask, union_mask, hot_pattern, h_hot_val,
+                                             sweeps, x_in, b, omega, x_out, n_coarse, coarse_stride, e_coarse, p_pid, p_npat,
+                                             p_val, p_mask, h_hot_pairs, h_hot_pval, nullptr, nullptr, 0, stream);
+}
+
+int lmg_stencil_smooth_restrict_census(int64_t n, int32_t line_stride, const uint8_t *pid, int32_t npat, const double *st_val,
+                                       const int32_t *st_mask, uint32_t union_mask, int32_t hot_pattern,
+                                       const double *h_hot_val, int sweeps, const double *x_in, const double *b, double omega,
+                                       double *x_out, int64_t n_coarse, int32_t coarse_stride, double *b_coarse,
+                                       const uint8_t *r_pid, int32_t r_npat, const double *r_val, const int32_t *r_mask,
+                                       int32_t hot_r, const double *h_hot_rval, const int32_t *census, int32_t census_stride,
+                                       const int32_t *r_census, int32_t r_census_stride, void *stream)
+{
+    if (!census_fits(census, census_stride, line_stride) || !census_fits(r_census, r_census_stride, coarse_stride)) return LMG_ERR_ARG;
+    const LmgRest r = {n_coarse, coarse_stride, b_coarse, r_pid, r_npat, r_val, r_mask, hot_r, h_hot_rval};
     return lmg_fused_pass<kMask5, kMask9>(
-        own_fields(union_mask), {n, line_stride, pid, npat, st_val, st_mask, union_mask, hot_pattern, h_hot_val},
-        {sweeps, x_in, b, omega, x_out, nullptr}, &p, nullptr,
-        [&](const MArgs &a, auto m) { return launch_prol<LMG_CT(m)>(a, sweeps, lmg_stream(stream)); });
+        own_fields(union_mask, census, nullptr, r_census),
+        {n, line_stride, pid, npat, st_val, st_mask, union_mask, hot_pattern, h_hot_val},
+        {sweeps, x_in, b, omega, x_out, nullptr}, nullptr, &r,
+        [&](const MArgs &a, auto m) { return launch_rest<LMG_CT(m)>(a, sweeps, x_in == nullptr, lmg_stream(stream)); });
 }
 
 int lmg_stencil_smooth_restrict(int64_t n, int32_t line_stride, const uint8_t *pid, int32_t npat, const double *st_val,
@@ -778,11 +888,36 @@
                                 int32_t r_npat, const double *r_val, const int32_t *r_mask, int32_t hot_r,
                                 const double *h_hot_rval, void *stream)
 {
-    const LmgRest r = {n_coarse, coarse_stride, b_coarse, r_pid, r_npat, r_val, r_mask, hot_r, h_hot_rval};
-    return lmg_fused_pass<kMask5, kMask9>(
-        own_fields(union_mask), {n, line_stride, pid, npat, st_val, st_mask, union_mask, hot_pattern, h_hot_val},
-        {sweeps, x_in, b, omega, x_out, nullptr}, nullptr, &r,
-        [&](const MArgs &a, auto m) { return launch_rest<LMG_CT(m)>(a, sweeps, x_in == nullptr, lmg_stream(stream)); });
+    return lmg_stencil_smooth_restrict_census(n, line_stride, pid, npat, st_val, st_mask, union_mask, hot_pattern, h_hot_val,
+                                              sweeps, x_in, b, omega, x_out, n_coarse, coarse_stride, b_coarse, r_pid, r_npat,
+                                              r_val, r_mask, hot_r, h_hot_rval, nullptr, 0, nullptr, 0, stream);
+}
+
+int lmg_stencil_smooth_uniform_items(int64_t n, int32_t line_stride, int sweeps, int with_residual, int zero_iterate, int form,
+                                     int64_t n_coarse, int32_t coarse_stride, const int32_t *h_census,
+                                     const int32_t *h_p_census, const int32_t *h_r_census, int64_t *h_counts)
+{
+    const bool prol = form == 1, rest = form == 2;
+    if (n < 2 || n >= MArgs::kRowLimit || line_stride < 3 || line_stride > n || sweeps < 1 || sweeps > 3 || form < 0 || form > 2 ||
+        !h_counts)
+        return LMG_ERR_ARG;
+    if ((prol && (with_residual || zero_iterate)) || (rest && !with_residual)) return LMG_ERR_ARG;
+    if ((prol || rest) && (coarse_stride < 1 || n_coarse < coarse_stride || n_coarse >= (1ll << 31))) return LMG_ERR_ARG;
+    MArgs a = own_fields(0, h_census, h_p_census, h_r_census);
+    a.n = (int)n;
+    a.W = line_stride;
+    a.lines = (int)((n + line_stride - 1) / line_stride);
+    a.nc = (prol || rest) ? (int)n_coarse : 0;
+    a.Wc = (prol || rest) ? coarse_stride : 0;
+    a.hot = a.phot[0] = a.phot[1] = a.rhot = 0;
+    h_counts[0] = h_counts[1] = h_counts[2] = 0;
+    return lmg_with_sweeps<1, 3>(sweeps, [&](auto s) {
+        if (prol) return count_bodies<LMG_CT(s), false, false, true, false>(a, h_counts);
+        return lmg_with_flag(zero_iterate != 0, [&](auto z) {
+            if (rest) return count_bodies<LMG_CT(s), true, LMG_CT(z), false, true>(a, h_counts);
+            return lmg_with_flag(with_residual != 0, [&](auto r) { return count_bodies<LMG_CT(s), LMG_CT(r), LMG_CT(z), false, false>(a, h_counts); });
+        });
+    });
 }
 
 int lmg_stencil_smooth_supported(uint32_t union_mask)
diff --git a/learnmultigrid_amd/csrc/vec.hip b/learnmultigrid_amd/csrc/vec.hip
--- a/learnmultigrid_amd/csrc/vec.hip
+++ b/learnmultigrid_amd/csrc/vec.hip
@@ -141,6 +141,60 @@
         if (s_cnt[i]) atomicAdd(&counts[i], s_cnt[i]);
 }
 
+__global__ void __launch_bounds__(kLmgBlock) pattern_census_lines_kernel(int64_t n, int W, int lines, const unsigned char *pid,
+                                                                         unsigned expect, unsigned none, int *table)
+{
+    const int lane = threadIdx.x & (LMG_WAVE - 1);
+    const int row = (int)blockIdx.x * (kLmgBlock / LMG_WAVE) + (int)(threadIdx.x / LMG_WAVE);
+    if (row > lines) return;
+    const int cells = lmg_census_cells(W);
+    int *out = table + (int64_t)row * (cells + 1);
+    if (row == 0) {
+        for (int c = lane; c <= cells; c += LMG_WAVE) out[c] = 0;
+        return;
+    }
+    const int y = row - 1;
+    if (lane == 0) out[0] = 0;
+    int carry = 0;
+    for (int cb = 0; cb < cells; cb += LMG_WAVE) {
+        const int c = cb + lane;
+        int bad = 0;
+        if (c < cells) {
+            for (int k = 0; k < kLmgCensusCell; ++k) {
+                const int x = c * kLmgCensusCell + k;
+                const int64_t i = (int64_t)y * W + x;
+                const int par = ((y & 1) << 1) | (x & 1);
+                const bool ok = x < W && i < n && !((none >> par) & 1u) && pid[i] == ((expect >> (8 * par)) & 0xffu);
+                bad += ok ? 0 : 1;
+            }
+        }
+        for (int d = 1; d < LMG_WAVE; d <<= 1) {
+            const int up = __shfl_up(bad, d, LMG_WAVE);
+            if (lane >= d) bad += up;
+        }
+        if (c < cells) out[c + 1] = carry + bad;
+        carry += __shfl(bad, LMG_WAVE - 1, LMG_WAVE);
+    }
+}
+
+__global__ void __launch_bounds__(kLmgBlock) pattern_census_columns_kernel(int lines, int cells, int *table)
+{
+    const int c = (int)blockIdx.x * kLmgBlock + (int)threadIdx.x + 1;
+    if (c > cells) return;
+    const int64_t cs = cells + 1;
+    int sum = 0;
+    for (int y0 = 1; y0 <= lines; y0 += 8) {
+        int v[8];
+#pragma unroll
+        for (int k = 0; k < 8; ++k) v[k] = y0 + k <= lines ? table[(int64_t)(y0 + k) * cs + c] : 0;
+#pragma unroll
+        for (int k = 0; k < 8; ++k) {
+            sum += v[k];
+            if (y0 + k <= lines) table[(int64_t)(y0 + k) * cs + c] = sum;
+        }
+    }
+}
+
 constexpr int kScanBlock = 1024;
 constexpr int kScanItems = 4;
 constexpr int kScanTile = kScanBlock * kScanItems;
@@ -373,6 +427,33 @@
     return LMG_OK;
 }
 
+int64_t lmg_pattern_census_count(int64_t n, int32_t line_stride)
+{
+    if (n < 1 || line_stride < 1 || (n + line_stride - 1) / line_stride >= INT_MAX) return 0;
+    return lmg_census_count((int)((n + line_stride - 1) / line_stride), line_stride);
+}
+
+int lmg_pattern_census(int64_t n, int32_t line_stride, const uint8_t *pid, const int32_t *h_expected, int32_t *table, void *stream)
+{
+    if (n < 0 || n >= (1ll << 31) - 8 || line_stride < 1 || !h_expected || (n > 0 && (!pid || !table))) return LMG_ERR_ARG;
+    if (n == 0) return LMG_OK;
+    unsigned expect = 0, none = 0;
+    for (int k = 0; k < 4; ++k) {
+        if (h_expected[k] > 255) return LMG_ERR_ARG;
+        if (h_expected[k] < 0) none |= 1u << k;
+        else expect |= (unsigned)h_expected[k] << (8 * k);
+    }
+    const int lines = (int)((n + line_stride - 1) / line_stride), cells = lmg_census_cells(line_stride);
+    constexpr int kWaves = kLmgBlock / LMG_WAVE;
+    hipLaunchKernelGGL(pattern_census_lines_kernel, dim3((unsigned)((lines + 1 + kWaves - 1) / kWaves)), dim3(kLmgBlock), 0,
+                       lmg_stream(stream), n, line_stride, lines, pid, expect, none, table);
+    LMG_CHECK_LAUNCH();
+    hipLaunchKernelGGL(pattern_census_columns_kernel, dim3((unsigned)((cells + kLmgBlock - 1) / kLmgBlock)), dim3(kLmgBlock), 0,
+                       lmg_stream(stream), lines, cells, table);
+    LMG_CHECK_LAUNCH();
+    return LMG_OK;
+}
+
 int64_t lmg_scan_scratch_count(int64_t n)
 {
     int64_t total = 0;
diff --git a/learnmultigrid_amd/hierarchy.py b/learnmultigrid_amd/hierarchy.py
--- a/learnmultigrid_amd/hierarchy.py
+++ b/learnmultigrid_amd/hierarchy.py
@@ -623,6 +623,9 @@
                 for name in ("patterns", "sell", "packed", "dia"):
                     T = getattr(M, name, None) if M is not None else None
                     tot += 0 if T is None else T.bytes()
+                for name in ("stencil", "prolong", "restrict"):
+                    census = getattr(getattr(M, name, None), "census", None)
+                    tot += 0 if census is None else 4 * census.numel()
         return tot
 
     @staticmethod
diff --git a/learnmultigrid_amd/ops.py b/learnmultigrid_amd/ops.py
--- a/learnmultigrid_amd/ops.py
+++ b/learnmultigrid_amd/ops.py
@@ -6,7 +6,7 @@
 from . import _lib
 from ._lib import LmgError, check
 from .twins import (F32, F64, I32, ColorSell, DiaTwin, PackedCSR, ProlongTwin, RestrictTwin, RowPatterns, SellCSR,
-                    StencilTwin, _p, _s, check_values)
+                    StencilTwin, _p, _s, census_stride, check_values)
 
 
 def _vec_ok(*ts):
@@ -296,7 +296,40 @@
             raise LmgError("%s: the register pass folds no transfer into an operator with entries across a line end" % who)
         tail = T.c_args(vec)
     name = "lmg_stencil_%s%s%s" % (stem, "_tiled" if tiled else "", "_" + form if form else "")
+    if not tiled and stem == "smooth" and _FUSED_UNIFORM_ENABLED and S.census is not None:
+        name += "_census"
+        tail += _census_args(S, T if form else None, form)
     check(getattr(_lib.lib(), name)(*S.c_args(), *head, *tail, _s(S.pid)), name)
+
+
+_FUSED_UNIFORM_ENABLED = True
+
+
+def set_fused_uniform_enabled(flag):
+    global _FUSED_UNIFORM_ENABLED
+    _FUSED_UNIFORM_ENABLED = bool(flag)
+
+
+def _census_args(S, T, form):
+    if form is None:
+        return (_p(S.census), census_stride(S.W))
+    if form == "prolong":
+        return (_p(S.census), _p(T.census), census_stride(S.W))
+    return (_p(S.census), census_stride(S.W), _p(T.census), census_stride(T.Wc))
+
+
+def fused_uniform_items(A, sweeps, with_residual=False, zero=False, prolong=None, restrict=None):
+    S = A.stencil
+    form, T = (1, prolong.prolong) if prolong is not None else (2, restrict.restrict) if restrict is not None else (0, None)
+    use = _FUSED_UNIFORM_ENABLED
+    host = [None if (t is None or not use) else t.cpu().numpy() for t in
+            (S.census, T.census if form == 1 else None, T.census if form == 2 else None)]
+    counts = (ctypes.c_int64 * 3)()
+    check(_lib.lib().lmg_stencil_smooth_uniform_items(
+        S.n, S.W, int(sweeps), int(bool(with_residual or form == 2)), int(bool(zero)), form, T.nc if T is not None else 0,
+        T.Wc if T is not None else 0, *[None if h is None else h.ctypes.data for h in host], ctypes.addressof(counts)),
+        "lmg_stencil_smooth_uniform_items")
+    return tuple(int(c) for c in counts)
 
 
 FUSED_TRANSFER_MIN_ROWS = 12_000_000
diff --git a/learnmultigrid_amd/twins.py b/learnmultigrid_amd/twins.py
--- a/learnmultigrid_amd/twins.py
+++ b/learnmultigrid_amd/twins.py
@@ -114,6 +114,26 @@
 
 def _hot_values(values, hot):
     return None if hot < 0 else (ctypes.c_double * 9)(*[float(v) for v in values[hot * 9: hot * 9 + 9]])
+
+
+CENSUS_CELL = 32
+
+
+def census_stride(W):
+    return (int(W) + CENSUS_CELL - 1) // CENSUS_CELL + 1
+
+
+def census_table(pid, n, W, expected):
+    if min(expected) < 0 or not pid.is_cuda:
+        return None
+    L = _lib.lib()
+    count = int(L.lmg_pattern_census_count(int(n), int(W)))
+    if count <= 0:
+        return None
+    table = torch.empty(count, dtype=I32, device=pid.device)
+    exp = (ctypes.c_int32 * 4)(*[int(e) for e in expected])
+    check(L.lmg_pattern_census(int(n), int(W), _p(pid), ctypes.addressof(exp), _p(table), _s(pid)), "lmg_pattern_census")
+    return table
 
 
 class PackedCSR:
@@ -497,7 +517,7 @@
 class StencilTwin:
 
     __slots__ = ("n", "W", "npat", "pid", "st_val", "st_mask", "umask", "bytes_", "patterns", "hot", "_hot_val",
-                 "_gs_ok", "_gs_work", "_line_end")
+                 "_gs_ok", "_gs_work", "_line_end", "census")
     _decompose = staticmethod(_decompose)
 
     @classmethod
@@ -524,6 +544,9 @@
         cand = [p for p in range(R.npat) if st_mask[p] == self.umask and (st_mask[p] & 16) and st_val[p * 9 + 4] != 0.0]
         self.hot = hot_pattern(cand, _pid_counts(R) if len(cand) > 1 else None)
         self._hot_val = _hot_values(st_val, self.hot)
+        self.census = None
+        if self.hot >= 0 and _lib.lib().lmg_stencil_smooth_supported(self.umask):
+            self.census = census_table(R.pid, self.n, self.W, [self.hot] * 4)
         self._gs_work = None
         self._gs_ok = None
         self._line_end = None
@@ -559,7 +582,7 @@
 
 class ProlongTwin:
 
-    __slots__ = ("n", "W", "nc", "Wc", "npat", "pid", "p_val", "p_mask", "_hot_pairs", "_hot_pval", "patterns")
+    __slots__ = ("n", "W", "nc", "Wc", "npat", "pid", "p_val", "p_mask", "_hot_pairs", "_hot_pval", "patterns", "census")
 
     @classmethod
     def from_patterns(cls, R, shape):
@@ -587,6 +610,8 @@
         self.p_mask = torch.from_numpy(p_mask).to(dev)
         self._hot_pairs = (ctypes.c_int32 * 2)(*hot[0])
         self._hot_pval = (ctypes.c_double * 9)(*hot[1])
+        pe, po = hot[0]
+        self.census = census_table(R.pid, n, W, [-1] * 4 if min(pe, po) < 0 else [pe & 255, pe >> 8, po & 255, po >> 8])
         return self
 
     def c_args(self, e):
@@ -596,7 +621,7 @@
 
 class RestrictTwin:
 
-    __slots__ = ("nc", "Wc", "n", "W", "npat", "pid", "r_val", "r_mask", "hot", "_hot_val", "patterns")
+    __slots__ = ("nc", "Wc", "n", "W", "npat", "pid", "r_val", "r_mask", "hot", "_hot_val", "patterns", "census")
 
     @classmethod
     def from_patterns(cls, R, shape):
@@ -621,6 +646,7 @@
         cand = [p for p in range(R.npat) if r_mask[p] == 0x1FF]
         self.hot = hot_pattern(cand, _pid_counts(R) if len(cand) > 1 else None)
         self._hot_val = _hot_values(r_val, self.hot)
+        self.census = census_table(R.pid, self.nc, self.Wc, [self.hot] * 4)
         return self
 
     def c_args(self, bc):
```

Measured after the change: 288.7 billion DoF*sweeps/s, median of 6. 5.1% higher.
